# namada-net/masp

Measured on AMD Instinct MI355X. Metric: Spend proofs/sec, higher is better.
Workload: dtype u32; 1 GPU; BASELINE.json configs[3]: batch of 256 distinct Spend proofs per step on one MI355X (throughput mode); proofs_per_gpu=4352, distinct_witnesses_per_gpu=256, ntt_log2=17, batch_cap=256, slots=4, calls_in_flight=4, hw_queues=4, parallelism=proofs sharded over 1 GPU(s), no data-path collective, gather of the proofs

## Files before the change

### include/masp_hip.h

```cpp
#ifndef MASP_HIP_H
#define MASP_HIP_H
#include <stddef.h>
#include <stdint.h>

#ifdef __cplusplus
extern "C" {
#endif

#define MASP_HIP_OK 0
#define MASP_HIP_E_INVALID_ARG 1
#define MASP_HIP_E_PARAMS_FORMAT 2
#define MASP_HIP_E_PARAMS_SHAPE 3
#define MASP_HIP_E_NO_DEVICE 4
#define MASP_HIP_E_HIP 5
#define MASP_HIP_E_UNEXPECTED_IDENTITY 6
#define MASP_HIP_E_NOT_LOADED 7
#define MASP_HIP_E_SCALAR_RANGE 8
#define MASP_HIP_E_POINT_ENCODING 9
#define MASP_HIP_E_CAPACITY 10

#define MASP_HIP_MAX_CIRCUITS 8
#define MASP_HIP_SPEND 0
#define MASP_HIP_OUTPUT 1
#define MASP_HIP_CONVERT 2

typedef struct masp_hip_ctx masp_hip_ctx;

typedef struct {
    uint32_t n_inputs, n_aux, n_constraints;
    const uint32_t* a_rowptr; const uint32_t* a_col; const uint8_t* a_coef;
    const uint32_t* b_rowptr; const uint32_t* b_col; const uint8_t* b_coef;
    const uint32_t* c_rowptr; const uint32_t* c_col; const uint8_t* c_coef;
} masp_hip_r1cs;

typedef struct {
    uint32_t circuit;
    const uint8_t* inputs;
    const uint8_t* aux;
    const uint8_t* a;
    const uint8_t* b;
    const uint8_t* c;
    uint8_t r[32], s[32];
    uint32_t aux_form;
    uint32_t reserved;
} masp_hip_job;
#define MASP_HIP_AUX_CANONICAL 0
#define MASP_HIP_AUX_MONTGOMERY 1

int masp_hip_device_count(void);
int masp_hip_device_pci_bus_id(int device, char* out, size_t cap);

typedef struct {
    uint32_t struct_size;
    int32_t slots;
    int32_t batch_cap;
    int32_t ntt_sub_batch;
    int32_t window_bits_h;
    int32_t window_bits_la;
    int32_t window_bits_b;
    int32_t window_bits_b2_lone;
    int32_t witness_nontrivial_percent;
    int32_t bucket_tree_levels;
    int32_t bucket_tree_sub_batch;
    int32_t bucket_tree_levels_g2;
    int32_t bucket_tree_scratch_mb;
    int32_t bucket_tree_fallback_proofs;
    int32_t lone_proof_graph;
    int32_t hw_queues;
    int32_t window_bits_h_lone;
    int32_t digit_recoding;
    int32_t window_bits_b2;
} masp_hip_options;
void masp_hip_options_default(masp_hip_options* opt);
#define MASP_HIP_MAX_USEFUL_HW_QUEUES 20
int masp_hip_runtime_prepare(int hw_queues, int overwrite);

int masp_hip_ctx_create(int device, masp_hip_ctx** out);
int masp_hip_ctx_create_ex(const int* devices, int n_devices, const masp_hip_options* opt, masp_hip_ctx** out);
int masp_hip_ctx_get_options(const masp_hip_ctx* ctx, masp_hip_options* out);
int masp_hip_ctx_create_multi(const int* devices, int n_devices, masp_hip_ctx** out);
int masp_hip_ctx_set_boolean_block_bits(masp_hip_ctx* ctx, int32_t bits);
int masp_hip_ctx_get_boolean_block_bits(const masp_hip_ctx* ctx, int32_t* out);
#define MASP_HIP_QUOTIENT_EVALUATION 0
#define MASP_HIP_QUOTIENT_COEFFICIENT 1
int masp_hip_ctx_set_quotient_form(masp_hip_ctx* ctx, int32_t form);
int masp_hip_ctx_get_quotient_form(const masp_hip_ctx* ctx, int32_t* out);
#define MASP_HIP_QUOTIENT_FUSED 0
#define MASP_HIP_QUOTIENT_SEPARATE 1
int masp_hip_ctx_set_quotient_schedule(masp_hip_ctx* ctx, int32_t schedule);
int masp_hip_ctx_get_quotient_schedule(const masp_hip_ctx* ctx, int32_t* out);
int masp_hip_ctx_set_tree_entry_share(masp_hip_ctx* ctx, int32_t percent);
int masp_hip_ctx_get_tree_entry_share(const masp_hip_ctx* ctx, int32_t* out);
int masp_hip_r1cs_boolean_variables(const masp_hip_r1cs* cs, uint8_t* out);
uint64_t masp_hip_tree_entry_bound(uint32_t n, int32_t window_bits, uint32_t n_witness, uint32_t n_boolean, int32_t share_percent);
int masp_hip_circuit_tree_entry_bounds(const masp_hip_ctx* ctx, uint32_t slot, uint64_t bounds[4], int32_t window_bits[4]);
int masp_hip_ctx_device_count(const masp_hip_ctx* ctx);
int masp_hip_ctx_device_proofs(const masp_hip_ctx* ctx, uint64_t* counts, int cap);
int masp_hip_ctx_device_status(const masp_hip_ctx* ctx, int32_t* status, int cap, uint64_t* requeued);
int masp_hip_ctx_inject_fault(masp_hip_ctx* ctx, int device, uint32_t nth);
int masp_hip_ctx_stream_concurrency(masp_hip_ctx* ctx, int mains_only, int* n_streams, int* concurrent);
int masp_hip_ctx_lone_graph_launches(const masp_hip_ctx* ctx, uint64_t* out);
void masp_hip_ctx_destroy(masp_hip_ctx* ctx);
const char* masp_hip_strerror(int code);
const char* masp_hip_last_error(const masp_hip_ctx* ctx);

int masp_hip_circuit_load(masp_hip_ctx* ctx, uint32_t slot, const uint8_t* params, size_t params_len, const masp_hip_r1cs* cs);
#define MASP_HIP_CIRCUIT_G1_ENDOMORPHISM 1u
int masp_hip_circuit_flags(const masp_hip_ctx* ctx, uint32_t slot, uint32_t* flags);

int masp_hip_circuit_quotient_form(const masp_hip_ctx* ctx, uint32_t slot, int32_t* form);
int masp_hip_circuit_eval_bases(const masp_hip_ctx* ctx, uint32_t slot, uint8_t* bases, size_t cap_points, size_t* n_points, uint32_t* input_cols,
                                size_t cap_inputs, size_t* n_input_cols);

int masp_hip_prove(masp_hip_ctx* ctx, uint32_t slot, const uint8_t* inputs, const uint8_t* aux, const uint8_t* a,
                   const uint8_t* b, const uint8_t* c, const uint8_t r[32], const uint8_t s[32], uint8_t proof_out[192]);
int masp_hip_prove_batch(masp_hip_ctx* ctx, size_t n, const masp_hip_job* jobs, uint8_t* proofs_out);

int masp_hip_generate_parameters(masp_hip_ctx* ctx, const masp_hip_r1cs* cs, const uint8_t toxic[160], uint8_t* out, size_t cap,
                                 size_t* out_len);
size_t masp_hip_parameters_max_size(const masp_hip_r1cs* cs);

int masp_hip_msm_g1(masp_hip_ctx* ctx, const uint8_t* bases, const uint8_t* scalars, size_t n, uint8_t out[96]);
int masp_hip_msm_g2(masp_hip_ctx* ctx, const uint8_t* bases, const uint8_t* scalars, size_t n, uint8_t out[192]);
int masp_hip_msm_g1_multi(masp_hip_ctx* ctx, const uint8_t* bases, size_t n, const uint8_t* scalars, size_t np, int window_bits,
                          uint8_t* out);
int masp_hip_msm_g2_multi(masp_hip_ctx* ctx, const uint8_t* bases, size_t n, const uint8_t* scalars, size_t np, int window_bits,
                          uint8_t* out);
int masp_hip_msm_g1_multi_ex(masp_hip_ctx* ctx, const uint8_t* bases, size_t n, const uint8_t* scalars, size_t np, int window_bits,
                             int block_bits, size_t sub_lo, size_t sub_hi, uint8_t* out, uint32_t* bucket0_entries);
int masp_hip_msm_g2_multi_ex(masp_hip_ctx* ctx, const uint8_t* bases, size_t n, const uint8_t* scalars, size_t np, int window_bits,
                             int block_bits, size_t sub_lo, size_t sub_hi, uint8_t* out, uint32_t* bucket0_entries);
int masp_hip_quotient_h(masp_hip_ctx* ctx, const uint8_t* a, const uint8_t* b, const uint8_t* c, size_t nrows,
                        uint32_t logm, uint8_t* h_out);
int masp_hip_ntt(masp_hip_ctx* ctx, uint8_t* data, uint32_t logm, int inverse);

typedef struct masp_hip_vk masp_hip_vk;
int masp_hip_vk_prepare(masp_hip_ctx* ctx, const uint8_t* params, size_t params_len, masp_hip_vk** out);
void masp_hip_vk_free(masp_hip_vk* vk);
int masp_hip_verify_batch(masp_hip_ctx* ctx, masp_hip_vk* vk, size_t n, const uint8_t* proofs, const uint8_t* public_inputs,
                          uint32_t n_public, const uint8_t* z, int* all_valid);
int masp_hip_verify_each(masp_hip_ctx* ctx, masp_hip_vk* vk, size_t n, const uint8_t* proofs, const uint8_t* public_inputs,
                         uint32_t n_public, uint8_t* verdicts);
int masp_hip_verify_each_last_timing(masp_hip_vk* vk, double ms[5]);

int masp_hip_jubjub_msm(masp_hip_ctx* ctx, size_t n, const uint8_t* points, const uint8_t* scalars, uint8_t out32[32], int64_t* bad_index);
int masp_hip_redjubjub_verify_batch(masp_hip_ctx* ctx, size_t n, const uint8_t* vks, const uint8_t* sigs, const uint8_t* sighashes,
                                    const uint8_t* kinds, const uint8_t* z, int* all_valid);
int masp_hip_redjubjub_verify_each(masp_hip_ctx* ctx, size_t n, const uint8_t* vks, const uint8_t* sigs, const uint8_t* sighashes,
                                   const uint8_t* kinds, uint8_t* verdicts);

int masp_hip_sapling_trial_decrypt(masp_hip_ctx* ctx, size_t n_ivk, const uint8_t* ivks, size_t n_out, const uint8_t* epks,
                                   const uint8_t* enc_ciphertexts, uint8_t* epk_status, size_t hit_capacity, uint32_t* hit_output,
                                   uint32_t* hit_ivk, uint8_t* hit_keys, size_t* n_hits);
int masp_hip_note_scan_configure(masp_hip_ctx* ctx, int signed_digits, int inversion);
int masp_hip_note_scan_last_timing(masp_hip_ctx* ctx, double ms[2]);

int masp_hip_sapling_compact_trial_decrypt(masp_hip_ctx* ctx, size_t n_ivk, const uint8_t* ivks, size_t n_out, const uint8_t* epks,
                                           const uint8_t* cmus, const uint8_t* enc_compact, int lead_byte, uint8_t* epk_status,
                                           size_t hit_capacity, uint32_t* hit_output, uint32_t* hit_ivk, uint8_t* hit_plaintexts,
                                           uint8_t* hit_pk_d, size_t* n_hits, size_t* n_candidates);
int masp_hip_note_scan_compact_last_timing(masp_hip_ctx* ctx, double ms[3]);

int masp_hip_sapling_output_recovery_scan(masp_hip_ctx* ctx, size_t n_ovk, const uint8_t* ovks, size_t n_out, const uint8_t* cvs,
                                          const uint8_t* epks, const uint8_t* cmus, const uint8_t* out_ciphertexts, size_t hit_capacity,
                                          uint32_t* hit_output, uint32_t* hit_ovk, uint8_t* hit_ocks, size_t* n_hits);
int masp_hip_out_recovery_last_timing(masp_hip_ctx* ctx, double ms[2]);

int masp_hip_merkle_tree_complete(masp_hip_ctx* ctx, unsigned height0, size_t n, const uint8_t* row, uint8_t* nodes_out, size_t nodes_capacity,
                                  size_t* n_nodes, uint8_t root32[32], size_t n_paths, const uint64_t* positions, uint8_t* paths_out,
                                  int64_t* bad_index);
int masp_hip_merkle_last_timing(masp_hip_ctx* ctx, double ms[3]);
int masp_hip_merkle_tree_append(masp_hip_ctx* ctx, uint64_t start, const uint8_t frontier[32 * 32], size_t n, const uint8_t* row,
                                uint8_t* nodes_out, size_t nodes_capacity, size_t* n_nodes, int64_t* bad_index);

int masp_hip_batch_upload(masp_hip_ctx* ctx, size_t n, const masp_hip_job* jobs);
int masp_hip_batch_prove_resident(masp_hip_ctx* ctx, int handle, uint8_t* proofs_out, float* elapsed_ms);
int masp_hip_batch_prove_resident_steps(masp_hip_ctx* ctx, int handle, size_t steps, const uint8_t* rs, uint8_t* proofs_out,
                                        float* elapsed_ms);
int masp_hip_batch_free(masp_hip_ctx* ctx, int handle);
int masp_hip_bench_msm(masp_hip_ctx* ctx, int handle, size_t job, int which, int iters, float* avg_ms, uint32_t* n_bases);

int masp_hip_profile_enable(masp_hip_ctx* ctx, int on);
int masp_hip_profile_read(masp_hip_ctx* ctx, double* total_ms, uint64_t* launches, uint64_t* alg_bytes);
int masp_hip_profile_read_split(masp_hip_ctx* ctx, double ms[8]);
int masp_hip_profile_read_lone(masp_hip_ctx* ctx, double ms[12]);
void* masp_hip_host_alloc(masp_hip_ctx* ctx, size_t bytes);
void masp_hip_host_free(masp_hip_ctx* ctx, void* ptr);
int masp_hip_sync(masp_hip_ctx* ctx);

#ifdef __cplusplus
}
#endif

// ... 22 lines not shown
```

### masp_amd/csrc/device/msm.hpp

```cpp
#pragma once
#include <hip/hip_runtime.h>

#include "curve.hpp"
#include "quad.hpp"
#include "oct.hpp"
#include "io.hpp"
#include "msm_geom.h"

namespace masp {

#define MSM_P (blockIdx.y)

template <class O, int BYTES>
__global__ void k_msm_import(const uint8_t* __restrict__ raw, TabRow<O>* __restrict__ tab, uint32_t n, int* __restrict__ status) {
    uint32_t i = blockIdx.x * blockDim.x + threadIdx.x;
    if (i >= n) return;
    Affine<O> p;
    int st;
    if constexpr (BYTES == 96)
        st = g1_read_uncompressed(raw + (size_t)i * 96, p);
    else
        st = g2_read_uncompressed(raw + (size_t)i * 192, p);
    if (st & ~PT_INFINITY) {
        atomicOr(status, st);
        p.x = O::zero();
        p.y = O::zero();
    } else if (st & PT_INFINITY) {
        atomicOr(status, PT_INFINITY);
    }
    tab[i].p = p;
}
template <class O>
__global__ void __launch_bounds__(64) k_msm_precompute(TabRow<O>* __restrict__ tab, uint32_t n, int c, int W) {
    uint32_t i = blockIdx.x * blockDim.x + threadIdx.x;
    if (i >= n) return;
    Affine<O> p = tab[i].p;
    for (int j = 1; j < W; ++j) {
        Xyzz<O> q = xyzz_dbl_affine(p);
        for (int k = 1; k < c; ++k) q = xyzz_dbl(q);
        p = xyzz_to_affine(q);
        tab[(size_t)j * n + i].p = p;
    }
}
template <class O>
__global__ void __launch_bounds__(64) k_msm_subset_rows(TabRow<O>* __restrict__ tab, MsmSubset sub, uint32_t n_rows) {
    const uint32_t r = blockIdx.x * blockDim.x + threadIdx.x;
    if (r >= n_rows) return;
    const uint32_t per = sub.patterns(), rb = r / per, pattern = r % per + 1u, i0 = (sub.b_first + rb) << sub.bits;
    Xyzz<O> acc = xyzz_inf<O>();
    for (uint32_t t = 0; t < (1u << sub.bits); ++t)
        if ((pattern >> t) & 1u) xyzz_madd_nc(acc, tab[i0 + t].p, false);
    if (xyzz_is_inf(acc)) atomicOr(&sub.bad[rb >> 5], 1u << (rb & 31u));
    tab[(size_t)sub.row0 + r].p = xyzz_to_affine(acc);
}


#ifndef MASP_TAIL_MIN_WAVES
#define MASP_TAIL_MIN_WAVES 1
#endif
template <class O>
__device__ __forceinline__ Xyzz<O> xyzz_load(const Xyzz<typename O::Base>* __restrict__ p, uint32_t h) {
    if constexpr (O::PARTS == 1) {
        const Xyzz<typename O::Base> v = *p;
        return reinterpret_cast<const Xyzz<O>&>(v);
    } else {
        const typename O::T* q = reinterpret_cast<const typename O::T*>(p);
        const uint32_t part = h % O::PARTS;
        Xyzz<O> r;
        r.X = q[part];
        r.Y = q[O::PARTS + part];
        r.ZZ = q[2 * O::PARTS + part];
        r.ZZZ = q[3 * O::PARTS + part];
        return r;
    }
}
template <class O>
__device__ __forceinline__ void xyzz_store(Xyzz<typename O::Base>* __restrict__ p, const Xyzz<O>& v, uint32_t h) {
    if constexpr (O::PARTS == 1) {
        if (h == 0) *p = reinterpret_cast<const Xyzz<typename O::Base>&>(v);
    } else {
        if (h >= O::PARTS) return;
        typename O::T* q = reinterpret_cast<typename O::T*>(p);
        q[h] = v.X;
        q[O::PARTS + h] = v.Y;
        q[2 * O::PARTS + h] = v.ZZ;
        q[3 * O::PARTS + h] = v.ZZZ;
    }
}
template <class O>
__global__ void __launch_bounds__(64, MASP_TAIL_MIN_WAVES)
k_msm_bucket_gather(const Xyzz<typename O::Base>* __restrict__ part, const uint32_t* __restrict__ start, uint32_t nb, uint32_t nchunks,
                    Xyzz<typename O::Base>* __restrict__ bkt, uint32_t* __restrict__ heavy, uint32_t* __restrict__ n_heavy, uint32_t heavy_span) {
    constexpr uint32_t LN = O::LANES;
    const uint32_t b = (blockIdx.x * blockDim.x + threadIdx.x) / LN, h = threadIdx.x % LN;
    if (b >= nb) return;
    part += (size_t)MSM_P * ((size_t)nchunks + nb);
    start += (size_t)MSM_P * (nb + 1);
    bkt += (size_t)MSM_P * nb;
    heavy += (size_t)MSM_P * nb;
    n_heavy += MSM_P;
    const uint32_t s0 = start[b], s1 = start[b + 1];
    Xyzz<O> acc = xyzz_inf<O>();
    if (s1 > s0) {
        const uint32_t K = msm_chunk_len(start[nb], nchunks);
        const uint32_t c0 = s0 / K, c1 = (s1 - 1) / K;
        if (c1 - c0 >= heavy_span) {
            if (h == 0) heavy[atomicAdd(n_heavy, 1u)] = b;
            return;
        }
        acc = xyzz_load<O>(part + c0 + b, h);
        for (uint32_t c = c0 + 1; c <= c1; ++c) xyzz_add_nc(acc, xyzz_load<O>(part + c + b, h));
    }
    xyzz_store<O>(bkt + b, acc, h);
}
template <class O>
__global__ void __launch_bounds__(64, MASP_TAIL_MIN_WAVES)
k_msm_bucket_gather_split(const Xyzz<typename O::Base>* __restrict__ part, const uint32_t* __restrict__ start, uint32_t nb, uint32_t nchunks,
                          Xyzz<typename O::Base>* __restrict__ bkt, uint32_t* __restrict__ heavy, uint32_t* __restrict__ n_heavy, uint32_t heavy_span,
                          uint32_t nbw) {
    constexpr uint32_t LN = O::LANES;
    const uint32_t h = threadIdx.x % LN;
    part += (size_t)MSM_P * ((size_t)nchunks + nb);
    start += (size_t)MSM_P * (nb + 1);
    bkt += (size_t)MSM_P * nb;
    heavy += (size_t)MSM_P * nb;
// ... 35 lines not shown
}
template <class O>
__device__ __forceinline__ Xyzz<O> xyzz_shfl_down(const Xyzz<O>& p, int d) {
    Xyzz<O> r;
    const uint32_t* src = reinterpret_cast<const uint32_t*>(&p);
    uint32_t* dst = reinterpret_cast<uint32_t*>(&r);
#pragma unroll
    for (uint32_t i = 0; i < sizeof(Xyzz<O>) / 4; ++i) dst[i] = (uint32_t)__shfl_down((int)src[i], d, 64);
    return r;
}
template <class O, uint32_t THREADS, uint32_t SPLIT = 1>
__global__ void __launch_bounds__(THREADS, MASP_TAIL_MIN_WAVES)
k_msm_bucket_heavy(const Xyzz<typename O::Base>* __restrict__ part, const uint32_t* __restrict__ start, uint32_t nb, uint32_t nchunks,
                   Xyzz<typename O::Base>* __restrict__ bkt, const uint32_t* __restrict__ heavy, const uint32_t* __restrict__ n_heavy,
                   Xyzz<typename O::Base>* __restrict__ hparts) {
    constexpr uint32_t LN = O::LANES, WE = 64 / LN, EL = THREADS / LN;
    __shared__ Xyzz<typename O::Base> sh[THREADS / 64];
    const uint32_t tid = threadIdx.x, e = tid / LN, h = tid % LN, le = (tid & 63) / LN, wid = tid >> 6;
    part += (size_t)MSM_P * ((size_t)nchunks + nb);
    start += (size_t)MSM_P * (nb + 1);
    bkt += (size_t)MSM_P * nb;
    heavy += (size_t)MSM_P * nb;
    n_heavy += MSM_P;
    if constexpr (SPLIT > 1) hparts += (size_t)MSM_P * MSM_HEAVY_SLOTS;
    const uint32_t nh = *n_heavy;
    const uint32_t K = msm_chunk_len(start[nb], nchunks);
    const uint32_t share = blockIdx.x % SPLIT, nwg = gridDim.x / SPLIT;
    for (uint32_t hb = blockIdx.x / SPLIT; hb < nh; hb += nwg) {
        const uint32_t b = heavy[hb];
        uint32_t c0 = start[b] / K, c1 = (start[b + 1] - 1) / K;
        const bool split = SPLIT > 1 && hb < MSM_HEAVY_SLOTS / SPLIT;
        if (split) {
            const uint32_t len = (c1 - c0 + SPLIT) / SPLIT;
            c0 += share * len;
            c1 = c0 + len - 1 < c1 ? c0 + len - 1 : c1;
        } else if (share != 0) {
            continue;
        }
        Xyzz<O> acc = xyzz_inf<O>();
        for (uint32_t c = c0 + e; c <= c1 && c1 + 1 > c0; c += EL) xyzz_add_nc(acc, xyzz_load<O>(part + c + b, h));
        const uint32_t span = c1 + 1 > c0 ? c1 - c0 + 1 : 0;
        for (uint32_t d = WE / 2; d >= 1; d >>= 1) {
            if (d >= span) continue;
            Xyzz<O> other = xyzz_shfl_down(acc, (int)(d * LN));
            if (le < d) xyzz_add_nc(acc, other);
        }
        if constexpr (THREADS > 64) {
            if (le == 0) xyzz_store<O>(sh + wid, acc, h);
            __syncthreads();
            if (e == 0)
                for (uint32_t w = 1; w < THREADS / 64; ++w) xyzz_add_nc(acc, xyzz_load<O>(sh + w, h));
        }
        if (e == 0) xyzz_store<O>(split ? hparts + hb * SPLIT + share : bkt + b, acc, h);
        if constexpr (THREADS > 64) __syncthreads();
    }
}
template <class O, uint32_t SPLIT>
__global__ void __launch_bounds__(64, MASP_TAIL_MIN_WAVES)
k_msm_heavy_join(const Xyzz<typename O::Base>* __restrict__ hparts, const uint32_t* __restrict__ heavy, const uint32_t* __restrict__ n_heavy, uint32_t nb,
                 Xyzz<typename O::Base>* __restrict__ bkt) {
    constexpr uint32_t LN = O::LANES, PER = 64 / (LN * SPLIT);
    static_assert(PER >= 1, "a bucket's shares fit one wave");
    const uint32_t e = threadIdx.x / LN, h = threadIdx.x % LN, share = e % SPLIT, hb = blockIdx.x * PER + e / SPLIT;
    hparts += (size_t)MSM_P * MSM_HEAVY_SLOTS;
    heavy += (size_t)MSM_P * nb;
    bkt += (size_t)MSM_P * nb;
    const uint32_t nh = n_heavy[MSM_P], lim = nh < MSM_HEAVY_SLOTS / SPLIT ? nh : MSM_HEAVY_SLOTS / SPLIT;
    if (hb >= lim) return;
    Xyzz<O> acc = xyzz_load<O>(hparts + hb * SPLIT + share, h);
    for (uint32_t d = SPLIT / 2; d >= 1; d >>= 1) {
        Xyzz<O> other = xyzz_shfl_down(acc, (int)(d * LN));
        if (share < d) xyzz_add_nc(acc, other);
    }
    if (share == 0) xyzz_store<O>(bkt + heavy[hb], acc, h);
}

#ifndef MASP_WSUM_PAIR_WAVES
#define MASP_WSUM_PAIR_WAVES 2
#endif
template <class O>
constexpr uint32_t wsum_points_log() {
    return O::LANES > 4 ? WSUM_L_LOG - 1 : WSUM_L_LOG;
}
template <class O, uint32_t G_LOG>
__global__ void __launch_bounds__((1u << wsum_points_log<O>()) * O::LANES, (O::LANES > 1 ? MASP_WSUM_PAIR_WAVES : sizeof(Xyzz<O>) > 200 || G_LOG < 3 ? MASP_TAIL_MIN_WAVES : 2))
k_msm_wsum_level(const Xyzz<typename O::Base>* __restrict__ B, size_t b_stride, uint32_t m, uint32_t off, Xyzz<typename O::Base>* __restrict__ S,
                 Xyzz<typename O::Base>* __restrict__ T, size_t st_stride) {
    constexpr uint32_t LP = 1u << wsum_points_log<O>(), GL = G_LOG + WSUM_L_LOG - wsum_points_log<O>(), G = 1u << GL, CS = G * LP, LN = O::LANES,
                       WE = 64 / LN, NW = LP / WE;
    __shared__ Xyzz<typename O::Base> sh[2][NW];
    const uint32_t tid = threadIdx.x, e = tid / LN, h = tid % LN, le = (tid & 63) / LN, wid = tid >> 6;
    B += MSM_P * b_stride;
    S += MSM_P * st_stride;
    T += MSM_P * st_stride;
    const uint32_t base = blockIdx.x * CS + e * G;
    Xyzz<O> run = xyzz_inf<O>(), acc = xyzz_inf<O>();
    for (uint32_t l = G; l-- > 0;) {
        if (base + l < m) xyzz_add_nc(run, xyzz_load<O>(B + base + l, h));
        if (l > 0 || off) xyzz_add_nc(acc, run);
    }
    Xyzz<O> x = run;
    for (uint32_t d = 1; d < WE; d <<= 1) {
        Xyzz<O> other = xyzz_shfl_down(x, (int)(d * LN));
        if (le + d < WE) xyzz_add_nc(x, other);
    }
    static_assert(NW <= WE, "the waves' totals fit the points of one wave");
    if (le == 0) xyzz_store<O>(&sh[0][wid], x, h);
    __syncthreads();
    if constexpr (NW > 1) {
        if (wid == 0) {
            Xyzz<O> v = le < NW ? xyzz_load<O>(&sh[0][le], h) : xyzz_inf<O>();
            for (uint32_t d = 1; d < NW; d <<= 1) {
                Xyzz<O> other = xyzz_shfl_down(v, (int)(d * LN));
                if (le + d < NW) xyzz_add_nc(v, other);
            }
            Xyzz<O> behind = xyzz_shfl_down(v, (int)LN);
            if (le + 1 < NW) xyzz_store<O>(&sh[0][le], behind, h);
        }
        __syncthreads();
        if (wid + 1 < NW) xyzz_add_nc(x, xyzz_load<O>(&sh[0][wid], h));
    }
    Xyzz<O> y = e > 0 ? x : xyzz_inf<O>();
    for (uint32_t k = 0; k < GL; ++k) y = xyzz_dbl(y);
    xyzz_add_nc(y, acc);
    for (uint32_t d = WE / 2; d >= 1; d >>= 1) {
        Xyzz<O> other = xyzz_shfl_down(y, (int)(d * LN));
        if (le < d) xyzz_add_nc(y, other);
    }
    if (le == 0) xyzz_store<O>(&sh[1][wid], y, h);
    __syncthreads();
    if (wid == 0) {
        if constexpr (NW > 1) {
            y = le < NW ? xyzz_load<O>(&sh[1][le], h) : xyzz_inf<O>();
            for (uint32_t d = NW / 2; d >= 1; d >>= 1) {
                Xyzz<O> other = xyzz_shfl_down(y, (int)(d * LN));
                if (le < d) xyzz_add_nc(y, other);
            }
        }
        if (e == 0) {
            xyzz_store<O>(S + blockIdx.x, x, h);
            xyzz_store<O>(T + blockIdx.x, y, h);
        }
    }
}
template <class O>
__global__ void __launch_bounds__(256) k_xyzz_reduce_block(const Xyzz<O>* __restrict__ in, size_t in_stride, uint32_t n,
                                                           Xyzz<O>* __restrict__ out, size_t out_stride) {
    extern __shared__ uint4 wsum_lds[];
    Xyzz<O>* sh = reinterpret_cast<Xyzz<O>*>(wsum_lds);
    const uint32_t tid = threadIdx.x;
    in += MSM_P * in_stride;
    out += MSM_P * out_stride;
    const uint32_t k = blockIdx.x * 256 + tid;
    Xyzz<O> y = k < n ? in[k] : xyzz_inf<O>();
    for (uint32_t d = 128; d >= 1; d >>= 1) {
        sh[tid] = y;
        __syncthreads();
        if (tid < d) xyzz_add_nc(y, sh[tid + d]);
        __syncthreads();
    }
    if (tid == 0) out[blockIdx.x] = y;
}
template <class O>
__global__ void __launch_bounds__(64) k_msm_combine(const Xyzz<O>* __restrict__ tsum, int levels, int cs_log, Xyzz<O>* __restrict__ out, size_t out_stride) {
    if (blockIdx.x != 0 || threadIdx.x != 0) return;
    tsum += (size_t)MSM_P * 32;
    out += MSM_P * out_stride;
    Xyzz<O> acc = xyzz_inf<O>();
    for (int l = levels - 1; l >= 0; --l) {
        for (int k = 0; k < cs_log; ++k) acc = xyzz_dbl(acc);
        xyzz_add_nc(acc, tsum[l]);
    }
    *out = acc;
}

template <class O>
constexpr uint32_t reduce_lanes_points() {
    return O::LANES > 4 ? 64u : 256u;
}
template <class O>
__global__ void __launch_bounds__(reduce_lanes_points<O>() * O::LANES) k_xyzz_reduce_block_lanes(const Xyzz<typename O::Base>* __restrict__ in, size_t in_stride, uint32_t n,
                                                                            Xyzz<typename O::Base>* __restrict__ out, size_t out_stride) {
    extern __shared__ uint4 wsum_lds[];
    constexpr uint32_t PTS = reduce_lanes_points<O>();
    Xyzz<typename O::Base>* sh = reinterpret_cast<Xyzz<typename O::Base>*>(wsum_lds);
    const uint32_t e = threadIdx.x / O::LANES, h = threadIdx.x % O::LANES;
    in += MSM_P * in_stride;
    out += MSM_P * out_stride;
    const uint32_t k = blockIdx.x * PTS + e;
    Xyzz<O> y = k < n ? xyzz_load<O>(in + k, h) : xyzz_inf<O>();
    for (uint32_t d = PTS / 2; d >= 1; d >>= 1) {
        xyzz_store<O>(sh + e, y, h);
        __syncthreads();
        if (e < d) xyzz_add_nc(y, xyzz_load<O>(sh + e + d, h));
        __syncthreads();
    }
    if (e == 0) xyzz_store<O>(out + blockIdx.x, y, h);
}
template <class O>
__global__ void __launch_bounds__(64) k_msm_combine_lanes(const Xyzz<typename O::Base>* __restrict__ tsum, int levels, int cs_log,
                                                          Xyzz<typename O::Base>* __restrict__ out, size_t out_stride) {
    if (blockIdx.x != 0 || threadIdx.x >= O::LANES) return;
    const uint32_t h = threadIdx.x;
    tsum += (size_t)MSM_P * 32;
    out += MSM_P * out_stride;
    Xyzz<O> acc = xyzz_inf<O>();
    for (int l = levels - 1; l >= 0; --l) {
        for (int k = 0; k < cs_log; ++k) acc = xyzz_dbl(acc);
        xyzz_add_nc(acc, xyzz_load<O>(tsum + l, h));
    }
    xyzz_store<O>(out, acc, h);
}

}
```

### masp_amd/csrc/device/msm_geom.h

```cpp
#pragma once
#include <hip/hip_runtime.h>

#include <cstdint>

namespace masp {

struct MsmGeom {
    int c;
    int W;
    int nb;
};
static inline MsmGeom msm_geom(int c) {
    MsmGeom g;
    g.c = c;
    g.W = (256 + c - 1) / c;
    g.nb = 1 << (c - 1);
    return g;
}
static inline uint32_t msm_mean_digits_x16(const MsmGeom& g) { return (uint32_t)g.W * 16; }

__host__ __device__ static inline uint32_t msm_chunk_len(uint32_t total, uint32_t nchunks) {
    uint32_t k = (total + nchunks - 1) / nchunks;
    return k < 4 ? 4 : k;
}

struct MsmSubset {
    uint32_t bits = 0;
    uint32_t b_first = 0, b_end = 0;
    uint32_t row0 = 0;
    uint32_t* bad = nullptr;
    __host__ __device__ uint32_t bad_words() const { return (b_end - b_first + 31) / 32; }
    __host__ __device__ uint32_t patterns() const { return (1u << (1u << bits)) - 1u; }
    __host__ __device__ uint64_t rows() const { return bits ? (uint64_t)(b_end - b_first) * patterns() : 0; }
};
__host__ __device__ static inline uint32_t msm_range_len(uint32_t n, uint32_t ng) { return ((n + ng - 1) / ng + 63u) & ~63u; }

static constexpr unsigned WSUM_L_LOG = 7, WSUM_L = 1u << WSUM_L_LOG;
static constexpr unsigned WSUM_G_LOG_MIN = 2;
static constexpr unsigned MSM_HEAVY_SPLIT = 8, MSM_HEAVY_SLOTS = 2048;
static constexpr unsigned MSM_SORT_THREADS = 1024;
static constexpr uint32_t MSM_PAD_ENTRY = 0xffffffffu;

}
```

### masp_amd/csrc/device/msm_sort.hpp

```cpp
#pragma once
#include <hip/hip_runtime.h>

#include <cstdint>

#include "msm_geom.h"

namespace masp {

#define MSM_P (blockIdx.y)

struct MsmDigitIter {
    const uint32_t* sw;
    uint32_t carry, mask, half, pos, j;
    int c;
    __device__ __forceinline__ MsmDigitIter(const uint32_t* sw_, const MsmGeom& g)
        : sw(sw_), carry(0), mask((1u << g.c) - 1u), half(1u << (g.c - 1)), pos(0), j(0), c(g.c) {}
    __device__ __forceinline__ uint32_t bits(uint32_t bit) const {
        const uint32_t w = bit >> 5, off = bit & 31u;
        const uint64_t two = ((uint64_t)(w + 1 < 8 ? sw[w + 1] : 0u) << 32) | sw[w];
        return (uint32_t)(two >> off);
    }
    __device__ __forceinline__ bool next(uint32_t& table, uint32_t& bucket, uint32_t& neg) {
        uint32_t v = (bits(pos) & mask) + carry;
        table = j++;
        pos += (uint32_t)c;
        neg = 0;
        carry = 0;
        if (v > half) {
            v = (1u << c) - v;
            neg = 1;
            carry = 1;
        }
        bucket = v - 1;
        return v != 0;
    }
};
__device__ __forceinline__ int msm_scalar_class(const uint32_t* sw) {
    const uint4* sp = reinterpret_cast<const uint4*>(sw);
    uint4 lo = sp[0], hi = sp[1];
    uint32_t rest = lo.y | lo.z | lo.w | hi.x | hi.y | hi.z | hi.w;
    if (rest == 0 && lo.x <= 1) return (int)lo.x;
    return 2;
}
__device__ __forceinline__ uint64_t msm_unit_lanes(int cls, uint32_t i, const MsmSubset& sub, uint32_t& entry) {
    const uint64_t ones = __ballot(cls == 1);
    entry = i;
    if (sub.bits == 0) return ones;
    const uint32_t lane = threadIdx.x & 63u, k = 1u << sub.bits, blk = i >> sub.bits;
    bool covered = false;
    if (cls <= 1 && blk >= sub.b_first && blk < sub.b_end) {
        const uint32_t rb = blk - sub.b_first;
        covered = ((sub.bad[rb >> 5] >> (rb & 31u)) & 1u) == 0;
    }
    const uint64_t boolean = __ballot(covered);
    const uint32_t g0 = lane & ~(k - 1u);
    const uint64_t gm = (uint64_t)((1u << k) - 1u) << g0;
    const bool full = (boolean & gm) == gm;
    const uint32_t pattern = (uint32_t)((ones & gm) >> g0);
    const bool lead = full && lane == g0 && pattern != 0;
    if (lead) entry = sub.row0 + (blk - sub.b_first) * sub.patterns() + pattern - 1u;
    return __ballot(full ? lead : cls == 1);
}
__global__ void __launch_bounds__(1024)
k_msm_hist(const uint32_t* __restrict__ scalars, size_t scalar_stride, uint32_t n, MsmGeom g, uint32_t ng, MsmSubset sub, uint32_t* __restrict__ hist_wg) {
    extern __shared__ uint32_t msm_lds[];
    const uint32_t tid = threadIdx.x, wg = blockIdx.x, nb = (uint32_t)g.nb;
    scalars += MSM_P * scalar_stride;
    hist_wg += ((size_t)MSM_P * ng + wg) * nb;
    for (uint32_t b = tid; b < nb; b += MSM_SORT_THREADS) msm_lds[b] = 0;
    __syncthreads();
    const uint32_t per = msm_range_len(n, ng), lo = wg * per, hi = lo < n && lo + per < n ? lo + per : n;
    for (uint32_t base = lo; base < hi; base += MSM_SORT_THREADS) {
        const uint32_t i = base + tid;
        const uint32_t* sw = scalars + (size_t)i * 8;
        const int cls = i < hi ? msm_scalar_class(sw) : 0;
        uint32_t unit_entry;
        const uint64_t units = msm_unit_lanes(cls, i, sub, unit_entry);
        if (cls != 2) {
            if (units && (uint32_t)__ffsll((unsigned long long)units) - 1u == (tid & 63u)) atomicAdd(&msm_lds[0], (uint32_t)__popcll(units));
        } else {
            MsmDigitIter it(sw, g);
            for (int j = 0; j < g.W; ++j) {
                uint32_t table, bucket, neg;
                if (it.next(table, bucket, neg)) atomicAdd(&msm_lds[bucket], 1u);
            }
        }
    }
    __syncthreads();
    for (uint32_t b = tid; b < nb; b += MSM_SORT_THREADS) hist_wg[b] = msm_lds[b];
}
__global__ void __launch_bounds__(256)
k_msm_offsets_cols(uint32_t* __restrict__ hist_wg, uint32_t ng, uint32_t nb, uint32_t* __restrict__ dense) {
    hist_wg += (size_t)MSM_P * ng * nb;
    dense += (size_t)MSM_P * (nb + 1);
    const uint32_t b = blockIdx.x * blockDim.x + threadIdx.x;
    if (b >= nb) return;
    uint32_t v = 0;
    for (uint32_t w0 = 0; w0 < ng; w0 += 16) {
        uint32_t h[16];
#pragma unroll
        for (uint32_t k = 0; k < 16; ++k) h[k] = w0 + k < ng ? hist_wg[(size_t)(w0 + k) * nb + b] : 0u;
#pragma unroll
        for (uint32_t k = 0; k < 16; ++k)
            if (w0 + k < ng) {
                hist_wg[(size_t)(w0 + k) * nb + b] = v;
                v += h[k];
            }
    }
    dense[b] = v;
}
static constexpr uint32_t MSM_SCAN_BLOCK = 1024;
__global__ void __launch_bounds__(256)
k_msm_offsets_scan_a(uint32_t nb, uint32_t* __restrict__ start, uint32_t* __restrict__ dense, uint32_t pad_log, uint2* __restrict__ btot) {
    __shared__ uint32_t wsum[2][4];
    start += (size_t)MSM_P * (nb + 1);
    dense += (size_t)MSM_P * (nb + 1);
// ... 298 lines not shown
```

### masp_amd/csrc/internal.h

```cpp
#pragma once
#include <hip/hip_runtime.h>

#include <algorithm>
#include <array>
#include <condition_variable>
#include <cstring>
#include <deque>
#include <map>
#include <memory>
#include <mutex>
#include <shared_mutex>
#include <string>
#include <thread>
#include <vector>

#include "chunk_pipeline.h"
#include "host/eval_form.h"
#include "device/io.hpp"
#include "device/ntt_geom.h"
#include "launch.h"
#include "msm_host.h"
#include <atomic>
#include "util.h"

#ifndef MASP_SUBSET_BITS
#define MASP_SUBSET_BITS 2
#endif
static_assert(MASP_SUBSET_BITS == 0 || MASP_SUBSET_BITS == 2 || MASP_SUBSET_BITS == 3, "subset blocks are 4 or 8 bases wide");
#ifndef MASP_TREE_ENTRY_SHARE
#define MASP_TREE_ENTRY_SHARE 100
#endif
static_assert(MASP_TREE_ENTRY_SHARE >= 1 && MASP_TREE_ENTRY_SHARE <= 100, "a percentage");


namespace masp {

template <class T>
struct DevBuf {
    T* p = nullptr;
    size_t cap = 0;
    ~DevBuf() { release(); }
    void release() {
        if (p) dev_free(p);
        p = nullptr;
        cap = 0;
    }
    int reserve(size_t n) {
        if (n <= cap) return MASP_HIP_OK;
        release();
        HIP_TRY(dev_malloc(&p, sizeof(T) * std::max<size_t>(n, 1)));
        cap = n;
        return MASP_HIP_OK;
    }
    int upload(const T* h, size_t n, hipStream_t s) {
        int rc = reserve(n);
        if (rc) return rc;
        if (n) HIP_TRY(hipMemcpyAsync(p, h, sizeof(T) * n, hipMemcpyHostToDevice, s));
        return MASP_HIP_OK;
    }
};

static inline Fr fr_from_u64_mont(uint64_t x) {
    Fr v = fe_zero<FrCfg>();
    v.v[0] = (uint32_t)x;
    v.v[1] = (uint32_t)(x >> 32);
    return fe_to_mont(v);
}
static inline Fr fr_const(const uint32_t* limbs) {
    Fr v;
    for (int i = 0; i < 8; ++i) v.v[i] = limbs[i];
    return v;
}

struct NttDomain {
    uint32_t logm = 0;
    size_t m = 0;
    DevBuf<Fr> tw_fwd, tw_inv, coset_scale, h_scale;
    DevBuf<Fr> coset_scale_rev;
    Fr c_scale;
    Fr e_scale;
    int init(uint32_t logm_, hipStream_t s) {
        logm = logm_;
        m = (size_t)1 << logm;
        Fr omega = fr_const(FrCfg::ROOT_OF_UNITY);
        for (uint32_t i = logm; i < 32; ++i) omega = fe_sqr(omega);
        Fr omega_inv = fe_inv(omega);
        Fr minv = fe_inv(fr_from_u64_mont(m));
        Fr g = fr_const(FrCfg::GEN), ginv = fr_const(FrCfg::GEN_INV);
        uint32_t e[2] = {(uint32_t)m, (uint32_t)((uint64_t)m >> 32)};
        const Fr zinv = fe_inv(fe_sub(fe_pow(g, e, 2), fe_one<FrCfg>()));
        const Fr mzinv = fe_mul(minv, zinv);
        c_scale = fe_from_mont(mzinv);
        e_scale = fe_from_mont(zinv);
        Fr one = fe_one<FrCfg>();
        size_t half = std::max<size_t>(m / 2, 1);
        int rc;
        if ((rc = tw_fwd.reserve(half)) || (rc = tw_inv.reserve(half)) || (rc = coset_scale.reserve(m)) || (rc = h_scale.reserve(m))) return rc;
        launch_fr_powers(s, tw_fwd.p, (uint32_t)half, omega, one, 0);
        launch_fr_powers(s, tw_inv.p, (uint32_t)half, omega_inv, one, 0);
        launch_fr_powers(s, coset_scale.p, (uint32_t)m, g, minv, 0);
        launch_fr_powers(s, h_scale.p, (uint32_t)m, ginv, mzinv, 1);
        if (ntt_fused_ok(logm)) {
            if ((rc = coset_scale_rev.reserve(m))) return rc;
            launch_fr_powers_bitrev(s, coset_scale_rev.p, logm, g, minv);
        }
        HIP_TRY(hipStreamSynchronize(s));
        return MASP_HIP_OK;
    }
    void passes(hipStream_t s, Fr* data, const Fr* tw, uint32_t np = 1) const {
        for (uint32_t s0 = 0; s0 < logm;) {
            uint32_t nst = std::min<uint32_t>(NTT_LT, logm - s0);
            launch_ntt_pass(s, data, tw, logm, s0, nst, np);
            s0 += nst;
        }
    }
};

struct Circuit {
    uint32_t n_inputs = 0, n_aux = 0, n_constraints = 0, nrows = 0, logm = 0;
    size_t m = 0;
    DevBuf<uint32_t> rowptr[3], col[3];
    DevBuf<uint32_t> row_order[3];
    uint32_t n_long_rows[3] = {0, 0, 0};
    DevBuf<Fr> coef[3];
    DevBuf<uint32_t> a_var, b_var;
    uint32_t na = 0, nbq = 0;
    DevBuf<VkDevice> vk;
    DevBuf<G1Xyzz> fb1;
    DevBuf<G2Xyzz> fb2;
    BasesG1 h, l, a, b1;
    BasesG1 hl;
    BasesG1 hl_eval;
    DevBuf<uint32_t> eval_in_var;
    uint32_t n_eval_in = 0;
    std::vector<uint32_t> eval_inputs;
    BasesG2 b2;
    BasesG2 b2_lone;
    bool g1_endo = false;
    NttDomain* dom = nullptr;
};

struct Slot {
    hipStream_t stream = nullptr;
    hipEvent_t done = nullptr;
    MsmWorkspace<FpOps> ws1;
    MsmWorkspace<Fp2Ops> ws2;
    static constexpr int N_AUX = 4;
    hipStream_t aux[N_AUX] = {nullptr, nullptr, nullptr, nullptr};
    hipEvent_t ev_fork = nullptr, ev_sort_b = nullptr, ev_fixed = nullptr, ev_join[N_AUX] = {nullptr, nullptr, nullptr, nullptr};
    hipEvent_t ev_uploaded = nullptr;
    MsmWorkspace<FpOps> ws_l, ws_a, ws_b;
    DevBuf<Fr> w, inp, abc, wm, ev[3], x0, x1, h, hl, sa, sb;
    DevBuf<G1Xyzz> res1, asm1;
    DevBuf<G2Xyzz> res2, asm2;
    DevBuf<uint32_t> rs;
    DevBuf<uint8_t> proof;
    DevBuf<int> flags;
    MsmProfile prof;
    bool profiling = false;
    static constexpr int N_LONE_MARKS = 12;
    hipEvent_t ev_lone[N_LONE_MARKS] = {};
    bool lone_marked = false;
    void lone_mark(hipStream_t st, int id) {
        if (!profiling) return;
        if (!ev_lone[id] && hipEventCreate(&ev_lone[id]) != hipSuccess) return;
        (void)hipEventRecord(ev_lone[id], st);
        if (id == N_LONE_MARKS - 1) lone_marked = true;
    }
    uint32_t ntt_sub = 8;
    const std::atomic<int>* quotient_schedule = nullptr;
    uint8_t* h_stage = nullptr;
    size_t h_stage_cap = 0;
    uint8_t* h_proof = nullptr;
    size_t h_proof_cap = 0;
    int* h_flags = nullptr;
    struct LoneGraph {
        const void *circuit, *w, *abc, *rs, *proof;
        size_t w_stride;
        uint32_t np;
        bool mont;
        int runs;
        bool dead;
        hipGraphExec_t exec;
    };
    std::vector<LoneGraph> graphs;
    uint64_t graph_epoch = 0;
    bool lone_graph = false;
    std::atomic<uint64_t> graph_launches{0};
    void drop_graphs() {
        for (auto& g : graphs)
            if (g.exec) hipGraphExecDestroy(g.exec);
        graphs.clear();
    }
    ~Slot() {
        drop_graphs();
        if (done) hipEventDestroy(done);
        for (hipEvent_t e : ev_join)
            if (e) hipEventDestroy(e);
        for (hipEvent_t e : ev_lone)
            if (e) hipEventDestroy(e);
        if (ev_fork) hipEventDestroy(ev_fork);
        if (ev_uploaded) hipEventDestroy(ev_uploaded);
        if (ev_sort_b) hipEventDestroy(ev_sort_b);
        if (ev_fixed) hipEventDestroy(ev_fixed);
        if (h_stage) hipHostFree(h_stage);
        if (h_proof) hipHostFree(h_proof);
        if (h_flags) hipHostFree(h_flags);
    }
    void configure(const masp_hip_options& o) {
        ntt_sub = (uint32_t)o.ntt_sub_batch;
        ws1.tree_levels = o.bucket_tree_levels;
        ws2.tree_levels = o.bucket_tree_levels_g2;
        ws1.tree_levels_shared = o.bucket_tree_levels_g2;
        ws1.tree_sub = ws2.tree_sub = (uint32_t)o.bucket_tree_sub_batch;
        ws2.tree.arena = &ws1.tree.own;
        ws1.tree.own.limit = (size_t)o.bucket_tree_scratch_mb << 20;
        lone_graph = o.lone_proof_graph > 0;
    }
    int init(const std::array<hipStream_t, 5>& streams) {
        stream = streams[0];
        for (int i = 0; i < N_AUX; ++i) aux[i] = streams[1 + i];
        HIP_TRY(hipEventCreateWithFlags(&done, hipEventDisableTiming));
        HIP_TRY(hipEventCreateWithFlags(&ev_fork, hipEventDisableTiming));
        HIP_TRY(hipEventCreateWithFlags(&ev_uploaded, hipEventDisableTiming));
        HIP_TRY(hipEventCreateWithFlags(&ev_sort_b, hipEventDisableTiming));
        HIP_TRY(hipEventCreateWithFlags(&ev_fixed, hipEventDisableTiming));
        for (hipEvent_t& e : ev_join) HIP_TRY(hipEventCreateWithFlags(&e, hipEventDisableTiming));
        HIP_TRY(hipHostMalloc(&h_flags, sizeof(int)));
        int rc;
        if ((rc = flags.reserve(1))) return rc;
        return reserve_batch(1);
    }
    int reserve_batch(size_t np) {
        int rc;
        if ((rc = res1.reserve(4 * np)) || (rc = res2.reserve(np)) || (rc = asm1.reserve(6 * np)) || (rc = asm2.reserve(np)) || (rc = rs.reserve(16 * np)) || (rc = proof.reserve(192 * np))) return rc;
        if (np > h_proof_cap) {
            if (h_proof) hipHostFree(h_proof);
            h_proof = nullptr;
            HIP_TRY(hipHostMalloc(&h_proof, 192 * np));
            h_proof_cap = np;
        }
        return MASP_HIP_OK;
    }
    int stage_reserve(size_t bytes) {
        if (bytes <= h_stage_cap) return MASP_HIP_OK;
        if (h_stage) hipHostFree(h_stage);
        h_stage = nullptr;
        HIP_TRY(hipHostMalloc(&h_stage, bytes));
        h_stage_cap = bytes;
        return MASP_HIP_OK;
    }
};

struct ResidentBatch {
    size_t n = 0;
    std::vector<uint32_t> circuit;
    std::vector<size_t> order;
    std::vector<size_t> w_off;
    DevBuf<Fr> w;
    DevBuf<uint32_t> rs;
};

struct StreamTable {
    hipStream_t main = nullptr;
    std::vector<std::array<hipStream_t, 5>> slot;
    hipStream_t vk[2] = {nullptr, nullptr};
    std::vector<hipStream_t> distinct() const {
        std::vector<hipStream_t> out;
        auto add = [&](hipStream_t s) {
            if (s && std::find(out.begin(), out.end(), s) == out.end()) out.push_back(s);
        };
        add(main);
        for (const auto& row : slot)
            for (hipStream_t s : row) add(s);
        for (hipStream_t s : vk) add(s);
        return out;
    }
    ~StreamTable() {
        for (hipStream_t s : distinct()) (void)hipStreamDestroy(s);
    }
};

}

using masp::Circuit;
using masp::DevBuf;
using masp::Fr;
using masp::G1Affine;
using masp::G1Xyzz;
using masp::G2Affine;
using masp::G2Xyzz;
using masp::NttDomain;
using masp::ResidentBatch;
using masp::Slot;

struct masp_hip_ctx {
    static constexpr size_t MAX_SLOTS = 64;
    int device = 0;
    std::vector<masp_hip_ctx*> children;
    masp_hip_options opt{};
    int boolean_block_bits = MASP_SUBSET_BITS;
    int quotient_form = 0;
    std::atomic<int> quotient_schedule{0};
    int tree_entry_share = MASP_TREE_ENTRY_SHARE;
    int n_slots = 4;
    size_t batch_cap = 256;
    std::shared_mutex mu;
    mutable std::mutex slot_mu;
    std::condition_variable slot_cv;
    std::vector<char> slot_busy;
    std::string err;
    masp::StreamTable streams;
    std::unique_ptr<Circuit> circ[MASP_HIP_MAX_CIRCUITS];
    std::map<uint32_t, std::unique_ptr<NttDomain>> domains;
    std::vector<std::unique_ptr<Slot>> slots;
    std::vector<std::unique_ptr<ResidentBatch>> batches;
    bool profiling = false;
    std::atomic<uint64_t> proofs_done{0};
    std::unique_ptr<std::atomic<int>[]> dev_status;
    std::atomic<uint64_t> requeued{0};
    std::atomic<uint32_t> fault_countdown{0};
    std::atomic<unsigned> vk_next{0};
    int main_streams_concurrent = 0;
    std::mutex upload_mu;
    hipEvent_t upload_tail = nullptr;
    std::atomic<uint64_t> block_tree_fallbacks{0};
    std::atomic<uint32_t> block_tree_sub{0xffffffffu};
    DevBuf<Fr> tmp_scalars;
    DevBuf<uint8_t> tmp_out;
    DevBuf<G1Xyzz> tmp_g1;
    DevBuf<G2Xyzz> tmp_g2;
    DevBuf<G1Affine> fb_g1;
    DevBuf<G2Affine> fb_g2;
    std::mutex jj_mu;
    DevBuf<uint8_t> jj_points, jj_scalars, jj_partial;
    DevBuf<int> jj_status;
    DevBuf<uint32_t> jj_out;
    struct NoteScanSet {
        DevBuf<uint8_t> epk, raw, ct, pts, status, hit_keys;
        DevBuf<uint32_t> count, hit_idx;
    };
    std::mutex ns_mu;
    NoteScanSet ns[2];
    DevBuf<uint32_t> ns_digits;
    std::atomic<int> ns_signed_digits{1}, ns_inversion{0};
    double ns_last_ms[2] = {0, 0};
    struct NoteScanCompactSet {
        DevBuf<uint8_t> cmu, enc, cand, state, hit_idx, hit_data;
        DevBuf<uint32_t> count, list;
    };
    NoteScanCompactSet nsc[2];
    DevBuf<uint8_t> nsc_ivks;
    DevBuf<uint8_t> nsc_table;
    double nsc_last_ms[3] = {0, 0, 0};
    struct OutRecoverySet {
        DevBuf<uint8_t> cv, cmu, epk, cout, cols, hit_ocks;
        DevBuf<uint32_t> count, hit_idx;
    };
    OutRecoverySet orc[2];
    DevBuf<uint32_t> orc_ovks;
    double orc_last_ms[2] = {0, 0};
    DevBuf<uint32_t> mt_nodes, mt_bad, mt_paths, mt_empties;
    DevBuf<uint64_t> mt_pos;
    double mt_last_ms[3] = {0, 0, 0};
};

namespace masp {

static inline int fail(masp_hip_ctx* ctx, int rc) {
    if (rc == MASP_HIP_E_HIP) {
        std::lock_guard<std::mutex> g(ctx->slot_mu);
        ctx->err = last_hip_error();
    }
    return rc;
}

#define FIRST_DEVICE(ctx) ((ctx) && !(ctx)->children.empty() ? (ctx)->children[0] : (ctx))

static inline int get_domain(masp_hip_ctx* ctx, uint32_t logm, NttDomain** out) {
    auto it = ctx->domains.find(logm);
    if (it == ctx->domains.end()) {
        std::unique_ptr<NttDomain> d(new NttDomain);
        int rc = d->init(logm, ctx->streams.main);
        if (rc) return rc;
// ... 26 lines not shown
```

### masp_amd/csrc/k_msm_g1_lone.hip

```cpp
#define MASP_TAILS_QUAD_UNIT
#include "msm_impl.hpp"

namespace masp {
template void msm_tails_enqueue<FpOps, FpQuadOps>(hipStream_t, MsmWorkspace<FpOps>&, const uint32_t*, uint32_t, uint32_t, uint32_t, bool, Xyzz<FpOps>*, size_t);
}
```

### masp_amd/csrc/k_msm_g2_lone.hip

```cpp
#define MASP_TAILS_OCT_UNIT
#include "msm_impl.hpp"

namespace masp {
template void msm_tails_enqueue<Fp2Ops, Fp2OctOps>(hipStream_t, MsmWorkspace<Fp2Ops>&, const uint32_t*, uint32_t, uint32_t, uint32_t, bool, Xyzz<Fp2Ops>*, size_t);
}
```

### masp_amd/csrc/k_msm_sort.hip

```cpp
#include <cstring>

#include "device/msm_sort.hpp"
#include "msm_host.h"

namespace masp {

int msm_sort_enqueue(hipStream_t s, uint32_t n, const MsmGeom& g, MsmSortBuf& sb, const uint32_t* d_scalars, size_t scalar_stride,
                                   uint32_t np, uint32_t pad_log, const MsmSubset& sub) {
    static_assert((1u << 15) / MSM_SCAN_BLOCK <= 64, "k_msm_offsets_scan_b: a wave's lanes fetch the block totals");
    if (g.c < 2 || g.nb > (1 << 15)) {
        last_hip_error() = "MSM window width must be 2..16 bits: the bucket histogram lives in LDS";
        return MASP_HIP_E_INVALID_ARG;
    }
    const uint64_t rows = (uint64_t)n * (uint32_t)g.W + sub.rows();
    if (rows > 0x7ffffffeull) {
        last_hip_error() = "msm_sort_enqueue: the base set has more table rows than an entry's 31 bits can name";
        return MASP_HIP_E_INVALID_ARG;
    }
    if (sub.bits && ((sub.bits != 2 && sub.bits != 3) || sub.b_end < sub.b_first || ((uint64_t)sub.b_end << sub.bits) > n || sub.row0 != n * (uint32_t)g.W ||
                     !sub.bad)) {
        last_hip_error() = "msm_sort_enqueue: subset rows that do not belong to this base set";
        return MASP_HIP_E_INVALID_ARG;
    }
    if (pad_log > 12) {
        last_hip_error() = "msm_sort_enqueue: runs can be aligned to at most 2^12 entries";
        return MASP_HIP_E_INVALID_ARG;
    }
    int rc = sb.reserve(n, g, np, pad_log, rows);
    if (rc) return rc;
    sb.n = n;
    sb.np = np;
    sb.g = g;
    sb.pad_log = pad_log;
    sb.ent_stride = MsmSortBuf::padded_entries(n, g, pad_log);
    const uint32_t ng = MsmSortBuf::ranges_for(n, np), nb = g.nb;
    const uint32_t wide = MsmSortBuf::msm_rows_wide(rows) ? 1u : 0u;
    const int part_entry = wide ? 6 : 5, part_fixed = 4 * (4 * 256 + 8), part_w_max = std::min(30, (160 * 1024 - part_fixed) / ((int)MSM_PART_TILE * part_entry));
    const bool two_pass = nb >= MSM_FINE && g.W <= part_w_max && (uint64_t)(nb >> MSM_FINE_LOG) * np >= 8;
    const int part_lds = part_fixed + part_entry * (int)MSM_PART_TILE * g.W;
    static PerDeviceOnce once;
    const bool lds_ok = once([] {
        int bytes = 4 << 15;
        const int part_bytes = 4 * (4 * 256 + 8) + 5 * (int)MSM_PART_TILE * 30;
        return hipFuncSetAttribute((const void*)k_msm_hist, hipFuncAttributeMaxDynamicSharedMemorySize, bytes) == hipSuccess &&
               hipFuncSetAttribute((const void*)k_msm_scatter, hipFuncAttributeMaxDynamicSharedMemorySize, bytes) == hipSuccess &&
               hipFuncSetAttribute((const void*)k_msm_partition, hipFuncAttributeMaxDynamicSharedMemorySize, part_bytes) == hipSuccess;
    });
    if (!lds_ok) {
        last_hip_error() = "hipFuncSetAttribute(MaxDynamicSharedMemorySize) failed";
        return MASP_HIP_E_HIP;
    }
    MASP_LAUNCH(k_msm_hist, dim3(ng, np), dim3(MSM_SORT_THREADS), 4 * nb, s, d_scalars, scalar_stride, n, g, ng, sub, sb.hist_wg);
    MASP_LAUNCH(k_msm_offsets_cols, dim3((nb + 255) / 256, np), dim3(256), 0, s, sb.hist_wg, ng, nb, sb.dense);
    const uint32_t scan_blocks = (nb + MSM_SCAN_BLOCK - 1) / MSM_SCAN_BLOCK;
    MASP_LAUNCH(k_msm_offsets_scan_a, dim3(scan_blocks, np), dim3(256), 0, s, nb, sb.start, sb.dense, pad_log, sb.btot);
    MASP_LAUNCH(k_msm_offsets_scan_b, dim3(scan_blocks, np), dim3(256), 0, s, nb, sb.start, sb.dense, sb.btot);
    if (two_pass) {
        const uint32_t nbins = nb >> MSM_FINE_LOG;
        const uint32_t cw = std::min(ng, 4u);
        MASP_LAUNCH(k_msm_coarse, dim3(nbins, np, (ng + cw - 1) / cw), dim3(64 * cw), 0, s, sb.hist_wg, ng, nb, sb.crel);
        MASP_LAUNCH(k_msm_partition, dim3(ng, np), dim3(MSM_PART_TILE), part_lds, s, d_scalars, scalar_stride, n, g, ng, sub, sb.crel, sb.dense, sb.tmp, sb.tmpf, wide);
        MASP_LAUNCH(k_msm_bucketize, dim3(nbins, np), dim3(1024), 0, s, sb.tmp, sb.tmpf, (size_t)n * g.W, sb.dense, sb.start, nb, sb.sorted, sb.ent_stride, wide);
    } else {
        if (pad_log) HIP_TRY(hipMemsetAsync(sb.sorted, 0xff, 4 * sb.ent_stride * np, s));
        MASP_LAUNCH(k_msm_scatter, dim3(ng, np), dim3(MSM_SORT_THREADS), 4 * nb, s, d_scalars, scalar_stride, n, g, ng, sub, sb.hist_wg, sb.start, sb.sorted,
                        sb.ent_stride);
    }
    return launch_status();
}

}
```

### masp_amd/csrc/msm_host.h

```cpp
#pragma once
#include <hip/hip_runtime.h>

#include <cstdio>
#include <vector>

#include "device/curve.hpp"
#include "device/msm_geom.h"
#include "util.h"

#ifndef MASP_LONE_NARROW_LANES_LOG
#define MASP_LONE_NARROW_LANES_LOG 16
#endif
namespace masp {

template <class O, int BYTES>
struct MsmBases {
    MsmGeom g{};
    uint32_t n = 0;
    uint32_t n_eff = 0;
    uint64_t ent_bound = 0;
    static uint64_t entry_bound(uint32_t n_, const MsmGeom& g_, uint64_t n_full) {
        n_full = std::min<uint64_t>(n_full, n_);
        return n_full * (uint32_t)g_.W + (n_ - n_full);
    }
    size_t tree_entries(uint32_t pad_log) const {
        const size_t unit = (size_t)1 << pad_log, worst = ((size_t)n * g.W + (size_t)g.nb * (unit - 1) + unit - 1) / unit * unit;
        if (!ent_bound) return worst;
        return std::min<size_t>(worst, ((size_t)ent_bound + (size_t)g.nb * (unit - 1) + unit - 1) / unit * unit);
    }
    TabRow<O>* tab = nullptr;
    int import_status = 0;
    MsmSubset sub;
    uint32_t sub_lo = 0, sub_hi = 0;
    const MsmSubset& subset() const { return sub; }
    uint64_t rows() const { return (uint64_t)n * (uint32_t)g.W + sub.rows(); }

    ~MsmBases() { release(); }
    void release() {
        if (tab) dev_free(tab);
        if (sub.bad) dev_free(sub.bad);
        tab = nullptr;
        sub = MsmSubset();
    }
    static MsmGeom pick_geom(uint32_t n_eff) {
        int c = n_eff >= (1u << 16) ? 16 : n_eff >= (1u << 12) ? 12 : n_eff >= (1u << 8) ? 10 : 7;
        return msm_geom(c);
    }
    int load_device(const uint8_t* d_raw, uint32_t n_, hipStream_t s, uint32_t n_eff = 0xffffffffu, int force_c = 0, int sub_bits_ = 0,
                    uint32_t sub_lo_ = 0, uint32_t sub_hi_ = 0xffffffffu);
    int load_host(const uint8_t* raw, uint32_t n_, hipStream_t s, uint32_t n_eff = 0xffffffffu, int force_c = 0, int sub_bits_ = 0, uint32_t sub_lo_ = 0,
                  uint32_t sub_hi_ = 0xffffffffu) {
        uint8_t* d_raw = nullptr;
        if (n_) {
            HIP_TRY(dev_malloc(&d_raw, (size_t)n_ * BYTES));
            HIP_TRY(hipMemcpyAsync(d_raw, raw, (size_t)n_ * BYTES, hipMemcpyHostToDevice, s));
        }
        int rc = load_device(d_raw, n_, s, n_eff, force_c, sub_bits_, sub_lo_, sub_hi_);
        if (d_raw) dev_free(d_raw);
        return rc;
    }
};

struct MsmSortBuf {
    size_t cap_ent = 0, cap_nb = 0, cap_np = 0, cap_hist = 0, cap_crel = 0;
    uint32_t *sorted = nullptr, *hist_wg = nullptr, *start = nullptr;
    uint32_t *tmp = nullptr, *crel = nullptr;
    uint8_t* tmpf = nullptr;
    bool has_tmpf = false;
    static bool msm_rows_wide(uint64_t rows) { return rows > (1u << 24); }
    uint32_t* dense = nullptr;
    uint2* btot = nullptr;
    uint32_t n = 0, np = 0;
    MsmGeom g{};
    uint32_t pad_log = 0;
    size_t ent_stride = 0;
    static size_t padded_entries(uint32_t n_, const MsmGeom& g_, uint32_t pad_log_) {
        const size_t unit = (size_t)1 << pad_log_;
        return ((size_t)n_ * g_.W + (size_t)g_.nb * (unit - 1) + unit - 1) / unit * unit;
    }

    ~MsmSortBuf() { release(); }
    void release() {
        void* ptrs[] = {sorted, hist_wg, start, tmp, crel, dense, tmpf, btot};
        for (void* p : ptrs)
            if (p) dev_free(p);
        sorted = hist_wg = start = tmp = crel = dense = nullptr;
        tmpf = nullptr;
        btot = nullptr;
        has_tmpf = false;
        cap_ent = cap_nb = cap_np = cap_hist = cap_crel = 0;
    }
    static uint32_t ranges_for(uint32_t n, uint32_t np) {
        uint32_t ng = std::max(1u, 512u / std::max(np, 1u));
        ng = std::min(ng, 64u);
        return std::max(1u, std::min(ng, (n + 1023) / 1024));
    }
    int reserve(uint32_t n_, const MsmGeom& g_, uint32_t np_, uint32_t pad_log_ = 0, uint64_t rows_ = 0) {
        const size_t need_ent = std::max(padded_entries(n_, g_, pad_log_), cap_ent), ng = ranges_for(n_, np_);
        const size_t bins = std::max<size_t>(g_.nb >> 7, 1);
        const size_t hist_need = (size_t)np_ * ng * g_.nb, crel_need = (size_t)np_ * ng * bins;
        const bool want_tmpf = has_tmpf || msm_rows_wide(std::max<uint64_t>(rows_, (uint64_t)n_ * (uint32_t)g_.W));
        if (need_ent <= cap_ent && (size_t)g_.nb <= cap_nb && np_ <= cap_np && hist_need <= cap_hist && crel_need <= cap_crel && want_tmpf == has_tmpf)
            return MASP_HIP_OK;
        const size_t need_nb = std::max<size_t>(g_.nb, cap_nb), need_np = std::max<size_t>(np_, cap_np);
        const size_t rows = std::max<size_t>(need_np, 512);
        const size_t need_hist = std::max(std::max(hist_need, cap_hist), rows * need_nb);
        const size_t need_crel = std::max(std::max(crel_need, cap_crel), rows * std::max<size_t>(need_nb >> 7, 1));
        release();
        auto alloc_all = [&]() -> int {
            HIP_TRY(dev_malloc(&sorted, need_np * 4 * std::max<size_t>(need_ent, 1)));
            HIP_TRY(dev_malloc(&hist_wg, 4 * need_hist));
            HIP_TRY(dev_malloc(&start, need_np * 4 * (need_nb + 1)));
            HIP_TRY(dev_malloc(&tmp, need_np * 4 * std::max<size_t>(need_ent, 1)));
            if (want_tmpf) HIP_TRY(dev_malloc(&tmpf, need_np * std::max<size_t>(need_ent, 1)));
            HIP_TRY(dev_malloc(&crel, 4 * need_crel));
            HIP_TRY(dev_malloc(&dense, need_np * 4 * (need_nb + 1)));
            HIP_TRY(dev_malloc(&btot, need_np * sizeof(uint2) * ((need_nb + 1023) / 1024)));
            return MASP_HIP_OK;
        };
        if (int rc = alloc_all()) {
            release();
            return rc;
        }
        has_tmpf = want_tmpf;
        cap_ent = need_ent;
        cap_nb = need_nb;
        cap_np = need_np;
        cap_hist = need_hist;
        cap_crel = need_crel;
        return MASP_HIP_OK;
    }
};

static constexpr int MASP_HIP_E_TREE_SCRATCH = -100;
struct MsmTreeArena {
    uint8_t* p = nullptr;
    size_t cap = 0;
    size_t limit = 0;
    uint64_t refused = 0;
    ~MsmTreeArena() { release(); }
    void release() {
        if (p) dev_free(p);
        p = nullptr;
        cap = 0;
    }
    int reserve(size_t bytes) {
        if (bytes <= cap) return MASP_HIP_OK;
        if (limit && bytes > limit) {
            ++refused;
            return MASP_HIP_E_TREE_SCRATCH;
        }
        release();
        const hipError_t e = dev_malloc(&p, bytes);
        if (e == hipErrorOutOfMemory) {
            (void)hipGetLastError();
            p = nullptr;
            ++refused;
            return MASP_HIP_E_TREE_SCRATCH;
        }
        HIP_TRY(e);
        cap = bytes;
        return MASP_HIP_OK;
    }
};
template <class O>
struct MsmTreeWs {
    typedef typename O::T F;
    static constexpr uint32_t BINV_C = 16, BINV_MID = 4096;
    MsmTreeArena own;
    MsmTreeArena* arena = &own;
    uint32_t *D = nullptr, *Q = nullptr;
    uint2* rec = nullptr;
    F *pre = nullptr, *tp = nullptr, *tinv = nullptr, *bpre = nullptr, *btot = nullptr, *bitot = nullptr, *bpre2 = nullptr;
    F *px[2] = {nullptr, nullptr}, *py[2] = {nullptr, nullptr};
    uint32_t q = 0, nb = 0, T = 0;
    size_t stride[2] = {0, 0};
    size_t pre_cap = 0;
    uint32_t* over_start = nullptr;
    struct MsmProfile* prof = nullptr;

    static size_t scratch_bytes(uint64_t E_ub, uint32_t nb, uint32_t q, uint32_t T);
    int reserve(uint64_t E_ub, uint32_t nb, uint32_t q, uint32_t T);
    void batch_invert(hipStream_t s, const F* in, uint32_t n, F* out);
    const F* points_x() const { return px[T & 1]; }
// ... 133 lines not shown
            Rec r = pool.back();
            pool.pop_back();
            return r;
        }
        Rec r;
        hipEventCreate(&r.e0);
        hipEventCreate(&r.e1);
        r.alg_bytes = 0;
        return r;
    }
    void collect() {
        for (auto& r : recs) {
            float ms = 0;
            if (hipEventElapsedTime(&ms, r.e0, r.e1) == hipSuccess) {
                total_ms += ms;
                ++launches;
                alg_bytes += r.alg_bytes;
            }
            pool.push_back(r);
        }
        recs.clear();
        for (size_t i = 0; i < marks.size(); ++i) {
            float ms = 0;
            if (i && marks[i].tag >= 0 && hipEventElapsedTime(&ms, marks[i - 1].e, marks[i].e) == hipSuccess) split_ms[marks[i].tag] += ms;
            mark_pool.push_back(marks[i].e);
        }
        marks.clear();
    }
    void reset() {
        collect();
        total_ms = 0;
        launches = 0;
        alg_bytes = 0;
        for (double& v : split_ms) v = 0;
    }
};

int msm_sort_enqueue(hipStream_t s, uint32_t n, const MsmGeom& g, MsmSortBuf& sb, const uint32_t* d_scalars, size_t scalar_stride, uint32_t np,
                     uint32_t pad_log = 0, const MsmSubset& sub = MsmSubset());

#ifndef MASP_TREE_PAD_LOG
#define MASP_TREE_PAD_LOG 2
#endif
inline uint32_t msm_tree_levels(uint32_t n_eff, const MsmGeom& g, uint32_t np, int opt) {
    if (np < 8 || opt < 0) return 0;
    if (opt > 0) return std::min<uint32_t>((uint32_t)opt, 12u);
    const uint64_t mean = std::max<uint64_t>((uint64_t)std::max(n_eff, 1u) * msm_mean_digits_x16(g) / 16 / g.nb, 1);
    uint32_t lg = 0;
    while (((uint64_t)1 << lg) < mean) ++lg;
    return std::min(4u, lg > 1 ? lg - 1 : 0u);
}

template <class O>
void msm_launch_accumulate(hipStream_t s, const TabRow<O>* tab, const uint32_t* sorted, size_t ent_stride, const uint32_t* start, uint32_t nb,
                           uint32_t nchunks, Xyzz<O>* part, uint32_t np);

template <class O, int BYTES>
int msm_tree_enqueue(hipStream_t s, const MsmBases<O, BYTES>& B, const MsmSortBuf& sb, MsmTreeWs<O>& tw, uint32_t p0, uint32_t q, uint32_t T,
                     uint32_t* keep_start, uint32_t* over_count);
template <class O>
void msm_launch_accumulate_pts(hipStream_t s, const typename O::T* xs, const typename O::T* ys, size_t pt_stride, const uint32_t* start, uint32_t nb,
                               uint32_t nchunks, Xyzz<O>* part, uint32_t np);

template <class O, int BYTES>
int msm_reduce_enqueue(hipStream_t s, const MsmBases<O, BYTES>& B, const MsmSortBuf& sb, MsmWorkspace<O>& ws, Xyzz<O>* d_out, size_t out_stride,
                       MsmProfile* prof = nullptr);

template <class O, int BYTES>
int msm_enqueue(hipStream_t s, const MsmBases<O, BYTES>& B, MsmWorkspace<O>& ws, const uint32_t* d_scalars, size_t scalar_stride,
                Xyzz<O>* d_out, size_t out_stride, uint32_t np, MsmProfile* prof = nullptr) {
    if (np == 0) return MASP_HIP_OK;
    if (B.n == 0) {
        HIP_TRY(hipMemset2DAsync(d_out, out_stride * sizeof(Xyzz<O>), 0, sizeof(Xyzz<O>), np, s));
        return MASP_HIP_OK;
    }
    const bool tree = msm_tree_levels(B.n_eff, B.g, np, ws.tree_levels) || msm_tree_levels(B.n_eff, B.g, np, ws.tree_levels_shared);
    int rc = msm_sort_enqueue(s, B.n, B.g, ws.sort, d_scalars, scalar_stride, np, tree ? (uint32_t)MASP_TREE_PAD_LOG : 0u, B.subset());
    if (rc) return rc;
    return msm_reduce_enqueue(s, B, ws.sort, ws, d_out, out_stride, prof);
}

template <class A, class B>
inline bool msm_same_sort(const A& a, const B& b) {
    return a.n == b.n && a.g.c == b.g.c;
}

typedef MsmBases<FpOps, 96> BasesG1;
typedef MsmBases<Fp2Ops, 192> BasesG2;

}
```

### masp_amd/csrc/msm_impl.hpp

```cpp
#pragma once
#include "device/msm.hpp"
#include "msm_host.h"
#include <type_traits>

namespace masp {

#ifndef MASP_G2_PAIR_TAILS
#define MASP_G2_PAIR_TAILS 1
#endif
#ifndef MASP_G2_OCT_LONE
#define MASP_G2_OCT_LONE 1
#endif
template <class O>
struct TailLaneOps {
    typedef typename std::conditional<(MASP_G2_PAIR_TAILS) != 0 && std::is_same<O, Fp2Ops>::value, Fp2PairOps, O>::type type;
};

static inline uint32_t log2_ceil_u64(uint64_t n) {
    uint32_t k = 0;
    while ((1ull << k) < n) ++k;
    return k;
}

template <class O, int BYTES>
int MsmBases<O, BYTES>::load_device(const uint8_t* d_raw, uint32_t n_, hipStream_t s, uint32_t n_eff, int force_c, int sub_bits_, uint32_t sub_lo_,
                                    uint32_t sub_hi_) {
        release();
        n = n_;
        this->n_eff = std::min(n_eff, n_);
        g = force_c ? msm_geom(force_c) : pick_geom(std::min(n_eff, n_));
        if (n == 0) return MASP_HIP_OK;
        if (sub_bits_ != 0 && sub_bits_ != 2 && sub_bits_ != 3) {
            last_hip_error() = "MsmBases: subset blocks are 4 or 8 bases wide";
            return MASP_HIP_E_INVALID_ARG;
        }
        sub_lo = std::min(sub_lo_, n);
        sub_hi = std::min(sub_hi_, n);
        if (sub_bits_) {
            MsmSubset u;
            u.bits = (uint32_t)sub_bits_;
            u.b_first = (uint32_t)(((uint64_t)sub_lo + (1u << sub_bits_) - 1) >> sub_bits_);
            u.b_end = sub_hi >> sub_bits_;
            u.row0 = n * (uint32_t)g.W;
            if (u.b_end > u.b_first) sub = u;
        }
        if (rows() > 0x7ffffffeull) {
            sub = MsmSubset();
            last_hip_error() = "MsmBases: more table rows than an entry's 31 bits can name";
            return MASP_HIP_E_INVALID_ARG;
        }
        HIP_TRY(dev_malloc(&tab, sizeof(TabRow<O>) * (size_t)rows()));
        int* d_status;
        HIP_TRY(dev_malloc(&d_status, sizeof(int)));
        HIP_TRY(hipMemsetAsync(d_status, 0, sizeof(int), s));
        dim3 grid((n + 63) / 64), block(64);
        MASP_LAUNCH((k_msm_import<O, BYTES>), grid, block, 0, s, d_raw, tab, n, d_status);
        MASP_LAUNCH((k_msm_precompute<O>), grid, block, 0, s, tab, n, g.c, g.W);
        if (sub.bits) {
            HIP_TRY(dev_malloc(&sub.bad, sizeof(uint32_t) * sub.bad_words()));
            HIP_TRY(hipMemsetAsync(sub.bad, 0, sizeof(uint32_t) * sub.bad_words(), s));
            const uint32_t n_rows = (uint32_t)sub.rows();
            MASP_LAUNCH((k_msm_subset_rows<O>), dim3((n_rows + 63) / 64), block, 0, s, tab, sub, n_rows);
        }
        HIP_TRY(hipMemcpyAsync(&import_status, d_status, sizeof(int), hipMemcpyDeviceToHost, s));
        HIP_TRY(hipStreamSynchronize(s));
        dev_free(d_status);
        return MASP_HIP_OK;
    }

template <class O>
void MsmWorkspace<O>::reduce_to_one(hipStream_t s, uint32_t np, const Xyzz<O>* src, size_t src_stride, uint32_t m, Xyzz<O>* dst, size_t dst_stride,
                                    size_t r_stride) {
        int flip = 0;
        const Xyzz<O>* cur = src;
        size_t cur_stride = src_stride;
        while (true) {
            uint32_t outn = (m + 255) / 256;
            Xyzz<O>* out = outn == 1 ? dst : R[flip];
            size_t out_stride = outn == 1 ? dst_stride : r_stride;
            MASP_LAUNCH((k_xyzz_reduce_block<O>), dim3(outn, np), dim3(256), 256 * sizeof(Xyzz<O>), s, cur, cur_stride, m, out, out_stride);
            if (outn == 1) break;
            cur = out;
            cur_stride = out_stride;
            m = outn;
            flip ^= 1;
        }
    }

template <class O>
template <class OT>
void MsmWorkspace<O>::reduce_to_one_lanes(hipStream_t s, uint32_t np, const Xyzz<O>* src, size_t src_stride, uint32_t m, Xyzz<O>* dst, size_t dst_stride,
                                          size_t r_stride) {
        int flip = 0;
        const Xyzz<O>* cur = src;
        size_t cur_stride = src_stride;
        constexpr uint32_t PTS = reduce_lanes_points<OT>();
        while (true) {
            uint32_t outn = (m + PTS - 1) / PTS;
            Xyzz<O>* out = outn == 1 ? dst : R[flip];
            size_t out_stride = outn == 1 ? dst_stride : r_stride;
            MASP_LAUNCH((k_xyzz_reduce_block_lanes<OT>), dim3(outn, np), dim3(PTS * OT::LANES), PTS * sizeof(Xyzz<O>), s, cur, cur_stride, m, out, out_stride);
            if (outn == 1) break;
            cur = out;
            cur_stride = out_stride;
            m = outn;
            flip ^= 1;
        }
    }

#ifndef MASP_LONE_HEAVY_THREADS
#define MASP_LONE_HEAVY_THREADS 256
#endif
template <class O, class OT>
void msm_tails_enqueue(hipStream_t s, MsmWorkspace<O>& ws, const uint32_t* start, uint32_t nb, uint32_t nchunks, uint32_t np, bool lone, Xyzz<O>* d_out,
                       size_t out_stride) {
    constexpr uint32_t LN = OT::LANES;
    if constexpr (OT::LANES <= 2) {
        if (!lone) {
            const uint32_t nbw = (nb * LN + 63) / 64, ncw = (nchunks * LN + 63) / 64;
            MASP_LAUNCH((k_msm_bucket_gather_split<OT>), dim3(nbw + ncw, np), dim3(64), 0, s, ws.part, start, nb, nchunks, ws.bkt, ws.heavy, ws.n_heavy, 8u, nbw);
        } else {
            MASP_LAUNCH((k_msm_bucket_gather<OT>), dim3((nb * LN + 63) / 64, np), dim3(64), 0, s, ws.part, start, nb, nchunks, ws.bkt, ws.heavy, ws.n_heavy, 12u);
        }
    } else {
        MASP_LAUNCH((k_msm_bucket_gather<OT>), dim3((nb * LN + 63) / 64, np), dim3(64), 0, s, ws.part, start, nb, nchunks, ws.bkt, ws.heavy,
                           ws.n_heavy, lone ? 12u : 8u);
    }
    if (lone) {
        const uint32_t heavy_blocks = std::min<uint32_t>(std::max<uint32_t>(4096u / np, 16u), nb) | 1u;
        if constexpr (OT::REPLICATED) {
            MASP_LAUNCH((k_msm_bucket_heavy<OT, MASP_LONE_HEAVY_THREADS, MSM_HEAVY_SPLIT>), dim3(heavy_blocks * MSM_HEAVY_SPLIT, np), dim3(MASP_LONE_HEAVY_THREADS), 0, s,
                        ws.part, start, nb, nchunks, ws.bkt, ws.heavy, ws.n_heavy, ws.hparts);
            constexpr uint32_t PER = 64 / (LN * MSM_HEAVY_SPLIT);
            const uint32_t joinable = std::min<uint32_t>(nb, MSM_HEAVY_SLOTS / MSM_HEAVY_SPLIT);
            MASP_LAUNCH((k_msm_heavy_join<OT, MSM_HEAVY_SPLIT>), dim3((joinable + PER - 1) / PER, np), dim3(64), 0, s, ws.hparts, ws.heavy, ws.n_heavy, nb, ws.bkt);
        } else {
            MASP_LAUNCH((k_msm_bucket_heavy<OT, MASP_LONE_HEAVY_THREADS>), dim3(heavy_blocks, np), dim3(MASP_LONE_HEAVY_THREADS), 0, s, ws.part, start, nb,
                        nchunks, ws.bkt, ws.heavy, ws.n_heavy, (Xyzz<O>*)nullptr);
        }
    } else {
        const uint32_t heavy_blocks = std::min<uint32_t>(64u, nb) | 1u;
        MASP_LAUNCH((k_msm_bucket_heavy<OT, 64>), dim3(heavy_blocks, np), dim3(64), 0, s, ws.part, start, nb, nchunks, ws.bkt, ws.heavy,
                           ws.n_heavy, (Xyzz<O>*)nullptr);
    }
    uint32_t g_log = nb <= WSUM_L ? 0 : WSUM_G_LOG_MIN;
    if (!lone) {
        const uint32_t hi = 6u;
        g_log = 3;
        while (g_log < hi && (1u << (g_log + 1 + WSUM_L_LOG)) <= nb) ++g_log;
    }
    const uint32_t cs = 1u << (g_log + WSUM_L_LOG);
    const size_t st_stride = (nb + cs - 1) / cs;
    const Xyzz<O>* bk = ws.bkt;
    size_t bk_stride = nb;
    uint32_t m = nb, off = 1;
    int level = 0, flip = 0;
    do {
        uint32_t chunks = (m + cs - 1) / cs;
        const dim3 grid(chunks, np), block((1u << wsum_points_log<OT>()) * LN);
        switch (g_log) {
#define MASP_WSUM_CASE(GL) \
    case GL: MASP_LAUNCH((k_msm_wsum_level<OT, GL>), grid, block, 0, s, bk, bk_stride, m, off, ws.S[flip], ws.T, st_stride); break;
            MASP_WSUM_CASE(0) MASP_WSUM_CASE(2)
            default:
                if constexpr (OT::LANES <= 2) {
                    switch (g_log) { MASP_WSUM_CASE(3) MASP_WSUM_CASE(4) MASP_WSUM_CASE(5) MASP_WSUM_CASE(6) }
                }
                break;
#undef MASP_WSUM_CASE
        }
        if constexpr (OT::REPLICATED)
            ws.template reduce_to_one_lanes<OT>(s, np, ws.T, st_stride, chunks, ws.tsum + level, 32, st_stride);
        else
            ws.reduce_to_one(s, np, ws.T, st_stride, chunks, ws.tsum + level, 32, st_stride);
        bk = ws.S[flip];
        bk_stride = st_stride;
        flip ^= 1;
        m = chunks;
        off = 0;
        ++level;
    } while (m > 1);
    if constexpr (OT::REPLICATED)
        MASP_LAUNCH((k_msm_combine_lanes<OT>), dim3(1, np), dim3(64), 0, s, ws.tsum, level, (int)(g_log + WSUM_L_LOG), d_out, out_stride);
    else
        MASP_LAUNCH((k_msm_combine<O>), dim3(1, np), dim3(64), 0, s, ws.tsum, level, (int)(g_log + WSUM_L_LOG), d_out, out_stride);
}
#ifndef MASP_TAILS_QUAD_UNIT
extern template void msm_tails_enqueue<FpOps, FpQuadOps>(hipStream_t, MsmWorkspace<FpOps>&, const uint32_t*, uint32_t, uint32_t, uint32_t, bool, Xyzz<FpOps>*, size_t);
#endif
#ifndef MASP_TAILS_OCT_UNIT
extern template void msm_tails_enqueue<Fp2Ops, Fp2OctOps>(hipStream_t, MsmWorkspace<Fp2Ops>&, const uint32_t*, uint32_t, uint32_t, uint32_t, bool, Xyzz<Fp2Ops>*, size_t);
#endif

template <class O, int BYTES>
int msm_reduce_enqueue(hipStream_t s, const MsmBases<O, BYTES>& B, const MsmSortBuf& sb, MsmWorkspace<O>& ws, Xyzz<O>* d_out, size_t out_stride,
                       MsmProfile* prof) {
    const MsmGeom& g = B.g;
    const uint32_t n = B.n, np = sb.np;
    if (sb.n != n || sb.g.c != g.c) {
        last_hip_error() = "msm_reduce_enqueue: sort does not match the base set";
        return MASP_HIP_E_INVALID_ARG;
    }
    int rc = ws.reserve(n, g, np);
    if (rc) return rc;
    {
        static PerDeviceOnce once;
        const bool lds_ok = once([] {
            int bytes = 256 * (int)sizeof(Xyzz<O>);
            return hipFuncSetAttribute((const void*)k_xyzz_reduce_block<O>, hipFuncAttributeMaxDynamicSharedMemorySize, bytes) == hipSuccess;
        });
        if (!lds_ok) {
            last_hip_error() = "hipFuncSetAttribute(MaxDynamicSharedMemorySize) failed";
            return MASP_HIP_E_HIP;
        }
    }
    const uint32_t nb = g.nb;
    const uint32_t total = n * g.W;
    const uint32_t nchunks = ws.nchunks_for(n, g, np);
    HIP_TRY(hipMemsetAsync(ws.n_heavy, 0, 4 * np, s));
    MsmProfile::Rec rec{};
    if (prof) {
        rec = prof->acquire();
        rec.alg_bytes = (uint64_t)np * n * (BYTES + 32);
        hipEventRecord(rec.e0, s);
        prof->mark(s, MsmProfile::PH_START);
    }
    const bool lone = np < 8;
    const uint32_t tree_T = sb.pad_log >= 1 ? msm_tree_levels(B.n_eff, g, np, ws.tree_levels) : 0;
    const uint32_t* start = sb.start;
    if (tree_T) {
        const bool bounded = sb.ent_stride > B.tree_entries(sb.pad_log);
        if (bounded && (rc = ws.reserve_tree_over(s))) return rc;
        uint32_t sub = std::max(1u, std::min(ws.tree_sub ? ws.tree_sub : 256u, np));
        if (!ws.tree_sub) {
            const MsmTreeArena& ar = *ws.tree.arena;
            const size_t budget = ar.limit ? ar.limit : std::max(ar.cap, MsmTreeWs<O>::scratch_bytes(sb.ent_stride, nb, std::min(86u, np), tree_T));
            const uint64_t E = std::min<uint64_t>(sb.ent_stride, B.tree_entries(sb.pad_log));
            for (uint32_t k = 1;; ++k) {
                sub = (np + k - 1) / k;
                if (sub <= 8 || MsmTreeWs<O>::scratch_bytes(E, nb, sub, tree_T) <= budget) break;
            }
        }
        ws.tree.prof = prof;
        for (uint32_t p0 = 0; p0 < np;) {
            uint32_t q = std::min(sub, np - p0);
            uint32_t* const keep = ws.startT + (size_t)p0 * (nb + 1);
            rc = msm_tree_enqueue<O, BYTES>(s, B, sb, ws.tree, p0, q, tree_T, keep, ws.d_tree_over);
            while (rc == MASP_HIP_E_TREE_SCRATCH && sub > 8) {
                sub = std::max(8u, sub / 2);
                ws.tree_sub = sub;
                q = std::min(sub, np - p0);
                rc = msm_tree_enqueue<O, BYTES>(s, B, sb, ws.tree, p0, q, tree_T, keep, ws.d_tree_over);
            }
            if (rc == MASP_HIP_E_TREE_SCRATCH) {
                const uint32_t rest = np - p0;
                ws.tree_fallbacks += rest;
                msm_launch_accumulate<O>(s, B.tab, sb.sorted + (size_t)p0 * sb.ent_stride, sb.ent_stride, sb.start + (size_t)p0 * (nb + 1), nb, nchunks,
                                         ws.part + (size_t)p0 * ((size_t)nchunks + nb), rest);
                HIP_TRY(hipMemcpyAsync(ws.startT + (size_t)p0 * (nb + 1), sb.start + (size_t)p0 * (nb + 1), sizeof(uint32_t) * rest * (nb + 1),
                                       hipMemcpyDeviceToDevice, s));
                break;
            }
            if (rc) return rc;
            ws.tree_sub_used = std::min(ws.tree_sub_used, sub);
            msm_launch_accumulate_pts<O>(s, ws.tree.points_x(), ws.tree.points_y(), ws.tree.point_stride(), ws.tree.plan_D(tree_T), nb, nchunks,
                                         ws.part + (size_t)p0 * ((size_t)nchunks + nb), q);
            if (bounded)
                msm_launch_accumulate<O>(s, B.tab, sb.sorted + (size_t)p0 * sb.ent_stride, sb.ent_stride, ws.tree.over_start, nb, nchunks,
                                         ws.part + (size_t)p0 * ((size_t)nchunks + nb), q);
            if (prof) prof->mark(s, MsmProfile::PH_ACC);
            p0 += q;
        }
        if (bounded) HIP_TRY(hipMemcpyAsync(ws.h_tree_over, ws.d_tree_over, sizeof(uint32_t), hipMemcpyDeviceToHost, s));
        ws.tree.prof = nullptr;
        start = ws.startT;
    } else {
        msm_launch_accumulate<O>(s, B.tab, sb.sorted, sb.ent_stride, sb.start, nb, nchunks, ws.part, np);
        if (prof) prof->mark(s, MsmProfile::PH_ACC);
    }
    if (prof) {
        hipEventRecord(rec.e1, s);
        prof->recs.push_back(rec);
    }
    if constexpr (std::is_same<O, FpOps>::value) {
        if (lone)
            msm_tails_enqueue<O, FpQuadOps>(s, ws, start, nb, nchunks, np, lone, d_out, out_stride);
        else
            msm_tails_enqueue<O, FpOps>(s, ws, start, nb, nchunks, np, lone, d_out, out_stride);
    } else {
        if (lone && (MASP_G2_OCT_LONE))
            msm_tails_enqueue<O, Fp2OctOps>(s, ws, start, nb, nchunks, np, lone, d_out, out_stride);
        else
            msm_tails_enqueue<O, typename TailLaneOps<O>::type>(s, ws, start, nb, nchunks, np, lone, d_out, out_stride);
    }
    return launch_status();
}


}
```

### masp_amd/csrc/prover.hip

```cpp
#include <hip/hip_runtime.h>

#include <chrono>
#include <cstring>
#include <map>
#include <memory>
#include <algorithm>
#include <condition_variable>
#include <deque>
#include <mutex>
#include <shared_mutex>
#include <string>
#include <thread>
#include <vector>

#include "internal.h"

using namespace masp;

#ifndef MASP_UPLOAD_CHAIN
#define MASP_UPLOAD_CHAIN 1
#endif

namespace {

// ... 206 lines not shown

static int enqueue_quotient_eval(Slot& sl, const NttDomain& D, const Fr* const in[2], size_t in_stride, uint32_t nrows, uint32_t np, Fr* e_out,
                                 size_t e_stride) {
    hipStream_t s = sl.stream;
    const uint32_t m = (uint32_t)D.m, logm = D.logm;
    const bool fused = ntt_fused_ok(logm) && D.coset_scale_rev.p && !(sl.quotient_schedule && sl.quotient_schedule->load(std::memory_order_relaxed));
    const uint32_t sub_max = fused ? 2 * sl.ntt_sub : sl.ntt_sub;
    const uint32_t sub = sub_max ? std::min(sub_max, np) : np;
    int rc;
    if ((rc = sl.x0.reserve((size_t)2 * m * sub)) || (!fused && (rc = sl.x1.reserve((size_t)2 * m * sub)))) return rc;
    Fr *x0 = sl.x0.p, *x1 = sl.x1.p;
    for (uint32_t p0 = 0; p0 < np; p0 += sub) {
        const uint32_t q = std::min(sub, np - p0);
        const size_t part = (size_t)q * m;
        if (fused) {
            launch_ntt_dif_top(s, in[0] + (size_t)p0 * in_stride, in[1] + (size_t)p0 * in_stride, in_stride, nrows, x0, D.tw_inv.p, logm, q);
            launch_ntt_mid(s, x0, D.tw_inv.p, D.coset_scale_rev.p, D.tw_fwd.p, logm, 2 * q);
            launch_ntt_dit_top_ab(s, x0, part, D.tw_fwd.p, D.e_scale, e_out + (size_t)p0 * e_stride, e_stride, logm, q);
            continue;
        }
        for (int i = 0; i < 2; ++i) launch_ntt_copy_bitrev(s, in[i] + (size_t)p0 * in_stride, in_stride, nrows, x0 + i * part, logm, q);
        D.passes(s, x0, D.tw_inv.p, 2 * q);
        launch_ntt_scale_bitrev(s, x0, D.coset_scale.p, x1, logm, 2 * q);
        D.passes(s, x1, D.tw_fwd.p, 2 * q);
        launch_ntt_ab_eval(s, x1, x1 + part, D.e_scale, e_out + (size_t)p0 * e_stride, m, q, e_stride);
    }
    return MASP_HIP_OK;
}

static int enqueue_proofs(Slot& sl, Circuit& C, uint32_t np, const Fr* d_w, size_t w_stride, const Fr* const d_abc[3], const uint32_t* d_rs,
                          uint8_t* d_proof, bool aux_montgomery = false) {
    hipStream_t s = sl.stream;
    const uint32_t nv = C.n_inputs + C.n_aux;
    int rc;
    if ((rc = sl.reserve_batch(np))) return rc;
    if ((rc = sl.wm.reserve((size_t)nv * np))) return rc;
    const bool lone = np < 8;
    if (aux_montgomery) launch_fr_split_forms(s, const_cast<Fr*>(d_w), w_stride, sl.wm.p, nv, C.n_inputs, np, sl.flags.p);
    if (lone) {
        sl.lone_mark(s, 0);
        HIP_TRY(hipEventRecord(sl.ev_fork, s));
        for (int i = 0; i < Slot::N_AUX; ++i) HIP_TRY(hipStreamWaitEvent(sl.aux[i], sl.ev_fork, 0));
    }
    if (!aux_montgomery) launch_fr_to_mont(s, d_w, w_stride, sl.wm.p, nv, np, sl.flags.p);
    const Fr* in[3] = {nullptr, nullptr, nullptr};
    bool mont_in;
    const bool eval_form = !lone && !d_abc[0] && C.hl_eval.n != 0;
    if (d_abc[0]) {
        in[0] = d_abc[0];
        in[1] = d_abc[1];
        in[2] = d_abc[2];
        mont_in = false;
    } else {
        R1csMatrices M;
        const int n_mat = eval_form ? 2 : 3;
        for (int i = 0; i < n_mat; ++i) {
            if ((rc = sl.ev[i].reserve((size_t)C.nrows * np))) return rc;
            M.rowptr[i] = C.rowptr[i].p;
            M.order[i] = C.row_order[i].p;
            M.n_long[i] = C.n_long_rows[i];
            M.col[i] = C.col[i].p;
            M.coef[i] = C.coef[i].p;
            M.out[i] = sl.ev[i].p;
            in[i] = sl.ev[i].p;
        }
        for (int i = n_mat; i < 3; ++i) {
            M.rowptr[i] = M.order[i] = M.col[i] = nullptr;
            M.coef[i] = nullptr;
            M.out[i] = nullptr;
            M.n_long[i] = 0;
        }
        launch_r1cs_eval(s, M, sl.wm.p, nv, C.n_constraints, C.n_inputs, np, (uint32_t)n_mat);
        mont_in = true;
    }
    if ((rc = sl.sa.reserve((size_t)C.na * np)) || (rc = sl.sb.reserve((size_t)C.nbq * np))) return rc;
    MsmProfile* prof = sl.profiling ? &sl.prof : nullptr;
    const size_t m8 = C.m * 8;
    const bool share_b = C.nbq && msm_same_sort(C.b1, C.b2);
    if (lone) {
        launch_groth16_fixed_g1(sl.aux[0], C.fb1.p, d_rs, 16, sl.asm1.p, np);
        launch_groth16_fixed_g2(sl.aux[0], C.fb2.p, d_rs, 16, sl.asm2.p, np);
        HIP_TRY(hipEventRecord(sl.ev_fixed, sl.aux[0]));
        const bool own_b2 = C.b2_lone.n != 0;
        auto chain_a = [&]() -> int {
            int r;
            if (C.na) launch_gather_scalars(sl.aux[1], d_w, w_stride, C.a_var.p, C.na, sl.sa.p, np);
            if ((r = msm_enqueue(sl.aux[1], C.a, sl.ws_a, (const uint32_t*)sl.sa.p, (size_t)C.na * 8, sl.res1.p + 2, 4, np))) return r;
            sl.lone_mark(sl.aux[1], 1);
            launch_groth16_var_mul(sl.aux[1], 0, sl.res1.p, d_rs, 16, sl.asm1.p, np, C.g1_endo);
            sl.lone_mark(sl.aux[1], 2);
            return MASP_HIP_OK;
        };
        auto chain_b = [&]() -> int {
            int r;
            if (C.nbq) launch_gather_scalars(sl.aux[2], d_w, w_stride, C.b_var.p, C.nbq, sl.sb.p, np);
            HIP_TRY(hipEventRecord(sl.ev_sort_b, sl.aux[2]));
            if (share_b) {
                if ((r = msm_sort_enqueue(sl.aux[2], C.b1.n, C.b1.g, sl.ws_b.sort, (const uint32_t*)sl.sb.p, (size_t)C.nbq * 8, np, 0, C.b1.subset()))) return r;
                if (!own_b2) HIP_TRY(hipEventRecord(sl.ev_sort_b, sl.aux[2]));
                if ((r = msm_reduce_enqueue(sl.aux[2], C.b1, sl.ws_b.sort, sl.ws_b, sl.res1.p + 3, 4))) return r;
            } else if ((r = msm_enqueue(sl.aux[2], C.b1, sl.ws_b, (const uint32_t*)sl.sb.p, (size_t)C.nbq * 8, sl.res1.p + 3, 4, np))) {
                return r;
            }
            sl.lone_mark(sl.aux[2], 3);
            launch_groth16_var_mul(sl.aux[2], 1, sl.res1.p, d_rs, 16, sl.asm1.p, np, C.g1_endo);
            sl.lone_mark(sl.aux[2], 4);
            HIP_TRY(hipStreamWaitEvent(sl.aux[3], sl.ev_sort_b, 0));
            if (own_b2) {
                if ((r = msm_enqueue(sl.aux[3], C.b2_lone, sl.ws2, (const uint32_t*)sl.sb.p, (size_t)C.nbq * 8, sl.res2.p, 1, np))) return r;
            } else if (share_b) {
                if ((r = msm_reduce_enqueue(sl.aux[3], C.b2, sl.ws_b.sort, sl.ws2, sl.res2.p, 1))) return r;
            } else if ((r = msm_enqueue(sl.aux[3], C.b2, sl.ws2, (const uint32_t*)sl.sb.p, (size_t)C.nbq * 8, sl.res2.p, 1, np))) {
                return r;
            }
            sl.lone_mark(sl.aux[3], 5);
            HIP_TRY(hipStreamWaitEvent(sl.aux[3], sl.ev_fixed, 0));
            launch_groth16_finish_b(sl.aux[3], C.vk.p, sl.asm2.p, sl.res2.p, d_proof, np);
            sl.lone_mark(sl.aux[3], 6);
            return MASP_HIP_OK;
        };
        auto chain_l = [&]() -> int {
            return msm_enqueue(sl.aux[0], C.l, sl.ws_l, (const uint32_t*)(d_w + C.n_inputs), w_stride * 8, sl.res1.p + 1, 4, np);
        };
        if ((rc = chain_a()) || (rc = chain_b())) return rc;
        if ((rc = enqueue_quotient(sl, *C.dom, in, C.nrows, C.nrows, mont_in, np))) return rc;
        sl.lone_mark(s, 7);
        if ((rc = msm_enqueue(s, C.h, sl.ws1, (const uint32_t*)sl.h.p, m8, sl.res1.p + 0, 4, np, prof))) return rc;
        sl.lone_mark(s, 8);
        if ((rc = chain_l())) return rc;
        sl.lone_mark(sl.aux[0], 9);
        for (int i = 1; i < Slot::N_AUX - 1; ++i) {
            HIP_TRY(hipEventRecord(sl.ev_join[i], sl.aux[i]));
            HIP_TRY(hipStreamWaitEvent(sl.aux[0], sl.ev_join[i], 0));
        }
        launch_groth16_finish_ac_early(sl.aux[0], C.vk.p, sl.asm1.p, sl.res1.p, d_proof, np);
        HIP_TRY(hipEventRecord(sl.ev_join[0], sl.aux[0]));
        HIP_TRY(hipStreamWaitEvent(s, sl.ev_join[0], 0));
    } else {
        const BasesG1& HL = eval_form ? C.hl_eval : C.hl;
        const size_t hl_stride = HL.n, aux_at = eval_form ? C.m : C.m - 1;
        if ((rc = sl.hl.reserve(hl_stride * np + 1))) return rc;
        if (eval_form) {
            if ((rc = enqueue_quotient_eval(sl, *C.dom, in, C.nrows, C.nrows, np, sl.hl.p, hl_stride))) return rc;
            if (C.n_eval_in) launch_gather_scalars(s, d_w, w_stride, C.eval_in_var.p, C.n_eval_in, sl.hl.p + C.m + C.n_aux, np, hl_stride);
        } else if ((rc = enqueue_quotient(sl, *C.dom, in, C.nrows, C.nrows, mont_in, np, sl.hl.p, hl_stride))) {
            return rc;
        }
        if (C.n_aux)
            HIP_TRY(hipMemcpy2DAsync(sl.hl.p + aux_at, hl_stride * sizeof(Fr), d_w + C.n_inputs, w_stride * sizeof(Fr), (size_t)C.n_aux * sizeof(Fr), np,
                                     hipMemcpyDeviceToDevice, s));
        if (C.na) launch_gather_scalars(s, d_w, w_stride, C.a_var.p, C.na, sl.sa.p, np);
        if (C.nbq) launch_gather_scalars(s, d_w, w_stride, C.b_var.p, C.nbq, sl.sb.p, np);
        if ((rc = msm_enqueue(s, HL, sl.ws1, (const uint32_t*)sl.hl.p, hl_stride * 8, sl.res1.p + 0, 4, np, prof))) return rc;
        HIP_TRY(hipMemset2DAsync(sl.res1.p + 1, 4 * sizeof(G1Xyzz), 0, sizeof(G1Xyzz), np, s));
        const BasesG1 &Aq = C.a, &B1q = C.b1;
        const BasesG2& B2q = C.b2;
        const bool share_bq = share_b;
        if ((rc = msm_enqueue(s, Aq, sl.ws1, (const uint32_t*)sl.sa.p, (size_t)C.na * 8, sl.res1.p + 2, 4, np, prof))) return rc;
        if ((rc = msm_enqueue(s, B1q, sl.ws1, (const uint32_t*)sl.sb.p, (size_t)C.nbq * 8, sl.res1.p + 3, 4, np, prof))) return rc;
        if (share_bq) {
            if ((rc = msm_reduce_enqueue(s, B2q, sl.ws1.sort, sl.ws2, sl.res2.p, 1))) return rc;
        } else if ((rc = msm_enqueue(s, B2q, sl.ws2, (const uint32_t*)sl.sb.p, (size_t)C.nbq * 8, sl.res2.p, 1, np))) {
            return rc;
        }
    }
    if (!lone) {
        launch_groth16_fixed_g1(s, C.fb1.p, d_rs, 16, sl.asm1.p, np);
        launch_groth16_fixed_g2(s, C.fb2.p, d_rs, 16, sl.asm2.p, np);
                launch_groth16_var_mul(s, 2, sl.res1.p, d_rs, 16, sl.asm1.p, np, C.g1_endo);
        launch_groth16_finish_b(s, C.vk.p, sl.asm2.p, sl.res2.p, d_proof, np);
    }
    if (lone)
        launch_groth16_finish_c_late(s, sl.asm1.p, sl.res1.p, d_proof, np);
    else
        launch_groth16_finish_ac(s, C.vk.p, sl.asm1.p, sl.res1.p, d_proof, np);
    if (lone) {
        sl.lone_mark(s, 10);
        HIP_TRY(hipEventRecord(sl.ev_join[Slot::N_AUX - 1], sl.aux[Slot::N_AUX - 1]));
        HIP_TRY(hipStreamWaitEvent(s, sl.ev_join[Slot::N_AUX - 1], 0));
        sl.lone_mark(s, 11);
    }
    return MASP_HIP_OK;
}

static int enqueue_proofs_graphed(Slot& sl, Circuit& C, uint32_t np, const Fr* d_w, size_t w_stride, const Fr* const d_abc[3], const uint32_t* d_rs,
                                  uint8_t* d_proof, bool aux_montgomery) {
    if (np >= 8 || !sl.lone_graph || sl.profiling) return enqueue_proofs(sl, C, np, d_w, w_stride, d_abc, d_rs, d_proof, aux_montgomery);
    const uint64_t epoch = device_alloc_epoch().load(std::memory_order_relaxed);
    if (epoch != sl.graph_epoch) {
        sl.drop_graphs();
        sl.graph_epoch = epoch;
    }
    Slot::LoneGraph* e = nullptr;
// ... 276 lines not shown
                ok = ok && hipStreamCreateWithFlags(&t.slot[si][j], hipStreamNonBlocking) == hipSuccess;
        }
    for (hipStream_t& v : t.vk) ok = ok && hipStreamCreateWithFlags(&v, hipStreamNonBlocking) == hipSuccess;
    if (!ok || separate_main_streams(ctx.get()) != MASP_HIP_OK) return MASP_HIP_E_NO_DEVICE;
    *out = ctx.release();
    return MASP_HIP_OK;
}

static int create_front(const int* devices, int n_devices, const masp_hip_options& opt, masp_hip_ctx** out) {
    std::unique_ptr<masp_hip_ctx> front(new masp_hip_ctx);
    front->device = devices[0];
    front->opt = opt;
    front->n_slots = opt.slots;
    front->batch_cap = (size_t)opt.batch_cap;
    for (int i = 0; i < n_devices; ++i) {
        masp_hip_ctx* ch = nullptr;
        if (int rc = create_single(devices[i], opt, &ch)) {
            for (masp_hip_ctx* c : front->children) masp_hip_ctx_destroy(c);
            return rc;
        }
        front->children.push_back(ch);
    }
    front->dev_status.reset(new std::atomic<int>[n_devices]);
    for (int i = 0; i < n_devices; ++i) front->dev_status[i] = MASP_HIP_OK;
    *out = front.release();
    return MASP_HIP_OK;
}

int masp_hip_ctx_create_ex(const int* devices, int n_devices, const masp_hip_options* opt_in, masp_hip_ctx** out) {
    if (!out || !devices || n_devices <= 0 || n_devices > 64) return MASP_HIP_E_INVALID_ARG;
    if (opt_in && opt_in->struct_size != 0 && opt_in->struct_size < 4 * sizeof(int32_t)) return MASP_HIP_E_INVALID_ARG;
    *out = nullptr;
    const masp_hip_options opt = resolve_options(opt_in);
    return n_devices == 1 ? create_single(devices[0], opt, out) : create_front(devices, n_devices, opt, out);
}

int masp_hip_ctx_get_options(const masp_hip_ctx* ctx, masp_hip_options* out) {
    if (!ctx || !out) return MASP_HIP_E_INVALID_ARG;
    const masp_hip_ctx* c = ctx->children.empty() ? ctx : ctx->children[0];
    const size_t room = out->struct_size ? std::min<size_t>(out->struct_size, sizeof(masp_hip_options)) : sizeof(masp_hip_options);
    if (room < 4 * sizeof(int32_t)) return MASP_HIP_E_INVALID_ARG;
    masp_hip_options full = c->opt, *const caller_out = out;
    out = &full;
    uint64_t fb = 0;
    int sub = out->bucket_tree_sub_batch ? out->bucket_tree_sub_batch : 256;
    auto scan = [&](const masp_hip_ctx* d) {
        std::lock_guard<std::mutex> g(d->slot_mu);
        for (const auto& sl : d->slots) {
            fb += sl->ws1.tree_fallbacks + sl->ws2.tree_fallbacks + sl->ws1.tree_over() + sl->ws2.tree_over();
            for (const uint32_t v : {sl->ws1.tree_sub, sl->ws2.tree_sub, sl->ws1.tree_sub_used, sl->ws2.tree_sub_used})
                if (v) sub = std::min<int>(sub, (int)std::min<uint32_t>(v, 256u));
        }
    };
    if (ctx->children.empty())
        scan(ctx);
    else
        for (const masp_hip_ctx* d : ctx->children) scan(d);
    fb += c->block_tree_fallbacks.load();
    if (c->block_tree_sub.load() != 0xffffffffu) sub = std::min<int>(sub, (int)c->block_tree_sub.load());
    out->bucket_tree_sub_batch = sub;
    out->bucket_tree_fallback_proofs = (int32_t)std::min<uint64_t>(fb, 0x7fffffff);
    full.struct_size = (uint32_t)room;
    memcpy(caller_out, &full, room);
    return MASP_HIP_OK;
}

int masp_hip_ctx_set_boolean_block_bits(masp_hip_ctx* ctx, int32_t bits) {
    if (!ctx || (bits != 0 && bits != -1 && bits != 2 && bits != 3)) return MASP_HIP_E_INVALID_ARG;
    const int resolved = bits == 0 ? (int)(MASP_SUBSET_BITS) : bits < 0 ? 0 : bits;
    auto set = [&](masp_hip_ctx* c) {
        std::unique_lock<std::shared_mutex> lock(c->mu);
        c->boolean_block_bits = resolved;
    };
    set(ctx);
    for (masp_hip_ctx* c : ctx->children) set(c);
    return MASP_HIP_OK;
}
int masp_hip_ctx_get_boolean_block_bits(const masp_hip_ctx* ctx, int32_t* out) {
    if (!ctx || !out) return MASP_HIP_E_INVALID_ARG;
    *out = (ctx->children.empty() ? ctx : ctx->children[0])->boolean_block_bits;
    return MASP_HIP_OK;
}

int masp_hip_ctx_set_quotient_form(masp_hip_ctx* ctx, int32_t form) {
    if (!ctx || (form != MASP_HIP_QUOTIENT_EVALUATION && form != MASP_HIP_QUOTIENT_COEFFICIENT)) return MASP_HIP_E_INVALID_ARG;
    auto set = [&](masp_hip_ctx* c) {
        std::unique_lock<std::shared_mutex> lock(c->mu);
        c->quotient_form = form;
    };
    set(ctx);
    for (masp_hip_ctx* c : ctx->children) set(c);
    return MASP_HIP_OK;
}
int masp_hip_ctx_get_quotient_form(const masp_hip_ctx* ctx, int32_t* out) {
    if (!ctx || !out) return MASP_HIP_E_INVALID_ARG;
    *out = (ctx->children.empty() ? ctx : ctx->children[0])->quotient_form;
    return MASP_HIP_OK;
}

int masp_hip_ctx_set_quotient_schedule(masp_hip_ctx* ctx, int32_t schedule) {
    if (!ctx || (schedule != MASP_HIP_QUOTIENT_FUSED && schedule != MASP_HIP_QUOTIENT_SEPARATE)) return MASP_HIP_E_INVALID_ARG;
    ctx->quotient_schedule.store(schedule, std::memory_order_relaxed);
    for (masp_hip_ctx* c : ctx->children) c->quotient_schedule.store(schedule, std::memory_order_relaxed);
    return MASP_HIP_OK;
}
int masp_hip_ctx_get_quotient_schedule(const masp_hip_ctx* ctx, int32_t* out) {
    if (!ctx || !out) return MASP_HIP_E_INVALID_ARG;
    *out = (ctx->children.empty() ? ctx : ctx->children[0])->quotient_schedule.load(std::memory_order_relaxed);
    return MASP_HIP_OK;
}

int masp_hip_ctx_set_tree_entry_share(masp_hip_ctx* ctx, int32_t percent) {
    if (!ctx || percent < 0 || percent > 100) return MASP_HIP_E_INVALID_ARG;
    const int resolved = percent == 0 ? (int)(MASP_TREE_ENTRY_SHARE) : percent;
    auto set = [&](masp_hip_ctx* c) {
        std::unique_lock<std::shared_mutex> lock(c->mu);
        c->tree_entry_share = resolved;
    };
    set(ctx);
    for (masp_hip_ctx* c : ctx->children) set(c);
    return MASP_HIP_OK;
}
int masp_hip_ctx_get_tree_entry_share(const masp_hip_ctx* ctx, int32_t* out) {
    if (!ctx || !out) return MASP_HIP_E_INVALID_ARG;
    *out = (ctx->children.empty() ? ctx : ctx->children[0])->tree_entry_share;
    return MASP_HIP_OK;
}
int masp_hip_r1cs_boolean_variables(const masp_hip_r1cs* cs, uint8_t* out) {
    if (!cs || !out || cs->n_inputs == 0) return MASP_HIP_E_INVALID_ARG;
    r1cs_boolean_variables(cs, out);
    return MASP_HIP_OK;
}
uint64_t masp_hip_tree_entry_bound(uint32_t n, int32_t window_bits, uint32_t n_witness, uint32_t n_boolean, int32_t share_percent) {
    if (window_bits < 2 || window_bits > 16 || share_percent < 0 || share_percent > 100) return 0;
    return tree_entry_bound(n, window_bits, n_witness, n_boolean, share_percent == 0 ? (int)(MASP_TREE_ENTRY_SHARE) : share_percent);
}
int masp_hip_circuit_tree_entry_bounds(const masp_hip_ctx* ctx, uint32_t slot, uint64_t bounds[4], int32_t window_bits[4]) {
    if (!ctx || !bounds) return MASP_HIP_E_INVALID_ARG;
    if (!ctx->children.empty()) return masp_hip_circuit_tree_entry_bounds(ctx->children[0], slot, bounds, window_bits);
    std::shared_lock<std::shared_mutex> lock(const_cast<masp_hip_ctx*>(ctx)->mu);
    if (slot >= MASP_HIP_MAX_CIRCUITS || !ctx->circ[slot]) return MASP_HIP_E_NOT_LOADED;
    const Circuit& C = *ctx->circ[slot];
    const BasesG1& HL = C.hl_eval.n ? C.hl_eval : C.hl;
    const uint64_t b[4] = {HL.ent_bound, C.a.ent_bound, C.b1.ent_bound, C.b2.ent_bound};
    const int c[4] = {HL.g.c, C.a.g.c, C.b1.g.c, C.b2.g.c};
    for (int i = 0; i < 4; ++i) {
        bounds[i] = b[i];
        if (window_bits) window_bits[i] = c[i];
    }
    return MASP_HIP_OK;
}

int masp_hip_ctx_create(int device, masp_hip_ctx** out) {
    if (!out) return MASP_HIP_E_INVALID_ARG;
    return masp_hip_ctx_create_ex(&device, 1, nullptr, out);
}

int masp_hip_ctx_create_multi(const int* devices, int n_devices, masp_hip_ctx** out) {
    if (!out || !devices || n_devices <= 0 || n_devices > 64) return MASP_HIP_E_INVALID_ARG;
    *out = nullptr;
    return create_front(devices, n_devices, resolve_options(nullptr), out);
}

int masp_hip_ctx_device_proofs(const masp_hip_ctx* ctx, uint64_t* counts, int cap) {
    if (!ctx || !counts || cap < 0) return MASP_HIP_E_INVALID_ARG;
    if (ctx->children.empty()) {
// ... 102 lines not shown
            if (cl[mi][t] >= nv) return MASP_HIP_E_INVALID_ARG;
            if (mi == 0) a_dense[cl[mi][t]] = 1;
            if (mi == 1) b_dense[cl[mi][t]] = 1;
        }
    }
    std::vector<uint32_t> a_var, b_var;
    for (uint32_t i = 0; i < cs->n_inputs; ++i) a_var.push_back(i);
    for (uint32_t v = cs->n_inputs; v < nv; ++v)
        if (a_dense[v]) a_var.push_back(v);
    for (uint32_t v = 0; v < nv; ++v)
        if (b_dense[v]) b_var.push_back(v);
    C->na = a_var.size();
    C->nbq = b_var.size();
    if (L.n_ic != cs->n_inputs || L.n_h < C->m - 1 || L.n_l != cs->n_aux || L.n_a != C->na || L.n_b1 != C->nbq || L.n_b2 != C->nbq)
        return MASP_HIP_E_PARAMS_SHAPE;
    int rc;
    if ((rc = C->a_var.upload(a_var.data(), a_var.size(), s)) || (rc = C->b_var.upload(b_var.data(), b_var.size(), s))) return fail(ctx, rc);
    DevBuf<int> d_flag;
    if ((rc = d_flag.reserve(1))) return fail(ctx, rc);
    hipMemsetAsync(d_flag.p, 0, sizeof(int), s);
    for (int mi = 0; mi < 3; ++mi) {
        uint32_t nnz = rp[mi][cs->n_constraints];
        DevBuf<Fr> raw;
        std::vector<uint32_t> order(cs->n_constraints);
        for (uint32_t r = 0; r < cs->n_constraints; ++r) order[r] = r;
        std::stable_sort(order.begin(), order.end(),
                         [&](uint32_t x, uint32_t y) { return rp[mi][x + 1] - rp[mi][x] > rp[mi][y + 1] - rp[mi][y]; });
        if ((rc = C->row_order[mi].upload(order.data(), order.size(), s))) return fail(ctx, rc);
        C->n_long_rows[mi] = 0;
        for (uint32_t r : order) {
            if (rp[mi][r + 1] - rp[mi][r] < R1CS_LONG_ROW) break;
            ++C->n_long_rows[mi];
        }
        if ((rc = C->rowptr[mi].upload(rp[mi], cs->n_constraints + 1, s)) || (rc = C->col[mi].upload(cl[mi], nnz, s)) ||
            (rc = raw.upload((const Fr*)cf[mi], nnz, s)) || (rc = C->coef[mi].reserve(nnz)))
            return fail(ctx, rc);
        if (nnz) launch_fr_to_mont(s, raw.p, (size_t)0, C->coef[mi].p, nnz, 1, d_flag.p);
        if (hipStreamSynchronize(s) != hipSuccess) return fail(ctx, MASP_HIP_E_HIP);
    }
    if ((rc = C->vk.reserve(1))) return fail(ctx, rc);
    {
        DevBuf<uint8_t> raw;
        if ((rc = raw.upload(params, 864, s))) return fail(ctx, rc);
        DevBuf<int> st;
        if ((rc = st.reserve(1))) return fail(ctx, rc);
        hipMemsetAsync(st.p, 0, sizeof(int), s);
        VkDevice* v = C->vk.p;
        launch_g1_import_one(s, raw.p + 0, &v->alpha_g1, st.p);
        launch_g1_import_one(s, raw.p + 96, &v->beta_g1, st.p);
        launch_g2_import_one(s, raw.p + 192, &v->beta_g2, st.p);
        launch_g1_import_one(s, raw.p + 576, &v->delta_g1, st.p);
        launch_g2_import_one(s, raw.p + 672, &v->delta_g2, st.p);
        int hst = 0, hflag = 0;
        if (hipMemcpyAsync(&hst, st.p, sizeof(int), hipMemcpyDeviceToHost, s) != hipSuccess ||
            hipMemcpyAsync(&hflag, d_flag.p, sizeof(int), hipMemcpyDeviceToHost, s) != hipSuccess || hipStreamSynchronize(s) != hipSuccess) {
            last_hip_error() = "vk import failed";
            return fail(ctx, MASP_HIP_E_HIP);
        }
        if (hflag) return MASP_HIP_E_SCALAR_RANGE;
        if (hst & (PT_BAD_FLAGS | PT_NOT_CANONICAL)) return MASP_HIP_E_PARAMS_FORMAT;
        DevBuf<G1Affine> p1;
        DevBuf<G2Affine> p2;
        if ((rc = p1.reserve(3)) || (rc = p2.reserve(1)) || (rc = C->fb1.reserve(3 * 32 * 255)) || (rc = C->fb2.reserve(32 * 255))) return fail(ctx, rc);
        hipMemcpyAsync(p1.p + 0, &v->delta_g1, sizeof(G1Affine), hipMemcpyDeviceToDevice, s);
        hipMemcpyAsync(p1.p + 1, &v->alpha_g1, sizeof(G1Affine), hipMemcpyDeviceToDevice, s);
        hipMemcpyAsync(p1.p + 2, &v->beta_g1, sizeof(G1Affine), hipMemcpyDeviceToDevice, s);
        hipMemcpyAsync(p2.p, &v->delta_g2, sizeof(G2Affine), hipMemcpyDeviceToDevice, s);
        launch_fixed_table_g1(s, p1.p, C->fb1.p, 3);
        launch_fixed_table_g2(s, p2.p, C->fb2.p, 1);
        if (hipStreamSynchronize(s) != hipSuccess) {
            last_hip_error() = std::string("fixed-base tables failed: ") + hipGetErrorString(hipGetLastError());
            return fail(ctx, MASP_HIP_E_HIP);
        }
        if ((params[576] & 0x40) || (params[672] & 0x40)) return MASP_HIP_E_UNEXPECTED_IDENTITY;
    }
    const uint32_t pct = (uint32_t)ctx->opt.witness_nontrivial_percent;
    auto eff = [&](uint32_t n) { return (uint32_t)((uint64_t)n * pct / 100); };
    const int c_la = ctx->opt.window_bits_la, c_b = ctx->opt.window_bits_b;
    const int c_b2 = ctx->opt.window_bits_b2 > 0 ? ctx->opt.window_bits_b2 : c_b;
    const uint32_t n_h = (uint32_t)(C->m - 1);
    const int c_h = ctx->opt.window_bits_h ? ctx->opt.window_bits_h : n_h >= 49152 ? 16 : n_h >= 16384 ? 15 : 0;
    const int c_h_lone = ctx->opt.window_bits_h_lone ? ctx->opt.window_bits_h_lone : c_h;
    const int sub_bits = ctx->boolean_block_bits;
    if ((rc = C->h.load_host(L.h, (uint32_t)(C->m - 1), s, 0xffffffffu, c_h_lone)) || (rc = C->l.load_host(L.l, L.n_l, s, eff(L.n_l), c_la)) ||
        (rc = C->a.load_host(L.a, L.n_a, s, eff(L.n_a), c_la, sub_bits)) || (rc = C->b1.load_host(L.b_g1, L.n_b1, s, eff(L.n_b1), c_b, sub_bits)) ||
        (rc = C->b2.load_host(L.b_g2, L.n_b2, s, eff(L.n_b2), c_b2, sub_bits)))
        return fail(ctx, rc);
    if (C->b1.sub.bits && C->b2.sub.bits && msm_same_sort(C->b1, C->b2)) {
        const uint32_t words = C->b1.sub.bad_words();
        std::vector<uint32_t> w1(words), w2(words);
        if (hipMemcpyAsync(w1.data(), C->b1.sub.bad, 4 * (size_t)words, hipMemcpyDeviceToHost, s) != hipSuccess ||
            hipMemcpyAsync(w2.data(), C->b2.sub.bad, 4 * (size_t)words, hipMemcpyDeviceToHost, s) != hipSuccess || hipStreamSynchronize(s) != hipSuccess)
            return fail(ctx, MASP_HIP_E_HIP);
        for (uint32_t i = 0; i < words; ++i) w1[i] |= w2[i];
        if (hipMemcpyAsync(C->b1.sub.bad, w1.data(), 4 * (size_t)words, hipMemcpyHostToDevice, s) != hipSuccess ||
            hipMemcpyAsync(C->b2.sub.bad, w1.data(), 4 * (size_t)words, hipMemcpyHostToDevice, s) != hipSuccess || hipStreamSynchronize(s) != hipSuccess)
            return fail(ctx, MASP_HIP_E_HIP);
    }
    {
        const int c_lone = ctx->opt.window_bits_b2_lone;
        if (c_lone > 0 && L.n_b2 && (rc = C->b2_lone.load_host(L.b_g2, L.n_b2, s, eff(L.n_b2), c_lone))) return fail(ctx, rc);
    }
    const int c_hl = c_h ? c_h : ctx->opt.window_bits_h_lone ? 0 : C->h.g.c;
    {
        const size_t nh = C->m - 1;
        std::vector<uint8_t> cat(96 * (nh + L.n_l));
        memcpy(cat.data(), L.h, 96 * nh);
        memcpy(cat.data() + 96 * nh, L.l, 96 * (size_t)L.n_l);
        if ((rc = C->hl.load_host(cat.data(), (uint32_t)(nh + L.n_l), s, 0xffffffffu, c_hl, sub_bits, (uint32_t)nh))) return fail(ctx, rc);
    }
    int st = C->h.import_status | C->l.import_status | C->a.import_status | C->b1.import_status | C->b2.import_status;
    if (st) return MASP_HIP_E_PARAMS_FORMAT;
    {
        DevBuf<int> out;
        if ((rc = out.reserve(1))) return fail(ctx, rc);
        hipMemsetAsync(out.p, 0, sizeof(int), s);
        launch_g1_subgroup_flag(s, C->a.tab, sizeof(*C->a.tab), C->a.n, out.p);
        launch_g1_subgroup_flag(s, C->b1.tab, sizeof(*C->b1.tab), C->b1.n, out.p);
        launch_g1_subgroup_flag(s, &C->vk.p->alpha_g1, 0, 1, out.p);
        launch_g1_subgroup_flag(s, &C->vk.p->beta_g1, 0, 1, out.p);
        launch_g1_subgroup_flag(s, &C->vk.p->delta_g1, 0, 1, out.p);
        int outside = 1;
        if (hipMemcpyAsync(&outside, out.p, sizeof(int), hipMemcpyDeviceToHost, s) != hipSuccess || hipStreamSynchronize(s) != hipSuccess ||
            launch_status() != MASP_HIP_OK)
            return fail(ctx, MASP_HIP_E_HIP);
        C->g1_endo = outside == 0;
    }
    if ((rc = get_domain(ctx, C->logm, &C->dom))) return fail(ctx, rc);
    if (ctx->quotient_form == 0) {
        masp::EvalBases E;
        if ((rc = build_eval_bases(ctx, *C->dom, L.h, L.l, cs, E))) return fail(ctx, rc);
        if (E.usable) {
            const masp::EvalLayout& lay = E.lay;
            if ((rc = C->hl_eval.load_device(E.d_raw.p, (uint32_t)lay.n(), s, 0xffffffffu, c_hl, sub_bits, (uint32_t)lay.aux_off(), (uint32_t)lay.in_off())))
                return fail(ctx, rc);
            if ((rc = C->eval_in_var.upload(lay.used_inputs.data(), lay.used_inputs.size(), s))) return fail(ctx, rc);
            if (hipStreamSynchronize(s) != hipSuccess) return fail(ctx, MASP_HIP_E_HIP);
            C->eval_inputs = lay.used_inputs;
            C->n_eval_in = (uint32_t)lay.used_inputs.size();
            if (C->hl_eval.import_status) {
                C->hl_eval.release();
                C->hl_eval.n = 0;
                C->eval_inputs.clear();
                C->n_eval_in = 0;
            }
        }
    }
    {
        std::vector<uint8_t> is_bool(nv);
        r1cs_boolean_variables(cs, is_bool.data());
        const int share = ctx->tree_entry_share;
        auto count = [&](const uint32_t* vars, size_t k) {
            uint32_t nbool = 0;
            for (size_t i = 0; i < k; ++i) nbool += is_bool[vars ? vars[i] : cs->n_inputs + i];
            return nbool;
        };
        const uint32_t aux_bool = count(nullptr, cs->n_aux);
        auto bound = [&](auto& B, uint32_t n_wit, uint32_t n_bool) {
            if (B.n) B.ent_bound = tree_entry_bound(B.n, B.g.c, n_wit, n_bool, share);
        };
        bound(C->hl, cs->n_aux, aux_bool);
        bound(C->hl_eval, cs->n_aux, aux_bool);
        bound(C->a, (uint32_t)a_var.size(), count(a_var.data(), a_var.size()));
        bound(C->b1, (uint32_t)b_var.size(), count(b_var.data(), b_var.size()));
        bound(C->b2, (uint32_t)b_var.size(), count(b_var.data(), b_var.size()));
    }
    ctx->circ[slot] = std::move(C);
    return MASP_HIP_OK;
}

int masp_hip_circuit_flags(const masp_hip_ctx* ctx, uint32_t slot, uint32_t* flags) {
    if (!ctx || !flags) return MASP_HIP_E_INVALID_ARG;
    if (!ctx->children.empty()) return masp_hip_circuit_flags(ctx->children[0], slot, flags);
    std::shared_lock<std::shared_mutex> lock(const_cast<masp_hip_ctx*>(ctx)->mu);
    if (slot >= MASP_HIP_MAX_CIRCUITS || !ctx->circ[slot]) return MASP_HIP_E_NOT_LOADED;
    *flags = ctx->circ[slot]->g1_endo ? MASP_HIP_CIRCUIT_G1_ENDOMORPHISM : 0u;
    return MASP_HIP_OK;
}

int masp_hip_circuit_quotient_form(const masp_hip_ctx* ctx, uint32_t slot, int32_t* form) {
    if (!ctx || !form) return MASP_HIP_E_INVALID_ARG;
    if (!ctx->children.empty()) return masp_hip_circuit_quotient_form(ctx->children[0], slot, form);
    std::shared_lock<std::shared_mutex> lock(const_cast<masp_hip_ctx*>(ctx)->mu);
    if (slot >= MASP_HIP_MAX_CIRCUITS || !ctx->circ[slot]) return MASP_HIP_E_NOT_LOADED;
    *form = ctx->circ[slot]->hl_eval.n ? MASP_HIP_QUOTIENT_EVALUATION : MASP_HIP_QUOTIENT_COEFFICIENT;
    return MASP_HIP_OK;
}
int masp_hip_circuit_eval_bases(const masp_hip_ctx* ctx, uint32_t slot, uint8_t* bases, size_t cap_points, size_t* n_points, uint32_t* input_cols,
                                size_t cap_inputs, size_t* n_input_cols) {
    if (!ctx || !n_points || !n_input_cols) return MASP_HIP_E_INVALID_ARG;
    if (!ctx->children.empty()) return masp_hip_circuit_eval_bases(ctx->children[0], slot, bases, cap_points, n_points, input_cols, cap_inputs, n_input_cols);
    std::shared_lock<std::shared_mutex> lock(const_cast<masp_hip_ctx*>(ctx)->mu);
    if (slot >= MASP_HIP_MAX_CIRCUITS || !ctx->circ[slot]) return MASP_HIP_E_NOT_LOADED;
    const Circuit& C = *ctx->circ[slot];
    *n_points = C.hl_eval.n;
    *n_input_cols = C.eval_inputs.size();
    if (!bases && !input_cols) return MASP_HIP_OK;
    if (!bases || !input_cols || cap_points < *n_points || cap_inputs < *n_input_cols) return MASP_HIP_E_CAPACITY;
    if (C.hl_eval.n) {
        std::vector<masp::TabRow<masp::FpOps>> rows(C.hl_eval.n);
        hipSetDevice(ctx->device);
        if (hipMemcpy(rows.data(), C.hl_eval.tab, sizeof(rows[0]) * rows.size(), hipMemcpyDeviceToHost) != hipSuccess) return MASP_HIP_E_HIP;
        for (size_t i = 0; i < rows.size(); ++i) masp::g1_write_uncompressed(rows[i].p, bases + 96 * i);
    }
    memcpy(input_cols, C.eval_inputs.data(), 4 * C.eval_inputs.size());
    return MASP_HIP_OK;
}

static int validate_jobs(const masp_hip_ctx* dev_ctx, size_t n, const masp_hip_job* jobs) {
    for (size_t j = 0; j < n; ++j) {
        const masp_hip_job& J = jobs[j];
        if (J.circuit >= MASP_HIP_MAX_CIRCUITS || !J.inputs || !J.aux) return MASP_HIP_E_INVALID_ARG;
        if (!dev_ctx->circ[J.circuit]) return MASP_HIP_E_NOT_LOADED;
        if ((J.a || J.b || J.c) && !(J.a && J.b && J.c)) return MASP_HIP_E_INVALID_ARG;
        if (J.reserved != 0) return MASP_HIP_E_INVALID_ARG;
        if (J.aux_form > MASP_HIP_AUX_MONTGOMERY || (J.aux_form && J.a)) return MASP_HIP_E_INVALID_ARG;
        if (!rs_in_range(J.r) || !rs_in_range(J.s)) return MASP_HIP_E_SCALAR_RANGE;
    }
    return MASP_HIP_OK;
}

static int prove_batch_multi(masp_hip_ctx* ctx, size_t n, const masp_hip_job* jobs, uint8_t* proofs_out) {
    const size_t nd = ctx->children.size();
    auto alive = [&](size_t d) { return ctx->dev_status[d].load() == MASP_HIP_OK; };
    size_t n_alive = 0, first_alive = nd;
    for (size_t d = 0; d < nd; ++d)
        if (alive(d)) {
            ++n_alive;
            if (first_alive == nd) first_alive = d;
        }
    if (!n_alive) return MASP_HIP_E_HIP;
    {
        std::shared_lock<std::shared_mutex> lock(ctx->children[first_alive]->mu);
        if (int rc = validate_jobs(ctx->children[first_alive], n, jobs)) return rc;
    }
    struct Block {
        std::vector<size_t> idx;
        uint64_t cost;
    };
    std::deque<Block> queue;
    {
        std::map<std::pair<uint32_t, bool>, std::vector<size_t>> by_kind;
        for (size_t j = 0; j < n; ++j) by_kind[{jobs[j].circuit | (jobs[j].aux_form ? 0x100u : 0u), jobs[j].a != nullptr}].push_back(j);
        std::vector<Block> blocks;
        for (auto& kv : by_kind) {
            const size_t cap = std::min(ctx->batch_cap, std::max<size_t>((kv.second.size() + n_alive - 1) / n_alive, 8));
            const Circuit& C = *ctx->children[first_alive]->circ[kv.first.first & 0xffu];
            for (auto& g : even_groups(kv.second.size(), cap)) {
                Block b;
                b.idx.assign(kv.second.begin() + g.first, kv.second.begin() + g.first + g.second);
                b.cost = (uint64_t)C.nrows * g.second;
                blocks.push_back(std::move(b));
            }
        }
        std::stable_sort(blocks.begin(), blocks.end(), [](const Block& x, const Block& y) { return x.cost > y.cost; });
        for (auto& b : blocks) queue.push_back(std::move(b));
    }
    std::mutex mu;
    std::condition_variable cv;
    size_t pending = queue.size();
    int fatal = MASP_HIP_OK;
    auto worker = [&](size_t d) {
        masp_hip_ctx* ch = ctx->children[d];
        std::vector<masp_hip_job> mine;
        std::vector<uint8_t> out;
        for (;;) {
            Block b;
            {
// ... 202 lines not shown
            if (!ok) {
                last_hip_error() = "D2H copy failed";
                result = fail(ctx, MASP_HIP_E_HIP);
            }
        }
        if (!ok) {
            for (int i = 0; i < Slot::N_AUX; ++i) hipStreamSynchronize(sl.aux[i]);
            hipStreamSynchronize(sl.stream);
            slot_release(ctx, si);
            break;
        }
        owned.push_back({si, gi});
#ifdef MASP_ENQ_TIMING
        fprintf(stderr, "[grp] call %p t=%8.2f ms group %zu circuit %u np %zu slot %zu: waited %.2f ms for the slot, staged + enqueued in %.2f ms\n", (void*)jobs,
                ms_since(tcall), gi, jobs[G.idx[0]].circuit, np, si, t_wait, ms_since(tg1));
#endif
    }
    while (!owned.empty()) slot_release(ctx, retire_oldest());
#ifdef MASP_ENQ_TIMING
    fprintf(stderr, "[call] %p done after %.2f ms (%zu jobs)\n", (void*)jobs, ms_since(tcall), n);
#endif
    if (result == MASP_HIP_OK) ctx->proofs_done += n;
    const int launch_rc = launch_status();
    if (launch_rc && result == MASP_HIP_OK) result = fail(ctx, launch_rc);
    if (hipGetLastError() != hipSuccess && result == MASP_HIP_OK) {
        last_hip_error() = "kernel launch failed";
        result = fail(ctx, MASP_HIP_E_HIP);
    }
    return result;
}

int masp_hip_prove(masp_hip_ctx* ctx, uint32_t slot, const uint8_t* inputs, const uint8_t* aux, const uint8_t* a, const uint8_t* b,
                   const uint8_t* c, const uint8_t r[32], const uint8_t s[32], uint8_t proof_out[192]) {
    if (!r || !s || !proof_out) return MASP_HIP_E_INVALID_ARG;
    masp_hip_job J;
    J.circuit = slot;
    J.inputs = inputs;
    J.aux = aux;
    J.a = a;
    J.b = b;
    J.c = c;
    J.aux_form = MASP_HIP_AUX_CANONICAL;
    J.reserved = 0;
    memcpy(J.r, r, 32);
    memcpy(J.s, s, 32);
    uint8_t tmp[192];
    int rc = masp_hip_prove_batch(ctx, 1, &J, tmp);
    if (rc == MASP_HIP_OK) memcpy(proof_out, tmp, 192);
    return rc;
}

}

template <class O, int BYTES>
static int msm_multi(masp_hip_ctx* ctx, const uint8_t* bases, size_t n, const uint8_t* scalars, size_t np, int window_bits, uint8_t* out,
                     int block_bits = 0, size_t sub_lo = 0, size_t sub_hi = (size_t)-1, uint32_t* bucket0_entries = nullptr) {
    if (!ctx || !out || !np || np > 256 || !n || !bases || !scalars || n > (1u << 22) || window_bits < 0 || window_bits == 1 || window_bits > 16)
        return MASP_HIP_E_INVALID_ARG;
    if (block_bits != 0 && block_bits != 2 && block_bits != 3) return MASP_HIP_E_INVALID_ARG;
    if (!ctx->children.empty()) ctx = ctx->children[0];
    sub_lo = std::min(sub_lo, n);
    sub_hi = std::min(sub_hi, n);
    std::unique_lock<std::shared_mutex> lock(ctx->mu);
    hipSetDevice(ctx->device);
    hipStream_t s = ctx->streams.main;
    for (size_t i = 0; i < n * np; ++i)
        if (!rs_in_range(scalars + 32 * i)) return MASP_HIP_E_SCALAR_RANGE;
    MsmBases<O, BYTES> B;
    MsmWorkspace<O> ws;
    ws.tree_levels = ctx->opt.bucket_tree_levels;
    ws.tree_sub = (uint32_t)ctx->opt.bucket_tree_sub_batch;
    ws.tree.own.limit = (size_t)ctx->opt.bucket_tree_scratch_mb << 20;
    struct Report {
        masp_hip_ctx* c;
        MsmWorkspace<O>& w;
        ~Report() {
            c->block_tree_fallbacks += w.tree_fallbacks;
            c->block_tree_sub = std::min<uint32_t>(c->block_tree_sub, std::min(w.tree_sub ? w.tree_sub : 256u, w.tree_sub_used));
        }
    } report{ctx, ws};
    DevBuf<Xyzz<O>> res;
    DevBuf<uint8_t> d_out;
    int rc;
    if ((rc = B.load_host(bases, (uint32_t)n, s, 0xffffffffu, window_bits, block_bits, (uint32_t)sub_lo, (uint32_t)sub_hi))) return fail(ctx, rc);
    if (B.import_status & (PT_BAD_FLAGS | PT_NOT_CANONICAL)) return MASP_HIP_E_PARAMS_FORMAT;
    if ((rc = ctx->tmp_scalars.upload((const Fr*)scalars, n * np, s)) || (rc = res.reserve(np)) || (rc = d_out.reserve(BYTES * np))) return fail(ctx, rc);
    if ((rc = msm_enqueue(s, B, ws, (const uint32_t*)ctx->tmp_scalars.p, n * 8, res.p, 1, (uint32_t)np))) return fail(ctx, rc);
    if (bucket0_entries) {
        if (hipMemcpy2DAsync(bucket0_entries, sizeof(uint32_t), ws.sort.dense + 1, sizeof(uint32_t) * ((size_t)B.g.nb + 1), sizeof(uint32_t), np,
                             hipMemcpyDeviceToHost, s) != hipSuccess)
            return fail(ctx, MASP_HIP_E_HIP);
    }
    for (size_t p = 0; p < np; ++p) {
        if constexpr (BYTES == 96)
            launch_g1_export(s, res.p + p, d_out.p + BYTES * p);
        else
            launch_g2_export(s, res.p + p, d_out.p + BYTES * p);
    }
    std::vector<uint8_t> tmp(BYTES * np);
    if (hipMemcpyAsync(tmp.data(), d_out.p, tmp.size(), hipMemcpyDeviceToHost, s) != hipSuccess || hipStreamSynchronize(s) != hipSuccess) {
        last_hip_error() = std::string("msm failed: ") + hipGetErrorString(hipGetLastError());
        return fail(ctx, MASP_HIP_E_HIP);
    }
    memcpy(out, tmp.data(), tmp.size());
    return MASP_HIP_OK;
}
template <class O, int BYTES, class X>
static int msm_block(masp_hip_ctx* ctx, const uint8_t* bases, const uint8_t* scalars, size_t n, uint8_t* out, DevBuf<X>& res) {
    if (!ctx || !out || (n && (!bases || !scalars)) || n > (1u << 26)) return MASP_HIP_E_INVALID_ARG;
    std::unique_lock<std::shared_mutex> lock(ctx->mu);
    hipSetDevice(ctx->device);
    hipStream_t s = ctx->streams.main;
    for (size_t i = 0; i < n; ++i)
        if (!rs_in_range(scalars + 32 * i)) return MASP_HIP_E_SCALAR_RANGE;
    MsmBases<O, BYTES> B;
    MsmWorkspace<O> ws;
    int rc;
    if ((rc = B.load_host(bases, (uint32_t)n, s))) return fail(ctx, rc);
    if (B.import_status & (PT_BAD_FLAGS | PT_NOT_CANONICAL)) return MASP_HIP_E_PARAMS_FORMAT;
    if ((rc = ctx->tmp_scalars.upload((const Fr*)scalars, n, s)) || (rc = res.reserve(1)) || (rc = ctx->tmp_out.reserve(BYTES))) return fail(ctx, rc);
    if ((rc = msm_enqueue(s, B, ws, (const uint32_t*)ctx->tmp_scalars.p, 0, res.p, 1, 1))) return fail(ctx, rc);
    if constexpr (BYTES == 96)
        launch_g1_export(s, res.p, ctx->tmp_out.p);
    else
        launch_g2_export(s, res.p, ctx->tmp_out.p);
    uint8_t tmp[BYTES];
    if (hipMemcpyAsync(tmp, ctx->tmp_out.p, BYTES, hipMemcpyDeviceToHost, s) != hipSuccess || hipStreamSynchronize(s) != hipSuccess) {
        last_hip_error() = std::string("msm failed: ") + hipGetErrorString(hipGetLastError());
        return fail(ctx, MASP_HIP_E_HIP);
    }
    memcpy(out, tmp, BYTES);
    return MASP_HIP_OK;
}
extern "C" {


int masp_hip_msm_g1(masp_hip_ctx* ctx, const uint8_t* bases, const uint8_t* scalars, size_t n, uint8_t out[96]) {
    const ApiLaunchScope api_scope;
    if (!ctx) return MASP_HIP_E_INVALID_ARG;
    ctx = FIRST_DEVICE(ctx);
    return msm_block<FpOps, 96>(ctx, bases, scalars, n, out, ctx->tmp_g1);
}
int masp_hip_msm_g2(masp_hip_ctx* ctx, const uint8_t* bases, const uint8_t* scalars, size_t n, uint8_t out[192]) {
    const ApiLaunchScope api_scope;
    if (!ctx) return MASP_HIP_E_INVALID_ARG;
    ctx = FIRST_DEVICE(ctx);
    return msm_block<Fp2Ops, 192>(ctx, bases, scalars, n, out, ctx->tmp_g2);
}

int masp_hip_msm_g1_multi(masp_hip_ctx* ctx, const uint8_t* bases, size_t n, const uint8_t* scalars, size_t np, int window_bits, uint8_t* out) {
    const ApiLaunchScope api_scope;
    return msm_multi<FpOps, 96>(ctx, bases, n, scalars, np, window_bits, out);
}
int masp_hip_msm_g2_multi(masp_hip_ctx* ctx, const uint8_t* bases, size_t n, const uint8_t* scalars, size_t np, int window_bits, uint8_t* out) {
    const ApiLaunchScope api_scope;
    return msm_multi<Fp2Ops, 192>(ctx, bases, n, scalars, np, window_bits, out);
}

int masp_hip_msm_g1_multi_ex(masp_hip_ctx* ctx, const uint8_t* bases, size_t n, const uint8_t* scalars, size_t np, int window_bits, int block_bits,
                             size_t sub_lo, size_t sub_hi, uint8_t* out, uint32_t* bucket0_entries) {
    const ApiLaunchScope api_scope;
    return msm_multi<FpOps, 96>(ctx, bases, n, scalars, np, window_bits, out, block_bits, sub_lo, sub_hi, bucket0_entries);
}
int masp_hip_msm_g2_multi_ex(masp_hip_ctx* ctx, const uint8_t* bases, size_t n, const uint8_t* scalars, size_t np, int window_bits, int block_bits,
                             size_t sub_lo, size_t sub_hi, uint8_t* out, uint32_t* bucket0_entries) {
    const ApiLaunchScope api_scope;
    return msm_multi<Fp2Ops, 192>(ctx, bases, n, scalars, np, window_bits, out, block_bits, sub_lo, sub_hi, bucket0_entries);
// ... 331 lines not shown
```

### masp_amd/hip.py

```python
import ctypes as C
import os

import numpy as np

_HERE = os.path.dirname(os.path.abspath(__file__))
_lib = None

ERRORS = {1: "invalid argument", 2: "Parameters bytes are malformed", 3: "Parameters do not match the circuit shape",
          4: "no usable HIP device (there is no CPU fallback)", 5: "HIP runtime error", 6: "UnexpectedIdentity",
          7: "circuit slot is empty", 8: "scalar is not a canonical field element", 9: "a Jubjub point encoding does not decode",
          10: "an output buffer is too small"}
E_POINT_ENCODING = 9
E_CAPACITY = 10
SPEND_AUTH, BINDING = 0, 1

SPEND, OUTPUT, CONVERT = 0, 1, 2


class MaspHipError(RuntimeError):
    def __init__(self, code, detail=""):
        self.code = code
        super().__init__("masp_hip error %d: %s%s" % (code, ERRORS.get(code, "?"), (" — " + detail) if detail else ""))


# ... 4 lines not shown

class OptionsStruct(C.Structure):
    _fields_ = ([("struct_size", C.c_uint32)] + [(f, C.c_int32) for f in OPTION_FIELDS[:OPTION_FIELDS.index("lone_proof_graph")]] +
                [("bucket_tree_fallback_proofs", C.c_int32), ("lone_proof_graph", C.c_int32), ("hw_queues", C.c_int32), ("window_bits_h_lone", C.c_int32),
                 ("digit_recoding", C.c_int32),
                 ("window_bits_b2", C.c_int32)])


assert C.sizeof(OptionsStruct) == 76 and OptionsStruct.window_bits_b2.offset == 72


class JobStruct(C.Structure):
    _fields_ = [("circuit", C.c_uint32), ("inputs", C.c_void_p), ("aux", C.c_void_p), ("a", C.c_void_p),
                ("b", C.c_void_p), ("c", C.c_void_p), ("r", C.c_uint8 * 32), ("s", C.c_uint8 * 32), ("aux_form", C.c_uint32),
                ("reserved", C.c_uint32)]


assert C.sizeof(JobStruct) == 120 and JobStruct.r.offset == 48 and JobStruct.aux_form.offset == 112
AUX_CANONICAL, AUX_MONTGOMERY = 0, 1
QUOTIENT_EVALUATION, QUOTIENT_COEFFICIENT = 0, 1
QUOTIENT_FUSED, QUOTIENT_SEPARATE = 0, 1


def library_path():
    return os.environ.get("MASP_HIP_LIBRARY") or os.path.join(_HERE, "libmasp_hip.so")


def load_library():
    global _lib
    if _lib is not None:
        return _lib
    path = library_path()
    if not os.path.exists(path):
        raise ImportError("libmasp_hip.so is not built: run `python -c 'import __graft_entry__ as g; g.build()'` "
                          "or `make -C masp_amd/csrc` (hipcc, --offload-arch=gfx950)")
    os.environ.setdefault("GPU_MAX_HW_QUEUES", "16")
    L = C.CDLL(path)
    if hasattr(L, "masp_hip_runtime_prepare"):
        L.masp_hip_runtime_prepare.argtypes = [C.c_int, C.c_int]
        q = L.masp_hip_runtime_prepare(0, 0)
        if q > 20:
            import warnings
            warnings.warn("masp_amd: GPU_MAX_HW_QUEUES=%d: once this process holds more than 20 hardware queues every kernel dispatch gets "
                          "slower (24: -7 %%, 32: -21 %% proofs/s; profiles/r06_second_context_root_cause.txt) — use 16" % q)
    vp, sz, u32 = C.c_void_p, C.c_size_t, C.c_uint32
    L.masp_hip_ctx_create.argtypes = [C.c_int, C.POINTER(vp)]
    L.masp_hip_ctx_create_multi.argtypes = [C.POINTER(C.c_int), C.c_int, C.POINTER(vp)]
    L.masp_hip_ctx_create_ex.argtypes = [C.POINTER(C.c_int), C.c_int, C.POINTER(OptionsStruct), C.POINTER(vp)]
    L.masp_hip_ctx_get_options.argtypes = [vp, C.POINTER(OptionsStruct)]
    L.masp_hip_device_count.argtypes = []
    L.masp_hip_options_default.argtypes = [C.POINTER(OptionsStruct)]
    L.masp_hip_options_default.restype = None
    L.masp_hip_ctx_device_count.argtypes = [vp]
    L.masp_hip_ctx_device_proofs.argtypes = [vp, C.POINTER(C.c_uint64), C.c_int]
    if hasattr(L, "masp_hip_ctx_stream_concurrency"):
        L.masp_hip_ctx_stream_concurrency.argtypes = [vp, C.c_int, C.POINTER(C.c_int), C.POINTER(C.c_int)]
    if hasattr(L, "masp_hip_ctx_device_status"):
        L.masp_hip_ctx_device_status.argtypes = [vp, C.POINTER(C.c_int32), C.c_int, C.POINTER(C.c_uint64)]
        L.masp_hip_ctx_inject_fault.argtypes = [vp, C.c_int, C.c_uint32]
    if hasattr(L, "masp_hip_ctx_lone_graph_launches"):
        L.masp_hip_ctx_lone_graph_launches.argtypes = [vp, C.POINTER(C.c_uint64)]
    if hasattr(L, "masp_hip_circuit_flags"):
        L.masp_hip_circuit_flags.argtypes = [vp, u32, C.POINTER(C.c_uint32)]
    L.masp_hip_ctx_destroy.argtypes = [vp]
    L.masp_hip_ctx_destroy.restype = None
    L.masp_hip_strerror.restype = C.c_char_p
    L.masp_hip_last_error.argtypes = [vp]
    L.masp_hip_last_error.restype = C.c_char_p
    L.masp_hip_circuit_load.argtypes = [vp, u32, vp, sz, vp]
    L.masp_hip_prove.argtypes = [vp, u32, vp, vp, vp, vp, vp, C.c_char_p, C.c_char_p, vp]
    L.masp_hip_prove_batch.argtypes = [vp, sz, vp, vp]
    L.masp_hip_generate_parameters.argtypes = [vp, vp, C.c_char_p, vp, sz, C.POINTER(sz)]
    L.masp_hip_parameters_max_size.argtypes = [vp]
    L.masp_hip_parameters_max_size.restype = sz
    L.masp_hip_msm_g1.argtypes = [vp, vp, vp, sz, vp]
    L.masp_hip_msm_g2.argtypes = [vp, vp, vp, sz, vp]
    L.masp_hip_msm_g1_multi.argtypes = [vp, vp, sz, vp, sz, C.c_int, vp]
    L.masp_hip_msm_g2_multi.argtypes = [vp, vp, sz, vp, sz, C.c_int, vp]
    if hasattr(L, "masp_hip_msm_g1_multi_ex"):
        L.masp_hip_msm_g1_multi_ex.argtypes = [vp, vp, sz, vp, sz, C.c_int, C.c_int, sz, sz, vp, vp]
        L.masp_hip_msm_g2_multi_ex.argtypes = [vp, vp, sz, vp, sz, C.c_int, C.c_int, sz, sz, vp, vp]
        L.masp_hip_ctx_set_boolean_block_bits.argtypes = [vp, C.c_int32]
        L.masp_hip_ctx_get_boolean_block_bits.argtypes = [vp, C.POINTER(C.c_int32)]
    if hasattr(L, "masp_hip_ctx_set_quotient_form"):
        L.masp_hip_ctx_set_quotient_form.argtypes = [vp, C.c_int32]
        L.masp_hip_ctx_get_quotient_form.argtypes = [vp, C.POINTER(C.c_int32)]
        L.masp_hip_circuit_quotient_form.argtypes = [vp, u32, C.POINTER(C.c_int32)]
        L.masp_hip_circuit_eval_bases.argtypes = [vp, u32, vp, sz, C.POINTER(sz), vp, sz, C.POINTER(sz)]
    if hasattr(L, "masp_hip_ctx_set_quotient_schedule"):
        L.masp_hip_ctx_set_quotient_schedule.argtypes = [vp, C.c_int32]
        L.masp_hip_ctx_get_quotient_schedule.argtypes = [vp, C.POINTER(C.c_int32)]
    if hasattr(L, "masp_hip_ctx_set_tree_entry_share"):
        L.masp_hip_ctx_set_tree_entry_share.argtypes = [vp, C.c_int32]
        L.masp_hip_ctx_get_tree_entry_share.argtypes = [vp, C.POINTER(C.c_int32)]
        L.masp_hip_r1cs_boolean_variables.argtypes = [vp, vp]
        L.masp_hip_tree_entry_bound.argtypes = [u32, C.c_int32, u32, u32, C.c_int32]
        L.masp_hip_tree_entry_bound.restype = C.c_uint64
        L.masp_hip_circuit_tree_entry_bounds.argtypes = [vp, u32, C.POINTER(C.c_uint64), C.POINTER(C.c_int32)]
    L.masp_hip_quotient_h.argtypes = [vp, vp, vp, vp, sz, u32, vp]
    L.masp_hip_ntt.argtypes = [vp, vp, u32, C.c_int]
    L.masp_hip_vk_prepare.argtypes = [vp, vp, sz, C.POINTER(vp)]
    L.masp_hip_vk_free.argtypes = [vp]
    L.masp_hip_vk_free.restype = None
    L.masp_hip_verify_batch.argtypes = [vp, vp, sz, vp, vp, u32, vp, C.POINTER(C.c_int)]
    if hasattr(L, "masp_hip_verify_each"):
        L.masp_hip_verify_each.argtypes = [vp, vp, sz, vp, vp, u32, C.c_char_p]
        L.masp_hip_verify_each_last_timing.argtypes = [vp, C.POINTER(C.c_double)]
        L.masp_hip_redjubjub_verify_each.argtypes = [vp, sz, C.c_char_p, C.c_char_p, C.c_char_p, C.c_char_p, C.c_char_p]
    if hasattr(L, "masp_hip_redjubjub_verify_batch"):
        L.masp_hip_jubjub_msm.argtypes = [vp, sz, vp, vp, vp, C.POINTER(C.c_int64)]
        L.masp_hip_redjubjub_verify_batch.argtypes = [vp, sz, C.c_char_p, C.c_char_p, C.c_char_p, C.c_char_p, C.c_char_p, C.POINTER(C.c_int)]
    if hasattr(L, "masp_hip_sapling_trial_decrypt"):
        L.masp_hip_sapling_trial_decrypt.argtypes = [vp, sz, vp, sz, vp, vp, vp, sz, vp, vp, vp, C.POINTER(sz)]
        L.masp_hip_note_scan_configure.argtypes = [vp, C.c_int, C.c_int]
        L.masp_hip_note_scan_last_timing.argtypes = [vp, C.POINTER(C.c_double)]
    if hasattr(L, "masp_hip_sapling_compact_trial_decrypt"):
        L.masp_hip_sapling_compact_trial_decrypt.argtypes = [vp, sz, vp, sz, vp, vp, vp, C.c_int, vp, sz, vp, vp, vp, vp, C.POINTER(sz), C.POINTER(sz)]
        L.masp_hip_note_scan_compact_last_timing.argtypes = [vp, C.POINTER(C.c_double)]
    if hasattr(L, "masp_hip_sapling_output_recovery_scan"):
        L.masp_hip_sapling_output_recovery_scan.argtypes = [vp, sz, vp, sz, vp, vp, vp, vp, sz, vp, vp, vp, C.POINTER(sz)]
        L.masp_hip_out_recovery_last_timing.argtypes = [vp, C.POINTER(C.c_double)]
    if hasattr(L, "masp_hip_merkle_tree_complete"):
        L.masp_hip_merkle_tree_complete.argtypes = [vp, C.c_uint, sz, vp, vp, sz, C.POINTER(sz), vp, sz, vp, vp, C.POINTER(C.c_int64)]
        L.masp_hip_merkle_last_timing.argtypes = [vp, C.POINTER(C.c_double)]
    if hasattr(L, "masp_hip_merkle_tree_append"):
        L.masp_hip_merkle_tree_append.argtypes = [vp, C.c_uint64, vp, sz, vp, vp, sz, C.POINTER(sz), C.POINTER(C.c_int64)]
    L.masp_hip_batch_upload.argtypes = [vp, sz, vp]
    L.masp_hip_batch_prove_resident.argtypes = [vp, C.c_int, vp, C.POINTER(C.c_float)]
    L.masp_hip_batch_prove_resident_steps.argtypes = [vp, C.c_int, sz, vp, vp, C.POINTER(C.c_float)]
    L.masp_hip_batch_free.argtypes = [vp, C.c_int]
    L.masp_hip_bench_msm.argtypes = [vp, C.c_int, sz, C.c_int, C.c_int, C.POINTER(C.c_float), C.POINTER(u32)]
    L.masp_hip_profile_enable.argtypes = [vp, C.c_int]
    L.masp_hip_profile_read.argtypes = [vp, C.POINTER(C.c_double), C.POINTER(C.c_uint64), C.POINTER(C.c_uint64)]
    L.masp_hip_profile_read_split.argtypes = [vp, C.POINTER(C.c_double)]
    if hasattr(L, "masp_hip_profile_read_lone"):
        L.masp_hip_profile_read_lone.argtypes = [vp, C.POINTER(C.c_double)]
    L.masp_hip_sync.argtypes = [vp]
    L.masp_hip_host_alloc.argtypes = [vp, sz]
    L.masp_hip_host_alloc.restype = vp
    L.masp_hip_host_free.argtypes = [vp, vp]
    L.masp_hip_host_free.restype = None
    _lib = L
    return L


def device_pci_bus_id(device=0):
    L = load_library()
    if not hasattr(L, "masp_hip_device_pci_bus_id"):
        return None
    buf = C.create_string_buffer(64)
    L.masp_hip_device_pci_bus_id.argtypes = [C.c_int, C.c_char_p, C.c_size_t]
    return buf.value.decode().lower() if L.masp_hip_device_pci_bus_id(int(device), buf, 64) == 0 else None


def device_count():
    return int(load_library().masp_hip_device_count())


def _p(a):
    return a.ctypes.data_as(C.c_void_p) if a is not None else None


def _u8(a, shape_last=None):
    if a is None:
        return None
    if isinstance(a, (bytes, bytearray, memoryview)):
        a = np.frombuffer(a, dtype=np.uint8)
    a = np.ascontiguousarray(a, dtype=np.uint8)
    if shape_last is not None:
        a = a.reshape(-1, shape_last)
# ... 260 lines not shown
            e.bad_index, e.needed = bad.value, nn.value
            raise e
        return (nodes[:nn.value] if want_nodes else None), root.tobytes(), paths

    def merkle_tree_append(self, start, frontier, row, nodes_capacity=None):
        from .host import merkle_append_args, merkle_append_error, merkle_append_node_count
        row, frontier = merkle_append_args(start, frontier, row)
        n = row.shape[0]
        if nodes_capacity is None:
            nodes_capacity = merkle_append_node_count(int(start), n)
        nodes = np.zeros((max(1, int(nodes_capacity)), 32), np.uint8)
        nn, bad = C.c_size_t(0), C.c_int64(-1)
        rc = self._L.masp_hip_merkle_tree_append(self._h, int(start), _p(frontier), n, _p(row) if n else None, _p(nodes), int(nodes_capacity),
                                                 C.byref(nn), C.byref(bad))
        if rc:
            detail = merkle_append_error("merkle_tree_append", bad.value) if bad.value != -1 else \
                "%d nodes" % nn.value if rc == E_CAPACITY else self._L.masp_hip_last_error(self._h).decode(errors="replace")
            e = MaspHipError(rc, detail)
            e.bad_index, e.needed = bad.value, nn.value
            raise e
        return nodes[:nn.value]

    def merkle_last_timing(self):
        ms = (C.c_double * 3)()
        self._check(self._L.masp_hip_merkle_last_timing(self._h, ms))
        return ms[0], ms[1], ms[2]

    def msm_g1(self, bases, scalars):
        bases, scalars = _u8(bases, 96), _u8(scalars, 32)
        out = np.zeros(96, dtype=np.uint8)
        self._check(self._L.masp_hip_msm_g1(self._h, _p(bases), _p(scalars), scalars.shape[0], _p(out)))
        return out.tobytes()

    def msm_g2(self, bases, scalars):
        bases, scalars = _u8(bases, 192), _u8(scalars, 32)
        out = np.zeros(192, dtype=np.uint8)
        self._check(self._L.masp_hip_msm_g2(self._h, _p(bases), _p(scalars), scalars.shape[0], _p(out)))
        return out.tobytes()

    def msm_g1_multi(self, bases, scalars, window_bits=0):
        bases = _u8(bases, 96)
        scalars = np.ascontiguousarray(scalars, dtype=np.uint8)
        npf, n = scalars.shape[0], scalars.shape[1]
        assert scalars.shape == (npf, n, 32) and bases.shape[0] == n
        out = np.zeros((npf, 96), dtype=np.uint8)
        self._check(self._L.masp_hip_msm_g1_multi(self._h, _p(bases), n, _p(scalars), npf, int(window_bits), _p(out)))
        return [out[i].tobytes() for i in range(npf)]

    def msm_g2_multi(self, bases, scalars, window_bits=0):
        bases = _u8(bases, 192)
        scalars = np.ascontiguousarray(scalars, dtype=np.uint8)
        npf, n = scalars.shape[0], scalars.shape[1]
        assert scalars.shape == (npf, n, 32) and bases.shape[0] == n
        out = np.zeros((npf, 192), dtype=np.uint8)
        self._check(self._L.masp_hip_msm_g2_multi(self._h, _p(bases), n, _p(scalars), npf, int(window_bits), _p(out)))
        return [out[i].tobytes() for i in range(npf)]

    def _msm_multi_ex(self, fn, size, bases, scalars, window_bits, block_bits, sub_lo, sub_hi):
        bases = _u8(bases, size)
        scalars = np.ascontiguousarray(scalars, dtype=np.uint8)
        npf, n = scalars.shape[0], scalars.shape[1]
        assert scalars.shape == (npf, n, 32) and bases.shape[0] == n
        out = np.zeros((npf, size), dtype=np.uint8)
        cnt = np.zeros(npf, dtype=np.uint32)
        self._check(fn(self._h, _p(bases), n, _p(scalars), npf, int(window_bits), int(block_bits), int(sub_lo), int(n if sub_hi is None else sub_hi),
                       _p(out), _p(cnt)))
        return [out[i].tobytes() for i in range(npf)], [int(c) for c in cnt]

    def msm_g1_multi_ex(self, bases, scalars, window_bits=0, block_bits=0, sub_lo=0, sub_hi=None):
        return self._msm_multi_ex(self._L.masp_hip_msm_g1_multi_ex, 96, bases, scalars, window_bits, block_bits, sub_lo, sub_hi)

    def msm_g2_multi_ex(self, bases, scalars, window_bits=0, block_bits=0, sub_lo=0, sub_hi=None):
        return self._msm_multi_ex(self._L.masp_hip_msm_g2_multi_ex, 192, bases, scalars, window_bits, block_bits, sub_lo, sub_hi)

    def set_boolean_block_bits(self, bits):
        self._check(self._L.masp_hip_ctx_set_boolean_block_bits(self._h, int(bits)))

    @property
    def boolean_block_bits(self):
        v = C.c_int32(0)
        self._check(self._L.masp_hip_ctx_get_boolean_block_bits(self._h, C.byref(v)))
        return int(v.value)

    def set_quotient_form(self, form):
        self._check(self._L.masp_hip_ctx_set_quotient_form(self._h, int(form)))

    @property
    def quotient_form(self):
        v = C.c_int32(0)
        self._check(self._L.masp_hip_ctx_get_quotient_form(self._h, C.byref(v)))
        return int(v.value)

    def set_quotient_schedule(self, schedule):
        self._check(self._L.masp_hip_ctx_set_quotient_schedule(self._h, int(schedule)))

    @property
    def quotient_schedule(self):
        v = C.c_int32(0)
        self._check(self._L.masp_hip_ctx_get_quotient_schedule(self._h, C.byref(v)))
        return int(v.value)

    def circuit_quotient_form(self, slot):
        v = C.c_int32(0)
        self._check(self._L.masp_hip_circuit_quotient_form(self._h, int(slot), C.byref(v)))
        return int(v.value)

    def circuit_eval_bases(self, slot):
        n, k = C.c_size_t(0), C.c_size_t(0)
        self._check(self._L.masp_hip_circuit_eval_bases(self._h, int(slot), None, 0, C.byref(n), None, 0, C.byref(k)))
        pts = np.zeros((n.value, 96), dtype=np.uint8)
        cols = np.zeros(max(k.value, 1), dtype=np.uint32)
        if n.value:
            self._check(self._L.masp_hip_circuit_eval_bases(self._h, int(slot), _p(pts), n.value, C.byref(n), _p(cols), cols.size, C.byref(k)))
        return pts, [int(c) for c in cols[:k.value]]

    def set_tree_entry_share(self, percent):
        self._check(self._L.masp_hip_ctx_set_tree_entry_share(self._h, int(percent)))

    @property
    def tree_entry_share(self):
        v = C.c_int32(0)
        self._check(self._L.masp_hip_ctx_get_tree_entry_share(self._h, C.byref(v)))
        return int(v.value)

    def circuit_tree_entry_bounds(self, slot):
        b, c = (C.c_uint64 * 4)(), (C.c_int32 * 4)()
        self._check(self._L.masp_hip_circuit_tree_entry_bounds(self._h, int(slot), b, c))
        return {k: (int(b[i]), int(c[i])) for i, k in enumerate(("hl", "a", "b_g1", "b_g2"))}

    def current_options(self):
        got = OptionsStruct()
        got.struct_size = C.sizeof(OptionsStruct)
        self._check(self._L.masp_hip_ctx_get_options(self._h, C.byref(got)))
        d = {f: int(getattr(got, f)) for f in OPTION_FIELDS}
        d["bucket_tree_fallback_proofs"] = int(got.bucket_tree_fallback_proofs)
        d["hw_queues"] = int(got.hw_queues)
        return d

    @property
    def device_count(self):
        return self._L.masp_hip_ctx_device_count(self._h)

    def circuit_uses_endomorphism(self, slot):
        f = C.c_uint32(0)
        self._check(self._L.masp_hip_circuit_flags(self._h, int(slot), C.byref(f)))
        return bool(f.value & 1)

    def lone_graph_launches(self):
        v = C.c_uint64(0)
        self._check(self._L.masp_hip_ctx_lone_graph_launches(self._h, C.byref(v)))
        return int(v.value)

    def device_proofs(self):
        n = self.device_count
        counts = (C.c_uint64 * n)()
        self._check(self._L.masp_hip_ctx_device_proofs(self._h, counts, n))
        return list(counts)

    def stream_concurrency(self, mains_only=False):
        n, c = C.c_int(0), C.c_int(0)
        self._check(self._L.masp_hip_ctx_stream_concurrency(self._h, 1 if mains_only else 0, C.byref(n), C.byref(c)))
        return int(n.value), int(c.value)

    def device_status(self):
        n = self.device_count
        st, rq = (C.c_int32 * n)(), C.c_uint64(0)
        self._check(self._L.masp_hip_ctx_device_status(self._h, st, n, C.byref(rq)))
        return list(st), int(rq.value)

    def inject_fault(self, device, nth):
        self._check(self._L.masp_hip_ctx_inject_fault(self._h, int(device), int(nth)))

    def quotient_h(self, a, b, c, logm):
        a, b, c = _u8(a, 32), _u8(b, 32), _u8(c, 32)
        out = np.zeros(((1 << logm) - 1, 32), dtype=np.uint8)
        self._check(self._L.masp_hip_quotient_h(self._h, _p(a), _p(b), _p(c), a.shape[0], logm, _p(out)))
        return out

    def ntt(self, data, logm, inverse=False):
        d = _u8(data, 32).copy()
        self._check(self._L.masp_hip_ntt(self._h, _p(d), logm, 1 if inverse else 0))
        return d

    def batch_upload(self, jobs):
        jobs = list(jobs)
        arr = (JobStruct * len(jobs))()
        keep = []
# ... 129 lines not shown
```

Before: 1499 proofs/s.

## Add twin-row MSM tables folding digit powers of two into fewer buckets

Adds a twin-table Pippenger layout: each base gets extra precomputed rows for 2x its window multiples, and signed digits are mapped by their power-of-two factor into a reduced bucket set (about 2/3 of the usual). The bucket reduction and window-sum kernels gain a twin path plus a combine kernel that weights each bucket class by powers of four. The aim is less bucket-accumulation and reduction work in the H/L, A and B MSMs, at the cost of doubled table memory, extra precompute at load time, more scattered table reads, and a larger window for mid-size sets. It is enabled by default for all bases through a compile-time default.

```diff
diff --git a/include/masp_hip.h b/include/masp_hip.h
--- a/include/masp_hip.h
+++ b/include/masp_hip.h
@@ -81,6 +81,8 @@
 int masp_hip_ctx_create_multi(const int* devices, int n_devices, masp_hip_ctx** out);
 int masp_hip_ctx_set_boolean_block_bits(masp_hip_ctx* ctx, int32_t bits);
 int masp_hip_ctx_get_boolean_block_bits(const masp_hip_ctx* ctx, int32_t* out);
+int masp_hip_ctx_set_window_row_multiples(masp_hip_ctx* ctx, int32_t v);
+int masp_hip_ctx_get_window_row_multiples(const masp_hip_ctx* ctx, int32_t* out);
 #define MASP_HIP_QUOTIENT_EVALUATION 0
 #define MASP_HIP_QUOTIENT_COEFFICIENT 1
 int masp_hip_ctx_set_quotient_form(masp_hip_ctx* ctx, int32_t form);
@@ -109,6 +111,7 @@
 int masp_hip_circuit_flags(const masp_hip_ctx* ctx, uint32_t slot, uint32_t* flags);
 
 int masp_hip_circuit_quotient_form(const masp_hip_ctx* ctx, uint32_t slot, int32_t* form);
+int masp_hip_circuit_window_row_multiples(const masp_hip_ctx* ctx, uint32_t slot, int32_t* sets);
 int masp_hip_circuit_eval_bases(const masp_hip_ctx* ctx, uint32_t slot, uint8_t* bases, size_t cap_points, size_t* n_points, uint32_t* input_cols,
                                 size_t cap_inputs, size_t* n_input_cols);
 
diff --git a/masp_amd/csrc/device/msm.hpp b/masp_amd/csrc/device/msm.hpp
--- a/masp_amd/csrc/device/msm.hpp
+++ b/masp_amd/csrc/device/msm.hpp
@@ -31,16 +31,18 @@
     tab[i].p = p;
 }
 template <class O>
-__global__ void __launch_bounds__(64) k_msm_precompute(TabRow<O>* __restrict__ tab, uint32_t n, int c, int W) {
+__global__ void __launch_bounds__(64) k_msm_precompute(TabRow<O>* __restrict__ tab, uint32_t n, int c, int W, int twin = 0) {
     uint32_t i = blockIdx.x * blockDim.x + threadIdx.x;
     if (i >= n) return;
     Affine<O> p = tab[i].p;
     for (int j = 1; j < W; ++j) {
         Xyzz<O> q = xyzz_dbl_affine(p);
+        if (twin) tab[(size_t)(W + j - 1) * n + i].p = xyzz_to_affine(q);
         for (int k = 1; k < c; ++k) q = xyzz_dbl(q);
         p = xyzz_to_affine(q);
         tab[(size_t)j * n + i].p = p;
     }
+    if (twin) tab[(size_t)(2 * W - 1) * n + i].p = xyzz_to_affine(xyzz_dbl_affine(p));
 }
 template <class O>
 __global__ void __launch_bounds__(64) k_msm_subset_rows(TabRow<O>* __restrict__ tab, MsmSubset sub, uint32_t n_rows) {
@@ -242,7 +244,7 @@
 constexpr uint32_t wsum_points_log() {
     return O::LANES > 4 ? WSUM_L_LOG - 1 : WSUM_L_LOG;
 }
-template <class O, uint32_t G_LOG>
+template <class O, uint32_t G_LOG, bool TWIN = false>
 __global__ void __launch_bounds__((1u << wsum_points_log<O>()) * O::LANES, (O::LANES > 1 ? MASP_WSUM_PAIR_WAVES : sizeof(Xyzz<O>) > 200 || G_LOG < 3 ? MASP_TAIL_MIN_WAVES : 2))
 k_msm_wsum_level(const Xyzz<typename O::Base>* __restrict__ B, size_t b_stride, uint32_t m, uint32_t off, Xyzz<typename O::Base>* __restrict__ S,
                  Xyzz<typename O::Base>* __restrict__ T, size_t st_stride) {
@@ -255,9 +257,22 @@
     T += MSM_P * st_stride;
     const uint32_t base = blockIdx.x * CS + e * G;
     Xyzz<O> run = xyzz_inf<O>(), acc = xyzz_inf<O>();
-    for (uint32_t l = G; l-- > 0;) {
-        if (base + l < m) xyzz_add_nc(run, xyzz_load<O>(B + base + l, h));
-        if (l > 0 || off) xyzz_add_nc(acc, run);
+    if constexpr (TWIN) {
+        const bool tail = blockIdx.x == gridDim.x - 1;
+        for (uint32_t l = G; l-- > 0;) {
+            if (!tail) {
+                xyzz_add_nc(run, xyzz_load<O>(B + base + l, h));
+            } else {
+                const uint32_t v = e * G + l + 1u, t = (uint32_t)__builtin_ctz(v);
+                if (v <= m && !(t & 1u)) xyzz_add_nc(run, xyzz_load<O>(B + blockIdx.x * CS + 2u * (m - (m >> t)) / 3u + ((v >> t) >> 1), h));
+            }
+            if (l > 0 || tail) xyzz_add_nc(acc, run);
+        }
+    } else {
+        for (uint32_t l = G; l-- > 0;) {
+            if (base + l < m) xyzz_add_nc(run, xyzz_load<O>(B + base + l, h));
+            if (l > 0 || off) xyzz_add_nc(acc, run);
+        }
     }
     Xyzz<O> x = run;
     for (uint32_t d = 1; d < WE; d <<= 1) {
@@ -330,6 +345,33 @@
     for (int l = levels - 1; l >= 0; --l) {
         for (int k = 0; k < cs_log; ++k) acc = xyzz_dbl(acc);
         xyzz_add_nc(acc, tsum[l]);
+    }
+    *out = acc;
+}
+
+template <class O>
+__global__ void __launch_bounds__(64) k_msm_twin_combine(const Xyzz<O>* __restrict__ S, const Xyzz<O>* __restrict__ T, size_t st_stride, int c, uint32_t s0,
+                                                         int cs_log, Xyzz<O>* __restrict__ out, size_t out_stride) {
+    if (blockIdx.x != 0 || threadIdx.x != 0) return;
+    S += MSM_P * st_stride;
+    T += MSM_P * st_stride;
+    out += MSM_P * out_stride;
+    Xyzz<O> acc = T[s0 ? msm_twin_class(c, s0).off >> cs_log : 0u];
+    for (uint32_t s = s0; s-- > 0;) {
+        const MsmTwinClass k = msm_twin_class(c, s);
+        const uint32_t ch0 = k.off >> cs_log, nch = k.size >> cs_log;
+        Xyzz<O> run = xyzz_inf<O>(), jsum = xyzz_inf<O>(), tsum = xyzz_inf<O>();
+        for (uint32_t j = nch; j-- > 0;) {
+            xyzz_add_nc(run, S[ch0 + j]);
+            xyzz_add_nc(tsum, T[ch0 + j]);
+            if (j > 0) xyzz_add_nc(jsum, run);
+        }
+        for (int i = 0; i < cs_log; ++i) jsum = xyzz_dbl(jsum);
+        xyzz_add_nc(jsum, tsum);
+        jsum = xyzz_dbl(jsum);
+        xyzz_add_nc(jsum, run);
+        acc = xyzz_dbl(xyzz_dbl(acc));
+        xyzz_add_nc(acc, jsum);
     }
     *out = acc;
 }
diff --git a/masp_amd/csrc/device/msm_geom.h b/masp_amd/csrc/device/msm_geom.h
--- a/masp_amd/csrc/device/msm_geom.h
+++ b/masp_amd/csrc/device/msm_geom.h
@@ -9,12 +9,45 @@
     int c;
     int W;
     int nb;
+    int twin;
+    __host__ __device__ int tables() const { return twin ? 2 * W : W; }
 };
 static inline MsmGeom msm_geom(int c) {
     MsmGeom g;
     g.c = c;
     g.W = (256 + c - 1) / c;
     g.nb = 1 << (c - 1);
+    g.twin = 0;
+    return g;
+}
+struct MsmTwinClass {
+    uint32_t off, size, weight;
+};
+__host__ __device__ static inline uint32_t msm_twin_classes(int c) { return (uint32_t)(c - 1) / 2u + 1u; }
+__host__ __device__ static inline MsmTwinClass msm_twin_class(int c, uint32_t s) {
+    const uint32_t H = 1u << (c - 1), sz = H >> (2u * s + 1u);
+    MsmTwinClass k;
+    k.off = 2u * (H - (H >> (2u * s))) / 3u;
+    k.size = sz ? sz : 1u;
+    k.weight = 1u << (2u * s);
+    return k;
+}
+__host__ __device__ static inline uint32_t msm_twin_buckets(int c) { return ((2u << (c - 1)) + 1u) / 3u; }
+__host__ __device__ static inline uint32_t msm_twin_bucket(int c, uint32_t v, uint32_t& mult) {
+#if defined(__HIP_DEVICE_COMPILE__)
+    const uint32_t t = (uint32_t)__builtin_ctz(v);
+#else
+    uint32_t t = 0;
+    while (!((v >> t) & 1u)) ++t;
+#endif
+    mult = t & 1u;
+    return msm_twin_class(c, t >> 1).off + ((v >> t) >> 1);
+}
+static inline MsmGeom msm_geom_twin(int c) {
+    MsmGeom g = msm_geom(c);
+    const uint32_t nbk = msm_twin_buckets(c);
+    g.nb = (int)(nbk < 128u ? nbk : (nbk + 127u) & ~127u);
+    g.twin = 1;
     return g;
 }
 static inline uint32_t msm_mean_digits_x16(const MsmGeom& g) { return (uint32_t)g.W * 16; }
diff --git a/masp_amd/csrc/device/msm_sort.hpp b/masp_amd/csrc/device/msm_sort.hpp
--- a/masp_amd/csrc/device/msm_sort.hpp
+++ b/masp_amd/csrc/device/msm_sort.hpp
@@ -11,10 +11,10 @@
 
 struct MsmDigitIter {
     const uint32_t* sw;
-    uint32_t carry, mask, half, pos, j;
+    uint32_t carry, mask, half, pos, j, twin_w;
     int c;
     __device__ __forceinline__ MsmDigitIter(const uint32_t* sw_, const MsmGeom& g)
-        : sw(sw_), carry(0), mask((1u << g.c) - 1u), half(1u << (g.c - 1)), pos(0), j(0), c(g.c) {}
+        : sw(sw_), carry(0), mask((1u << g.c) - 1u), half(1u << (g.c - 1)), pos(0), j(0), twin_w(g.twin ? (uint32_t)g.W : 0u), c(g.c) {}
     __device__ __forceinline__ uint32_t bits(uint32_t bit) const {
         const uint32_t w = bit >> 5, off = bit & 31u;
         const uint64_t two = ((uint64_t)(w + 1 < 8 ? sw[w + 1] : 0u) << 32) | sw[w];
@@ -32,6 +32,11 @@
             carry = 1;
         }
         bucket = v - 1;
+        if (twin_w && v != 0) {
+            uint32_t mult;
+            bucket = msm_twin_bucket(c, v, mult);
+            if (mult) table += twin_w;
+        }
         return v != 0;
     }
 };
diff --git a/masp_amd/csrc/internal.h b/masp_amd/csrc/internal.h
--- a/masp_amd/csrc/internal.h
+++ b/masp_amd/csrc/internal.h
@@ -27,6 +27,10 @@
 #define MASP_SUBSET_BITS 2
 #endif
 static_assert(MASP_SUBSET_BITS == 0 || MASP_SUBSET_BITS == 2 || MASP_SUBSET_BITS == 3, "subset blocks are 4 or 8 bases wide");
+#ifndef MASP_TWIN_ROWS
+#define MASP_TWIN_ROWS 3
+#endif
+static_assert(MASP_TWIN_ROWS >= 0 && MASP_TWIN_ROWS <= 3, "bit 0: h + l, bit 1: a, b_g1, b_g2");
 #ifndef MASP_TREE_ENTRY_SHARE
 #define MASP_TREE_ENTRY_SHARE 100
 #endif
@@ -136,6 +140,7 @@
     std::vector<uint32_t> eval_inputs;
     BasesG2 b2;
     BasesG2 b2_lone;
+    BasesG1 a_lone, b1_lone;
     bool g1_endo = false;
     NttDomain* dom = nullptr;
 };
@@ -300,6 +305,8 @@
     std::vector<masp_hip_ctx*> children;
     masp_hip_options opt{};
     int boolean_block_bits = MASP_SUBSET_BITS;
+    int twin_rows = MASP_TWIN_ROWS;
+    bool twin_rows_msm = false;
     int quotient_form = 0;
     std::atomic<int> quotient_schedule{0};
     int tree_entry_share = MASP_TREE_ENTRY_SHARE;
diff --git a/masp_amd/csrc/k_msm_g1_lone.hip b/masp_amd/csrc/k_msm_g1_lone.hip
--- a/masp_amd/csrc/k_msm_g1_lone.hip
+++ b/masp_amd/csrc/k_msm_g1_lone.hip
@@ -2,5 +2,5 @@
 #include "msm_impl.hpp"
 
 namespace masp {
-template void msm_tails_enqueue<FpOps, FpQuadOps>(hipStream_t, MsmWorkspace<FpOps>&, const uint32_t*, uint32_t, uint32_t, uint32_t, bool, Xyzz<FpOps>*, size_t);
+template void msm_tails_enqueue<FpOps, FpQuadOps>(hipStream_t, MsmWorkspace<FpOps>&, const uint32_t*, uint32_t, uint32_t, uint32_t, bool, Xyzz<FpOps>*, size_t, int);
 }
diff --git a/masp_amd/csrc/k_msm_g2_lone.hip b/masp_amd/csrc/k_msm_g2_lone.hip
--- a/masp_amd/csrc/k_msm_g2_lone.hip
+++ b/masp_amd/csrc/k_msm_g2_lone.hip
@@ -2,5 +2,5 @@
 #include "msm_impl.hpp"
 
 namespace masp {
-template void msm_tails_enqueue<Fp2Ops, Fp2OctOps>(hipStream_t, MsmWorkspace<Fp2Ops>&, const uint32_t*, uint32_t, uint32_t, uint32_t, bool, Xyzz<Fp2Ops>*, size_t);
+template void msm_tails_enqueue<Fp2Ops, Fp2OctOps>(hipStream_t, MsmWorkspace<Fp2Ops>&, const uint32_t*, uint32_t, uint32_t, uint32_t, bool, Xyzz<Fp2Ops>*, size_t, int);
 }
diff --git a/masp_amd/csrc/k_msm_sort.hip b/masp_amd/csrc/k_msm_sort.hip
--- a/masp_amd/csrc/k_msm_sort.hip
+++ b/masp_amd/csrc/k_msm_sort.hip
@@ -12,12 +12,12 @@
         last_hip_error() = "MSM window width must be 2..16 bits: the bucket histogram lives in LDS";
         return MASP_HIP_E_INVALID_ARG;
     }
-    const uint64_t rows = (uint64_t)n * (uint32_t)g.W + sub.rows();
+    const uint64_t rows = (uint64_t)n * (uint32_t)g.tables() + sub.rows();
     if (rows > 0x7ffffffeull) {
         last_hip_error() = "msm_sort_enqueue: the base set has more table rows than an entry's 31 bits can name";
         return MASP_HIP_E_INVALID_ARG;
     }
-    if (sub.bits && ((sub.bits != 2 && sub.bits != 3) || sub.b_end < sub.b_first || ((uint64_t)sub.b_end << sub.bits) > n || sub.row0 != n * (uint32_t)g.W ||
+    if (sub.bits && ((sub.bits != 2 && sub.bits != 3) || sub.b_end < sub.b_first || ((uint64_t)sub.b_end << sub.bits) > n || sub.row0 != n * (uint32_t)g.tables() ||
                      !sub.bad)) {
         last_hip_error() = "msm_sort_enqueue: subset rows that do not belong to this base set";
         return MASP_HIP_E_INVALID_ARG;
diff --git a/masp_amd/csrc/msm_host.h b/masp_amd/csrc/msm_host.h
--- a/masp_amd/csrc/msm_host.h
+++ b/masp_amd/csrc/msm_host.h
@@ -33,7 +33,7 @@
     MsmSubset sub;
     uint32_t sub_lo = 0, sub_hi = 0;
     const MsmSubset& subset() const { return sub; }
-    uint64_t rows() const { return (uint64_t)n * (uint32_t)g.W + sub.rows(); }
+    uint64_t rows() const { return (uint64_t)n * (uint32_t)g.tables() + sub.rows(); }
 
     ~MsmBases() { release(); }
     void release() {
@@ -42,20 +42,20 @@
         tab = nullptr;
         sub = MsmSubset();
     }
-    static MsmGeom pick_geom(uint32_t n_eff) {
-        int c = n_eff >= (1u << 16) ? 16 : n_eff >= (1u << 12) ? 12 : n_eff >= (1u << 8) ? 10 : 7;
+    static MsmGeom pick_geom(uint32_t n_eff, bool twin = false) {
+        int c = n_eff >= (1u << 16) ? 16 : n_eff >= (1u << 12) ? (twin ? 13 : 12) : n_eff >= (1u << 8) ? 10 : 7;
         return msm_geom(c);
     }
     int load_device(const uint8_t* d_raw, uint32_t n_, hipStream_t s, uint32_t n_eff = 0xffffffffu, int force_c = 0, int sub_bits_ = 0,
-                    uint32_t sub_lo_ = 0, uint32_t sub_hi_ = 0xffffffffu);
+                    uint32_t sub_lo_ = 0, uint32_t sub_hi_ = 0xffffffffu, bool twin_ = false);
     int load_host(const uint8_t* raw, uint32_t n_, hipStream_t s, uint32_t n_eff = 0xffffffffu, int force_c = 0, int sub_bits_ = 0, uint32_t sub_lo_ = 0,
-                  uint32_t sub_hi_ = 0xffffffffu) {
+                  uint32_t sub_hi_ = 0xffffffffu, bool twin_ = false) {
         uint8_t* d_raw = nullptr;
         if (n_) {
             HIP_TRY(dev_malloc(&d_raw, (size_t)n_ * BYTES));
             HIP_TRY(hipMemcpyAsync(d_raw, raw, (size_t)n_ * BYTES, hipMemcpyHostToDevice, s));
         }
-        int rc = load_device(d_raw, n_, s, n_eff, force_c, sub_bits_, sub_lo_, sub_hi_);
+        int rc = load_device(d_raw, n_, s, n_eff, force_c, sub_bits_, sub_lo_, sub_hi_, twin_);
         if (d_raw) dev_free(d_raw);
         return rc;
     }
@@ -99,7 +99,7 @@
         const size_t need_ent = std::max(padded_entries(n_, g_, pad_log_), cap_ent), ng = ranges_for(n_, np_);
         const size_t bins = std::max<size_t>(g_.nb >> 7, 1);
         const size_t hist_need = (size_t)np_ * ng * g_.nb, crel_need = (size_t)np_ * ng * bins;
-        const bool want_tmpf = has_tmpf || msm_rows_wide(std::max<uint64_t>(rows_, (uint64_t)n_ * (uint32_t)g_.W));
+        const bool want_tmpf = has_tmpf || msm_rows_wide(std::max<uint64_t>(rows_, (uint64_t)n_ * (uint32_t)g_.tables()));
         if (need_ent <= cap_ent && (size_t)g_.nb <= cap_nb && np_ <= cap_np && hist_need <= cap_hist && crel_need <= cap_crel && want_tmpf == has_tmpf)
             return MASP_HIP_OK;
         const size_t need_nb = std::max<size_t>(g_.nb, cap_nb), need_np = std::max<size_t>(np_, cap_np);
@@ -399,7 +399,7 @@
 
 template <class A, class B>
 inline bool msm_same_sort(const A& a, const B& b) {
-    return a.n == b.n && a.g.c == b.g.c;
+    return a.n == b.n && a.g.c == b.g.c && a.g.twin == b.g.twin;
 }
 
 typedef MsmBases<FpOps, 96> BasesG1;
diff --git a/masp_amd/csrc/msm_impl.hpp b/masp_amd/csrc/msm_impl.hpp
--- a/masp_amd/csrc/msm_impl.hpp
+++ b/masp_amd/csrc/msm_impl.hpp
@@ -24,11 +24,11 @@
 
 template <class O, int BYTES>
 int MsmBases<O, BYTES>::load_device(const uint8_t* d_raw, uint32_t n_, hipStream_t s, uint32_t n_eff, int force_c, int sub_bits_, uint32_t sub_lo_,
-                                    uint32_t sub_hi_) {
+                                    uint32_t sub_hi_, bool twin_) {
         release();
         n = n_;
         this->n_eff = std::min(n_eff, n_);
-        g = force_c ? msm_geom(force_c) : pick_geom(std::min(n_eff, n_));
+        g = force_c ? msm_geom(force_c) : pick_geom(std::min(n_eff, n_), twin_);
         if (n == 0) return MASP_HIP_OK;
         if (sub_bits_ != 0 && sub_bits_ != 2 && sub_bits_ != 3) {
             last_hip_error() = "MsmBases: subset blocks are 4 or 8 bases wide";
@@ -36,14 +36,20 @@
         }
         sub_lo = std::min(sub_lo_, n);
         sub_hi = std::min(sub_hi_, n);
-        if (sub_bits_) {
-            MsmSubset u;
-            u.bits = (uint32_t)sub_bits_;
-            u.b_first = (uint32_t)(((uint64_t)sub_lo + (1u << sub_bits_) - 1) >> sub_bits_);
-            u.b_end = sub_hi >> sub_bits_;
-            u.row0 = n * (uint32_t)g.W;
-            if (u.b_end > u.b_first) sub = u;
-        }
+        auto layout = [&](bool twin) {
+            if (twin) g = msm_geom_twin(g.c);
+            else g = msm_geom(g.c);
+            sub = MsmSubset();
+            if (sub_bits_) {
+                MsmSubset u;
+                u.bits = (uint32_t)sub_bits_;
+                u.b_first = (uint32_t)(((uint64_t)sub_lo + (1u << sub_bits_) - 1) >> sub_bits_);
+                u.b_end = sub_hi >> sub_bits_;
+                u.row0 = n * (uint32_t)g.tables();
+                if (u.b_end > u.b_first) sub = u;
+            }
+        };
+        layout(twin_);
         if (rows() > 0x7ffffffeull) {
             sub = MsmSubset();
             last_hip_error() = "MsmBases: more table rows than an entry's 31 bits can name";
@@ -55,7 +61,20 @@
         HIP_TRY(hipMemsetAsync(d_status, 0, sizeof(int), s));
         dim3 grid((n + 63) / 64), block(64);
         MASP_LAUNCH((k_msm_import<O, BYTES>), grid, block, 0, s, d_raw, tab, n, d_status);
-        MASP_LAUNCH((k_msm_precompute<O>), grid, block, 0, s, tab, n, g.c, g.W);
+        if (twin_) {
+            HIP_TRY(hipMemcpyAsync(&import_status, d_status, sizeof(int), hipMemcpyDeviceToHost, s));
+            HIP_TRY(hipStreamSynchronize(s));
+            if (import_status & PT_INFINITY) {
+                layout(false);
+                TabRow<O>* plain = nullptr;
+                HIP_TRY(dev_malloc(&plain, sizeof(TabRow<O>) * (size_t)rows()));
+                HIP_TRY(hipMemcpyAsync(plain, tab, sizeof(TabRow<O>) * (size_t)n, hipMemcpyDeviceToDevice, s));
+                HIP_TRY(hipStreamSynchronize(s));
+                dev_free(tab);
+                tab = plain;
+            }
+        }
+        MASP_LAUNCH((k_msm_precompute<O>), grid, block, 0, s, tab, n, g.c, g.W, g.twin);
         if (sub.bits) {
             HIP_TRY(dev_malloc(&sub.bad, sizeof(uint32_t) * sub.bad_words()));
             HIP_TRY(hipMemsetAsync(sub.bad, 0, sizeof(uint32_t) * sub.bad_words(), s));
@@ -113,7 +132,7 @@
 #endif
 template <class O, class OT>
 void msm_tails_enqueue(hipStream_t s, MsmWorkspace<O>& ws, const uint32_t* start, uint32_t nb, uint32_t nchunks, uint32_t np, bool lone, Xyzz<O>* d_out,
-                       size_t out_stride) {
+                       size_t out_stride, int twin_c = 0) {
     constexpr uint32_t LN = OT::LANES;
     if constexpr (OT::LANES <= 2) {
         if (!lone) {
@@ -144,6 +163,29 @@
                            ws.n_heavy, (Xyzz<O>*)nullptr);
     }
     uint32_t g_log = nb <= WSUM_L ? 0 : WSUM_G_LOG_MIN;
+    if (twin_c) {
+        if constexpr (!OT::REPLICATED) {
+            g_log = 3;
+            while (g_log < 6u && (1u << (g_log + 1 + WSUM_L_LOG)) <= nb) ++g_log;
+            const uint32_t cs_log = g_log + WSUM_L_LOG, cs = 1u << cs_log;
+            uint32_t s0 = 0;
+            while (s0 < msm_twin_classes(twin_c) && msm_twin_class(twin_c, s0).size >= cs) ++s0;
+            const uint32_t big = s0 < msm_twin_classes(twin_c) ? msm_twin_class(twin_c, s0).off >> cs_log : msm_twin_buckets(twin_c) >> cs_log;
+            const uint32_t span = s0 < msm_twin_classes(twin_c) ? (1u << (twin_c - 1)) >> (2u * s0) : 0u;
+            const size_t st_stride = big + 1;
+            const dim3 grid(big + 1, np), block((1u << wsum_points_log<OT>()) * LN);
+            switch (g_log) {
+#define MASP_WSUM_CASE(GL) \
+    case GL: MASP_LAUNCH((k_msm_wsum_level<OT, GL, true>), grid, block, 0, s, ws.bkt, (size_t)nb, span, 0u, ws.S[0], ws.T, st_stride); break;
+                MASP_WSUM_CASE(3) MASP_WSUM_CASE(4) MASP_WSUM_CASE(5) MASP_WSUM_CASE(6)
+#undef MASP_WSUM_CASE
+            }
+            MASP_LAUNCH((k_msm_twin_combine<O>), dim3(1, np), dim3(64), 0, s, ws.S[0], ws.T, st_stride, twin_c, s0, (int)cs_log, d_out, out_stride);
+        } else {
+            last_hip_error() = "msm_tails_enqueue: doubled window rows have no replicated-lane form";
+        }
+        return;
+    }
     if (!lone) {
         const uint32_t hi = 6u;
         g_log = 3;
@@ -186,10 +228,10 @@
         MASP_LAUNCH((k_msm_combine<O>), dim3(1, np), dim3(64), 0, s, ws.tsum, level, (int)(g_log + WSUM_L_LOG), d_out, out_stride);
 }
 #ifndef MASP_TAILS_QUAD_UNIT
-extern template void msm_tails_enqueue<FpOps, FpQuadOps>(hipStream_t, MsmWorkspace<FpOps>&, const uint32_t*, uint32_t, uint32_t, uint32_t, bool, Xyzz<FpOps>*, size_t);
+extern template void msm_tails_enqueue<FpOps, FpQuadOps>(hipStream_t, MsmWorkspace<FpOps>&, const uint32_t*, uint32_t, uint32_t, uint32_t, bool, Xyzz<FpOps>*, size_t, int);
 #endif
 #ifndef MASP_TAILS_OCT_UNIT
-extern template void msm_tails_enqueue<Fp2Ops, Fp2OctOps>(hipStream_t, MsmWorkspace<Fp2Ops>&, const uint32_t*, uint32_t, uint32_t, uint32_t, bool, Xyzz<Fp2Ops>*, size_t);
+extern template void msm_tails_enqueue<Fp2Ops, Fp2OctOps>(hipStream_t, MsmWorkspace<Fp2Ops>&, const uint32_t*, uint32_t, uint32_t, uint32_t, bool, Xyzz<Fp2Ops>*, size_t, int);
 #endif
 
 template <class O, int BYTES>
@@ -197,7 +239,7 @@
                        MsmProfile* prof) {
     const MsmGeom& g = B.g;
     const uint32_t n = B.n, np = sb.np;
-    if (sb.n != n || sb.g.c != g.c) {
+    if (sb.n != n || sb.g.c != g.c || sb.g.twin != g.twin) {
         last_hip_error() = "msm_reduce_enqueue: sort does not match the base set";
         return MASP_HIP_E_INVALID_ARG;
     }
@@ -282,16 +324,17 @@
         hipEventRecord(rec.e1, s);
         prof->recs.push_back(rec);
     }
+    const int twin_c = g.twin ? g.c : 0;
     if constexpr (std::is_same<O, FpOps>::value) {
-        if (lone)
+        if (lone && !twin_c)
             msm_tails_enqueue<O, FpQuadOps>(s, ws, start, nb, nchunks, np, lone, d_out, out_stride);
         else
-            msm_tails_enqueue<O, FpOps>(s, ws, start, nb, nchunks, np, lone, d_out, out_stride);
+            msm_tails_enqueue<O, FpOps>(s, ws, start, nb, nchunks, np, lone, d_out, out_stride, twin_c);
     } else {
-        if (lone && (MASP_G2_OCT_LONE))
+        if (lone && !twin_c && (MASP_G2_OCT_LONE))
             msm_tails_enqueue<O, Fp2OctOps>(s, ws, start, nb, nchunks, np, lone, d_out, out_stride);
         else
-            msm_tails_enqueue<O, typename TailLaneOps<O>::type>(s, ws, start, nb, nchunks, np, lone, d_out, out_stride);
+            msm_tails_enqueue<O, typename TailLaneOps<O>::type>(s, ws, start, nb, nchunks, np, lone, d_out, out_stride, twin_c);
     }
     return launch_status();
 }
diff --git a/masp_amd/csrc/prover.hip b/masp_amd/csrc/prover.hip
--- a/masp_amd/csrc/prover.hip
+++ b/masp_amd/csrc/prover.hip
@@ -312,10 +312,12 @@
         launch_groth16_fixed_g2(sl.aux[0], C.fb2.p, d_rs, 16, sl.asm2.p, np);
         HIP_TRY(hipEventRecord(sl.ev_fixed, sl.aux[0]));
         const bool own_b2 = C.b2_lone.n != 0;
+        const BasesG1 &Al = C.a_lone.n ? C.a_lone : C.a, &B1l = C.b1_lone.n ? C.b1_lone : C.b1;
+        const bool share_bl = C.nbq && msm_same_sort(B1l, C.b2);
         auto chain_a = [&]() -> int {
             int r;
             if (C.na) launch_gather_scalars(sl.aux[1], d_w, w_stride, C.a_var.p, C.na, sl.sa.p, np);
-            if ((r = msm_enqueue(sl.aux[1], C.a, sl.ws_a, (const uint32_t*)sl.sa.p, (size_t)C.na * 8, sl.res1.p + 2, 4, np))) return r;
+            if ((r = msm_enqueue(sl.aux[1], Al, sl.ws_a, (const uint32_t*)sl.sa.p, (size_t)C.na * 8, sl.res1.p + 2, 4, np))) return r;
             sl.lone_mark(sl.aux[1], 1);
             launch_groth16_var_mul(sl.aux[1], 0, sl.res1.p, d_rs, 16, sl.asm1.p, np, C.g1_endo);
             sl.lone_mark(sl.aux[1], 2);
@@ -325,11 +327,11 @@
             int r;
             if (C.nbq) launch_gather_scalars(sl.aux[2], d_w, w_stride, C.b_var.p, C.nbq, sl.sb.p, np);
             HIP_TRY(hipEventRecord(sl.ev_sort_b, sl.aux[2]));
-            if (share_b) {
-                if ((r = msm_sort_enqueue(sl.aux[2], C.b1.n, C.b1.g, sl.ws_b.sort, (const uint32_t*)sl.sb.p, (size_t)C.nbq * 8, np, 0, C.b1.subset()))) return r;
+            if (share_bl) {
+                if ((r = msm_sort_enqueue(sl.aux[2], B1l.n, B1l.g, sl.ws_b.sort, (const uint32_t*)sl.sb.p, (size_t)C.nbq * 8, np, 0, B1l.subset()))) return r;
                 if (!own_b2) HIP_TRY(hipEventRecord(sl.ev_sort_b, sl.aux[2]));
-                if ((r = msm_reduce_enqueue(sl.aux[2], C.b1, sl.ws_b.sort, sl.ws_b, sl.res1.p + 3, 4))) return r;
-            } else if ((r = msm_enqueue(sl.aux[2], C.b1, sl.ws_b, (const uint32_t*)sl.sb.p, (size_t)C.nbq * 8, sl.res1.p + 3, 4, np))) {
+                if ((r = msm_reduce_enqueue(sl.aux[2], B1l, sl.ws_b.sort, sl.ws_b, sl.res1.p + 3, 4))) return r;
+            } else if ((r = msm_enqueue(sl.aux[2], B1l, sl.ws_b, (const uint32_t*)sl.sb.p, (size_t)C.nbq * 8, sl.res1.p + 3, 4, np))) {
                 return r;
             }
             sl.lone_mark(sl.aux[2], 3);
@@ -338,7 +340,7 @@
             HIP_TRY(hipStreamWaitEvent(sl.aux[3], sl.ev_sort_b, 0));
             if (own_b2) {
                 if ((r = msm_enqueue(sl.aux[3], C.b2_lone, sl.ws2, (const uint32_t*)sl.sb.p, (size_t)C.nbq * 8, sl.res2.p, 1, np))) return r;
-            } else if (share_b) {
+            } else if (share_bl) {
                 if ((r = msm_reduce_enqueue(sl.aux[3], C.b2, sl.ws_b.sort, sl.ws2, sl.res2.p, 1))) return r;
             } else if ((r = msm_enqueue(sl.aux[3], C.b2, sl.ws2, (const uint32_t*)sl.sb.p, (size_t)C.nbq * 8, sl.res2.p, 1, np))) {
                 return r;
@@ -781,6 +783,24 @@
     return MASP_HIP_OK;
 }
 
+int masp_hip_ctx_set_window_row_multiples(masp_hip_ctx* ctx, int32_t v) {
+    if (!ctx || v < -1 || v > 2) return MASP_HIP_E_INVALID_ARG;
+    const int resolved = v == 0 ? (int)(MASP_TWIN_ROWS) : v < 0 ? 0 : v == 1 ? 3 : 1;
+    auto set = [&](masp_hip_ctx* c) {
+        std::unique_lock<std::shared_mutex> lock(c->mu);
+        c->twin_rows = resolved;
+        c->twin_rows_msm = v == 1;
+    };
+    set(ctx);
+    for (masp_hip_ctx* c : ctx->children) set(c);
+    return MASP_HIP_OK;
+}
+int masp_hip_ctx_get_window_row_multiples(const masp_hip_ctx* ctx, int32_t* out) {
+    if (!ctx || !out) return MASP_HIP_E_INVALID_ARG;
+    *out = (ctx->children.empty() ? ctx : ctx->children[0])->twin_rows;
+    return MASP_HIP_OK;
+}
+
 int masp_hip_ctx_set_quotient_form(masp_hip_ctx* ctx, int32_t form) {
     if (!ctx || (form != MASP_HIP_QUOTIENT_EVALUATION && form != MASP_HIP_QUOTIENT_COEFFICIENT)) return MASP_HIP_E_INVALID_ARG;
     auto set = [&](masp_hip_ctx* c) {
@@ -1049,9 +1069,11 @@
     const int c_h = ctx->opt.window_bits_h ? ctx->opt.window_bits_h : n_h >= 49152 ? 16 : n_h >= 16384 ? 15 : 0;
     const int c_h_lone = ctx->opt.window_bits_h_lone ? ctx->opt.window_bits_h_lone : c_h;
     const int sub_bits = ctx->boolean_block_bits;
+    const bool twin_hl = ctx->twin_rows & 1, twin_ab = ctx->twin_rows & 2;
     if ((rc = C->h.load_host(L.h, (uint32_t)(C->m - 1), s, 0xffffffffu, c_h_lone)) || (rc = C->l.load_host(L.l, L.n_l, s, eff(L.n_l), c_la)) ||
-        (rc = C->a.load_host(L.a, L.n_a, s, eff(L.n_a), c_la, sub_bits)) || (rc = C->b1.load_host(L.b_g1, L.n_b1, s, eff(L.n_b1), c_b, sub_bits)) ||
-        (rc = C->b2.load_host(L.b_g2, L.n_b2, s, eff(L.n_b2), c_b2, sub_bits)))
+        (rc = C->a.load_host(L.a, L.n_a, s, eff(L.n_a), c_la, sub_bits, 0, 0xffffffffu, twin_ab)) ||
+        (rc = C->b1.load_host(L.b_g1, L.n_b1, s, eff(L.n_b1), c_b, sub_bits, 0, 0xffffffffu, twin_ab)) ||
+        (rc = C->b2.load_host(L.b_g2, L.n_b2, s, eff(L.n_b2), c_b2, sub_bits, 0, 0xffffffffu, twin_ab)))
         return fail(ctx, rc);
     if (C->b1.sub.bits && C->b2.sub.bits && msm_same_sort(C->b1, C->b2)) {
         const uint32_t words = C->b1.sub.bad_words();
@@ -1064,6 +1086,8 @@
             hipMemcpyAsync(C->b2.sub.bad, w1.data(), 4 * (size_t)words, hipMemcpyHostToDevice, s) != hipSuccess || hipStreamSynchronize(s) != hipSuccess)
             return fail(ctx, MASP_HIP_E_HIP);
     }
+    if (C->a.g.twin && (rc = C->a_lone.load_host(L.a, L.n_a, s, eff(L.n_a), c_la, sub_bits))) return fail(ctx, rc);
+    if (C->b1.g.twin && (rc = C->b1_lone.load_host(L.b_g1, L.n_b1, s, eff(L.n_b1), c_b, sub_bits))) return fail(ctx, rc);
     {
         const int c_lone = ctx->opt.window_bits_b2_lone;
         if (c_lone > 0 && L.n_b2 && (rc = C->b2_lone.load_host(L.b_g2, L.n_b2, s, eff(L.n_b2), c_lone))) return fail(ctx, rc);
@@ -1074,7 +1098,7 @@
         std::vector<uint8_t> cat(96 * (nh + L.n_l));
         memcpy(cat.data(), L.h, 96 * nh);
         memcpy(cat.data() + 96 * nh, L.l, 96 * (size_t)L.n_l);
-        if ((rc = C->hl.load_host(cat.data(), (uint32_t)(nh + L.n_l), s, 0xffffffffu, c_hl, sub_bits, (uint32_t)nh))) return fail(ctx, rc);
+        if ((rc = C->hl.load_host(cat.data(), (uint32_t)(nh + L.n_l), s, 0xffffffffu, c_hl, sub_bits, (uint32_t)nh, 0xffffffffu, twin_hl))) return fail(ctx, rc);
     }
     int st = C->h.import_status | C->l.import_status | C->a.import_status | C->b1.import_status | C->b2.import_status;
     if (st) return MASP_HIP_E_PARAMS_FORMAT;
@@ -1099,7 +1123,7 @@
         if ((rc = build_eval_bases(ctx, *C->dom, L.h, L.l, cs, E))) return fail(ctx, rc);
         if (E.usable) {
             const masp::EvalLayout& lay = E.lay;
-            if ((rc = C->hl_eval.load_device(E.d_raw.p, (uint32_t)lay.n(), s, 0xffffffffu, c_hl, sub_bits, (uint32_t)lay.aux_off(), (uint32_t)lay.in_off())))
+            if ((rc = C->hl_eval.load_device(E.d_raw.p, (uint32_t)lay.n(), s, 0xffffffffu, c_hl, sub_bits, (uint32_t)lay.aux_off(), (uint32_t)lay.in_off(), twin_hl)))
                 return fail(ctx, rc);
             if ((rc = C->eval_in_var.upload(lay.used_inputs.data(), lay.used_inputs.size(), s))) return fail(ctx, rc);
             if (hipStreamSynchronize(s) != hipSuccess) return fail(ctx, MASP_HIP_E_HIP);
@@ -1151,6 +1175,15 @@
     std::shared_lock<std::shared_mutex> lock(const_cast<masp_hip_ctx*>(ctx)->mu);
     if (slot >= MASP_HIP_MAX_CIRCUITS || !ctx->circ[slot]) return MASP_HIP_E_NOT_LOADED;
     *form = ctx->circ[slot]->hl_eval.n ? MASP_HIP_QUOTIENT_EVALUATION : MASP_HIP_QUOTIENT_COEFFICIENT;
+    return MASP_HIP_OK;
+}
+int masp_hip_circuit_window_row_multiples(const masp_hip_ctx* ctx, uint32_t slot, int32_t* sets) {
+    if (!ctx || !sets) return MASP_HIP_E_INVALID_ARG;
+    if (!ctx->children.empty()) return masp_hip_circuit_window_row_multiples(ctx->children[0], slot, sets);
+    std::shared_lock<std::shared_mutex> lock(const_cast<masp_hip_ctx*>(ctx)->mu);
+    if (slot >= MASP_HIP_MAX_CIRCUITS || !ctx->circ[slot]) return MASP_HIP_E_NOT_LOADED;
+    const Circuit& C = *ctx->circ[slot];
+    *sets = (C.hl.g.twin ? 1 : 0) | (C.hl_eval.n && C.hl_eval.g.twin ? 2 : 0) | (C.a.g.twin ? 4 : 0) | (C.b1.g.twin ? 8 : 0) | (C.b2.g.twin ? 16 : 0);
     return MASP_HIP_OK;
 }
 int masp_hip_circuit_eval_bases(const masp_hip_ctx* ctx, uint32_t slot, uint8_t* bases, size_t cap_points, size_t* n_points, uint32_t* input_cols,
@@ -1519,7 +1552,8 @@
     DevBuf<Xyzz<O>> res;
     DevBuf<uint8_t> d_out;
     int rc;
-    if ((rc = B.load_host(bases, (uint32_t)n, s, 0xffffffffu, window_bits, block_bits, (uint32_t)sub_lo, (uint32_t)sub_hi))) return fail(ctx, rc);
+    if ((rc = B.load_host(bases, (uint32_t)n, s, 0xffffffffu, window_bits, block_bits, (uint32_t)sub_lo, (uint32_t)sub_hi, ctx->twin_rows_msm)))
+        return fail(ctx, rc);
     if (B.import_status & (PT_BAD_FLAGS | PT_NOT_CANONICAL)) return MASP_HIP_E_PARAMS_FORMAT;
     if ((rc = ctx->tmp_scalars.upload((const Fr*)scalars, n * np, s)) || (rc = res.reserve(np)) || (rc = d_out.reserve(BYTES * np))) return fail(ctx, rc);
     if ((rc = msm_enqueue(s, B, ws, (const uint32_t*)ctx->tmp_scalars.p, n * 8, res.p, 1, (uint32_t)np))) return fail(ctx, rc);
diff --git a/masp_amd/hip.py b/masp_amd/hip.py
--- a/masp_amd/hip.py
+++ b/masp_amd/hip.py
@@ -110,10 +110,13 @@
         L.masp_hip_msm_g2_multi_ex.argtypes = [vp, vp, sz, vp, sz, C.c_int, C.c_int, sz, sz, vp, vp]
         L.masp_hip_ctx_set_boolean_block_bits.argtypes = [vp, C.c_int32]
         L.masp_hip_ctx_get_boolean_block_bits.argtypes = [vp, C.POINTER(C.c_int32)]
+        L.masp_hip_ctx_set_window_row_multiples.argtypes = [vp, C.c_int32]
+        L.masp_hip_ctx_get_window_row_multiples.argtypes = [vp, C.POINTER(C.c_int32)]
     if hasattr(L, "masp_hip_ctx_set_quotient_form"):
         L.masp_hip_ctx_set_quotient_form.argtypes = [vp, C.c_int32]
         L.masp_hip_ctx_get_quotient_form.argtypes = [vp, C.POINTER(C.c_int32)]
         L.masp_hip_circuit_quotient_form.argtypes = [vp, u32, C.POINTER(C.c_int32)]
+        L.masp_hip_circuit_window_row_multiples.argtypes = [vp, u32, C.POINTER(C.c_int32)]
         L.masp_hip_circuit_eval_bases.argtypes = [vp, u32, vp, sz, C.POINTER(sz), vp, sz, C.POINTER(sz)]
     if hasattr(L, "masp_hip_ctx_set_quotient_schedule"):
         L.masp_hip_ctx_set_quotient_schedule.argtypes = [vp, C.c_int32]
@@ -540,6 +543,15 @@
         self._check(self._L.masp_hip_ctx_get_boolean_block_bits(self._h, C.byref(v)))
         return int(v.value)
 
+    def set_window_row_multiples(self, v):
+        self._check(self._L.masp_hip_ctx_set_window_row_multiples(self._h, int(v)))
+
+    @property
+    def window_row_multiples(self):
+        v = C.c_int32(0)
+        self._check(self._L.masp_hip_ctx_get_window_row_multiples(self._h, C.byref(v)))
+        return int(v.value)
+
     def set_quotient_form(self, form):
         self._check(self._L.masp_hip_ctx_set_quotient_form(self._h, int(form)))
 
@@ -561,6 +573,11 @@
     def circuit_quotient_form(self, slot):
         v = C.c_int32(0)
         self._check(self._L.masp_hip_circuit_quotient_form(self._h, int(slot), C.byref(v)))
+        return int(v.value)
+
+    def circuit_window_row_multiples(self, slot):
+        v = C.c_int32(0)
+        self._check(self._L.masp_hip_circuit_window_row_multiples(self._h, int(slot), C.byref(v)))
         return int(v.value)
 
     def circuit_eval_bases(self, slot):
```

After: 1531 proofs/s (median of 6 runs). 2.1% higher.
